# shayneobrien/generative-models

Hardware: AMD Instinct MI355X
Metric: images/sec (28x28 MNIST) per D+G step, NSGAN bs=256 (higher is better)
Workload: dtype f32; 1 GPU; NSGAN MNIST bs=256 fp32 per GPU (BASELINE.json configs[1]); 784-400-20 MLPs, N=50000 synthetic Bernoulli images, parity-mode RNG protocol, Adam 2e-4, D_steps=1; global_batch=256, parallelism=dp1, ranks_seen=1, gradient_exchange=none (1 rank), timing=one 2064-step timed region, cold_start_inclusive=False

## Files before the change

generative_models_amd/_lib.py:

```python
import ctypes
import os
from ctypes import POINTER, c_char_p, c_float, c_int, c_int32, c_int64, c_void_p

HERE = os.path.dirname(os.path.abspath(__file__))
LIB_PATH = os.environ.get("GM_LIB_PATH") or os.path.join(HERE, "libgm_hip.so")

GM_EINVAL = -10001
ACT_ID, ACT_RELU, ACT_SIGMOID = 0, 1, 2
ACT = {"id": ACT_ID, None: ACT_ID, "relu": ACT_RELU, "sigmoid": ACT_SIGMOID}
LOSS = {"ns": 0, "mm": 1, "w": 2, "ls": 3, "ra": 4, "fisher": 5, "f_total_variation": 6,
        "f_forward_kl": 7, "f_reverse_kl": 8, "f_pearson": 9, "f_hellinger": 10,
        "f_jensen_shannon": 11}


class Slot(ctypes.Structure):
    _fields_ = [("ctr", c_void_p), ("mul", c_int32), ("add", c_int32), ("ring", c_int32),
                ("stride", c_int64)]


def slot(ctr=0, mul=0, add=0, ring=0, stride=0):
    return Slot(ctr or None, mul, add, ring, stride)


NO_SLOT = Slot(None, 0, 0, 0, 0)
# ... 74 lines not shown


DRAW_SAMPLER, DRAW_NORMAL, DRAW_UNIFORM, DRAW_INFO = 0, 1, 2, 3
GM_EUNSUPPORTED = -10002

_P = c_void_p

_SIGNATURES = {
    "gm_version": (c_int, []),
    "gm_arch": (c_char_p, []),
    "gm_last_error": (c_char_p, []),
    "gm_tick": (c_int, [_P, _P, c_int64]),
    "gm_copy_slot_f32": (c_int, [_P, _P, Slot, _P, Slot, c_int64]),
    "gm_gather_rows": (c_int, [_P, _P, c_int64, _P, Slot, _P, c_int64, c_int, c_int]),
    "gm_linear_fwd": (c_int, [_P, _P, c_int64, Slot, _P, _P, _P, c_int64, c_int, c_int, c_int,
                              c_int]),
    "gm_linear_bwd_dx": (c_int, [_P, _P, c_int64, _P, _P, c_int64, _P, c_int64, c_int, c_int,
                                 c_int, c_int]),
    "gm_linear_bwd_dw": (c_int, [_P, _P, c_int64, _P, c_int64, Slot, _P, _P, c_int, c_int, c_int,
                                 c_int]),
    "gm_gan_loss": (c_int, [_P, c_int, c_int, _P, _P, c_int, c_int, POINTER(c_float), c_int,
                            c_float, _P, Slot, _P, _P, _P, _P]),
    "gm_gan_loss_phase": (c_int, [_P, c_int, c_int, _P, _P, c_int, c_int, POINTER(c_float), c_int,
                                  c_float, _P, Slot, _P, _P, _P, _P, c_int, _P, c_float]),
    "gm_l1_rows_dp": (c_int, [_P, _P, c_int64, _P, c_int64, c_int, c_int, c_int, c_int, _P, _P, c_int64, _P]),
    "gm_began_dloss_dp": (c_int, [_P, _P, c_int, c_int, _P, _P, Slot]),
    "gm_std_sums": (c_int, [_P, _P, c_int64, c_int, c_int, _P, _P]),
    "gm_std_from_sums": (c_int, [_P, _P, c_int64, _P]),
    "gm_adam": (c_int, [_P, _P, _P, _P, _P, c_int64, _P, Slot, ctypes.c_double, ctypes.c_double,
                        ctypes.c_double, ctypes.c_double, c_float]),
    "gm_interp": (c_int, [_P, _P, Slot, _P, c_int64, _P, c_int64, _P, c_int64, c_int, c_int]),
    "gm_gp_u": (c_int, [_P, _P, _P, c_int64, _P, _P, c_int64, c_int, c_int]),
    "gm_gp_norm": (c_int, [_P, _P, c_int64, _P, c_int64, _P, c_float, c_float, c_float, c_int,
                           c_int]),
    "gm_gp_dw2": (c_int, [_P, _P, _P, c_int64, _P, c_int64, _P, c_int, c_int]),
    "gm_bir_reparam": (c_int, [_P, _P, c_int64, _P, Slot, _P, c_int64, c_int, c_int]),
    "gm_bir_mmd": (c_int, [_P, _P, c_int64, _P, Slot, _P, _P, c_int64, c_int, c_int, c_float]),
    "gm_vae_reparam": (c_int, [_P, _P, c_int64, _P, Slot, _P, c_int64, _P, Slot, c_int, c_int]),
    "gm_vae_reparam_bwd": (c_int, [_P, _P, c_int64, _P, Slot, _P, c_int64, _P, c_int64, c_int,
                                   c_int]),
    "gm_sqerr_sigmoid_bwd": (c_int, [_P, _P, c_int64, _P, c_int64, _P, c_int64, _P, c_int, c_int]),
    "gm_sum_finalize": (c_int, [_P, _P, c_int, c_float, _P, Slot]),
    "gm_sum_finalize_tick": (c_int, [_P, _P, c_int, c_float, _P, Slot, _P]),
    "gm_sum_finalize2_tick": (c_int, [_P, _P, c_int, c_float, _P, Slot, _P, c_int, c_float, _P, Slot, _P]),
    "gm_vae_reparam_wide": (c_int, [_P, _P, c_int64, _P, Slot, _P, c_int64, _P, c_int, c_int, c_int]),
    "gm_vae_bwd_mid": (c_int, [_P, _P, c_int64, _P, _P, c_int64, _P, Slot, _P, c_int64, _P, _P, c_int64, _P, c_int64,
                               c_int, c_int, c_int]),
    "gm_vae_reparam_fwd": (c_int, [_P, _P, c_int64, _P, Slot, _P, c_int64, _P, c_int, c_int, c_int, _P, _P, _P,
                                   c_int64, c_int, c_int]),
    "gm_linear_bwd_dw_adam": (c_int, [_P, _P, c_int64, _P, c_int64, Slot, _P, _P, c_int, c_int, c_int,
                                      _P, _P, _P, _P, _P, _P, _P, Slot, ctypes.c_double,
                                      ctypes.c_double, ctypes.c_double, ctypes.c_double, c_float]),
    "gm_linear_fwd_interp": (c_int, [_P, _P, c_int64, Slot, _P, _P, _P, c_int64, c_int, c_int, c_int, c_int,
                                     _P, Slot, _P, c_int64, _P, c_int64, c_int]),
    "gm_linear_fwd_gather": (c_int, [_P, _P, c_int64, Slot, _P, _P, _P, c_int64, c_int, c_int, c_int,
                                     c_int, _P, c_int64, _P, Slot, _P, c_int64, c_int, c_int]),
    "gm_linear_fwd_gather_bits": (c_int, [_P, _P, c_int64, Slot, _P, _P, _P, c_int64, c_int, c_int, c_int,
                                          c_int, _P, c_int, c_int64, _P, Slot, _P, c_int64, c_int, c_int]),
    "gm_gather_rows_bits": (c_int, [_P, _P, c_int, c_int64, _P, Slot, _P, c_int64, c_int, c_int]),
    "gm_linear_bwd_dx_head": (c_int, [_P, _P, c_int64, _P, _P, c_int64, _P, c_int64, c_int, c_int,
                                      c_int, c_int, POINTER(HeadBwdArgs)]),
    "gm_linear_bwd_dx_head_fold": (c_int, [_P, _P, c_int64, _P, _P, c_int64, _P, c_int64, c_int, c_int,
                                           c_int, c_int, POINTER(HeadBwdArgs), POINTER(HeadFoldArgs)]),
    "gm_linear_fwd_sqerr": (c_int, [_P, _P, c_int64, _P, _P, _P, c_int64, c_int, c_int, c_int, _P, c_int64,
                                    _P, c_int64, _P, c_int64]),
    "gm_linear_bwd_dx_reparam": (c_int, [_P, _P, c_int64, _P, _P, c_int64, c_int, c_int, c_int, _P, c_int64,
                                         _P, Slot, _P, c_int64]),
    "gm_linear_fwd_headpart": (c_int, [_P, _P, c_int64, Slot, _P, _P, _P, c_int64, c_int, c_int, c_int, c_int,
                                       _P, _P, _P, c_int64, _P]),
    "gm_linear_bwd_dw_adam_head_fold": (c_int, [_P, _P, c_int64, _P, c_int64, Slot, _P, _P, c_int, c_int,
                                                c_int, _P, _P, _P, _P, _P, _P, _P, Slot, ctypes.c_double,
                                                ctypes.c_double, ctypes.c_double, ctypes.c_double, c_float,
                                                POINTER(HeadBwdArgs), POINTER(HeadFoldArgs)]),
    "gm_gather_rows_bits_packed": (c_int, [_P, _P, c_int, c_int64, _P, Slot, _P, c_int]),
    "gm_linear_fwd_gather_bits_packed": (c_int, [_P, _P, c_int64, Slot, _P, _P, _P, c_int64, c_int, c_int, c_int,
                                                 c_int, _P, c_int, c_int64, _P, Slot, _P, c_int]),
    "gm_linear_fwd_headpart_bits": (c_int, [_P, _P, c_int64, Slot, _P, _P, _P, c_int64, c_int, c_int, c_int, c_int,
                                            _P, _P, _P, c_int64, _P, _P, c_int, c_int]),
    "gm_linear_bwd_dw_adam_head_fold_bits": (c_int, [_P, _P, c_int64, _P, c_int64, Slot, _P, _P, c_int, c_int,
                                                     c_int, _P, _P, _P, _P, _P, _P, _P, Slot, ctypes.c_double,
                                                     ctypes.c_double, ctypes.c_double, ctypes.c_double, c_float,
                                                     POINTER(HeadBwdArgs), POINTER(HeadFoldArgs), _P, c_int, c_int]),
    "gm_linear_bwd_dw_adam_pair": (c_int, [_P, POINTER(DwAdamArgs), POINTER(DwAdamArgs)]),
    "gm_linear_bwd_dw_adam_pair_finalize": (c_int, [_P, POINTER(DwAdamArgs), POINTER(DwAdamArgs),
                                                    POINTER(Finalize2Args)]),
    "gm_linear_bwd_dw_adam_head": (c_int, [_P, _P, c_int64, _P, c_int64, Slot, _P, _P, c_int, c_int,
                                           c_int, _P, _P, _P, _P, _P, _P, _P, Slot, ctypes.c_double,
                                           ctypes.c_double, ctypes.c_double, ctypes.c_double, c_float,
                                           POINTER(HeadBwdArgs)]),
    "gm_linear_bwd_dw_adam_head_ex": (c_int, [_P, _P, c_int64, _P, c_int64, Slot, _P, _P, c_int, c_int,
                                              c_int, _P, _P, _P, _P, _P, _P, _P, Slot, ctypes.c_double,
                                              ctypes.c_double, ctypes.c_double, ctypes.c_double, c_float,
                                              POINTER(HeadBwdArgs), c_int]),
    "gm_gp_dw2_store": (c_int, [_P, _P, _P, c_int64, _P, c_int64, _P, c_int, c_int]),
    "gm_head_gp": (c_int, [_P, _P, c_int64, _P, _P, _P, _P, c_int64, c_int, c_int]),
    "gm_head_bwd_fused": (c_int, [_P, _P, c_int64, _P, _P, _P, _P, _P, c_int64, _P, _P, _P, Slot,
                                  c_float, c_int, c_int, c_int, c_int, _P, _P, _P, _P, _P, Slot,
                                  ctypes.c_double, ctypes.c_double, ctypes.c_double,
                                  ctypes.c_double, c_float, _P]),
    "gm_head_fwd_loss": (c_int, [_P, c_int, c_int, _P, c_int64, _P, _P, c_int, c_int, c_int,
                                 POINTER(c_float), c_int, c_float, _P, _P, _P, _P, _P, c_int64]),
    "gm_head_fwd_loss_final": (c_int, [_P, c_int, c_int, _P, c_int64, _P, _P, c_int, c_int, c_int,
                                       POINTER(c_float), c_int, c_float, _P, _P, _P, _P, _P, c_int64,
                                       _P, Slot, _P, _P]),
    "gm_head_bwd": (c_int, [_P, _P, c_int64, _P, _P, _P, _P, c_int64, _P, _P, _P, Slot, c_float,
                            c_int, c_int, c_int]),
    "gm_clock_probe": (c_int, [_P, c_int, _P, _P]),
    "gm_stream_create": (c_int, [POINTER(c_void_p)]),
    "gm_stream_destroy": (c_int, [_P]),
    "gm_stream_wait_event": (c_int, [_P, _P]),
    "gm_l1_rows": (c_int, [_P, _P, c_int64, _P, c_int64, c_int, c_int, c_int, _P, _P, c_int64, _P]),
    "gm_began_dloss": (c_int, [_P, _P, c_int, _P, _P, Slot]),
    "gm_began_update": (c_int, [_P, _P, _P, _P, c_float, c_float, c_int64, _P]),
    "gm_adam_scaled": (c_int, [_P, _P, _P, _P, _P, c_int64, _P, Slot, ctypes.c_double, ctypes.c_double,
                               ctypes.c_double, ctypes.c_double, c_float, _P]),
    "gm_linear_bwd_dx_add": (c_int, [_P, _P, c_int64, _P, _P, c_int64, _P, c_int64, c_int, c_int,
                                     c_int, c_int, _P, c_int64, c_float]),
    "gm_std_all": (c_int, [_P, _P, c_int64, c_int, c_int, _P, _P]),
    "gm_dragan_xhat": (c_int, [_P, _P, c_int64, _P, Slot, _P, Slot, _P, c_float, _P, c_int64, c_int,
                               c_int]),
    "gm_dragan_rows": (c_int, [_P, _P, _P, c_int64, _P, c_int64, _P, _P, c_float, c_float, c_float,
                               c_int, c_int]),
    "gm_dragan_head_bwd": (c_int, [_P, _P, c_int64, _P, c_int64, _P, _P, _P, _P, _P, c_int64, c_int,
                                   c_int]),
    "gm_fisher_commit": (c_int, [_P, _P]),
    "gm_dragan_head_bwd_store": (c_int, [_P, _P, c_int64, _P, c_int64, _P, _P, _P, _P, _P, c_int64, c_int,
                                   c_int]),
    "gm_info_q_loss": (c_int, [_P, _P, c_int64, _P, Slot, c_int64, c_int, c_int, c_int, c_int, c_float,
                               _P, c_int64, _P, Slot]),
    "gm_info_q_loss_dp": (c_int, [_P, _P, c_int64, _P, Slot, c_int64, c_int, c_int, c_int, c_int, c_int, c_float,
                                  _P, c_int64, _P, Slot]),
    "gm_act_bwd": (c_int, [_P, _P, _P, _P, c_int64, c_int]),
    "gm_randperm_prefix": (c_int, [ctypes.c_uint64, c_int64, c_int, _P]),
    "gm_mt19937_skip": (c_int, [_P, c_int64, ctypes.c_uint64]),
    "gm_comm_create": (c_int, [c_int, c_int, c_int64, POINTER(c_void_p), _P]),
    "gm_comm_connect": (c_int, [_P, _P]),
    "gm_comm_destroy": (c_int, [_P]),
    "gm_comm_error": (c_int, [_P, POINTER(c_int)]),
    "gm_comm_info": (c_int, [_P, POINTER(c_int)]),
    "gm_rccl_available": (c_int, []),
    "gm_rccl_unique_id": (c_int, [_P]),
    "gm_rccl_comm_create": (c_int, [c_int, c_int, _P, POINTER(c_void_p)]),
    "gm_rccl_allreduce_f32": (c_int, [_P, _P, _P, c_int64]),
    "gm_rccl_comm_destroy": (c_int, [_P]),
    "gm_comm_set_exchange": (c_int, [_P, c_int]),
    "gm_comm_set_max_blocks": (c_int, [_P, c_int]),
    "gm_comm_set_wait_seconds": (c_int, [_P, ctypes.c_double]),
    "gm_comm_buffer": (c_int, [_P, POINTER(c_void_p), POINTER(c_int64)]),
    "gm_allreduce_f32": (c_int, [_P, _P, _P, c_int64]),
    "gm_allreduce_adam_f32": (c_int, [_P, _P, _P, c_int64, _P, _P, _P, _P, Slot, ctypes.c_double,
                                      ctypes.c_double, ctypes.c_double, ctypes.c_double, c_float, _P]),
    "gm_allreduce_scalars": (c_int, [_P, _P, _P, c_int]),
    "gm_stage_in": (c_int, [_P, POINTER(StageSeg), c_int, Slot, c_int]),
    "gm_stage_in_gated": (c_int, [_P, POINTER(StageSeg), c_int, Slot, c_int, _P, Slot, ctypes.c_double, _P,
                                  c_int]),
    "gm_host_device_ptr": (c_int, [_P, POINTER(c_void_p)]),
    "gm_host_replay": (c_int, [_P, c_int64, POINTER(DrawOp), c_int, c_int]),
    "gm_host_replay_threads": (c_int, [c_int]),
    "gm_numpy_legacy_normal_f32": (c_int, [_P, _P, _P, _P, ctypes.c_double, ctypes.c_double, c_int64, _P, c_int]),
    "gm_fill_submit": (c_int64, [_P, c_int64, POINTER(DrawOp), c_int, c_int, _P, c_int64]),
    "gm_fill_wait": (c_int, [c_int64]),
    "gm_fill_completed": (c_int64, []),
    "gm_fill_reset": (c_int, []),
    "gm_host_replay_flavour": (c_int, [c_int]),
    "gm_graph_begin": (c_int, [_P]),
    "gm_graph_end": (c_int, [_P, POINTER(c_void_p)]),
# ... 61 lines not shown
```

generative_models_amd/csrc/gm_gemm.hip:

```cpp
#include "gm_common.h"
#include "gm_head.h"
#include "gm_gather.h"
#include "gm_ldsdma.h"

#include <cstdlib>
#include <type_traits>

typedef float f32x16 __attribute__((ext_vector_type(16)));

#ifdef GM_STAMPS
namespace gm_stamps {
constexpr int WAVES = 16, IDS = 40, HDR = 8, MAXB = 512, SLOT_WORDS = HDR + 2 * MAXB + WAVES * IDS * 2, SLOTS = 64;
static unsigned long long* host_buf = nullptr;
static int host_tile = 0, host_next = 0;
struct Ctx { unsigned long long* slot; int tile; };
__device__ __forceinline__ void rec(const Ctx& c, int tile, int id) {
    if (!c.slot || tile != c.tile || (threadIdx.x & 63)) return;
    __builtin_amdgcn_sched_barrier(0);
    unsigned long long* w = c.slot + HDR + 2 * MAXB + ((threadIdx.x >> 6) * IDS + id) * 2;
    w[0] = clock64(); w[1] = wall_clock64();
    __builtin_amdgcn_sched_barrier(0);
}
__device__ __forceinline__ void edge(const Ctx& c, bool exit_, int tile, int M, int N, int K, int mode) {
    if (!c.slot || threadIdx.x) return;
// ... 44 lines not shown
    int epi;
    int accumulate;
    gm_slot a_slot, b_slot;
    int tn;
    int lds_tm, lds_mpx;
    int dma;
    int vec_epi;
    const float* ip_eps; gm_slot ip_slot;
    const float* ip_x; int64_t ip_ldx;
    float* ip_out; int64_t ip_ldo;
    int ip_rows;
    gm_adam_epi adam;
    const float* hd_w2; const float* hd_b2; float* hd_part; int64_t hd_ldp; float* hd_snap;
    const float* sq_x; int64_t sq_ldx; float* sq_dA; int64_t sq_lda; float* sq_part; int64_t sq_ldp;
    const float* rp_ml; int64_t rp_ldml; const float* rp_eps; gm_slot rp_slot; float* rp_dml; int64_t rp_ldd;
    int rp_Z;
    const float* fold_w2;
    const float* add;
    int64_t ldadd;
    float add_scale;
    const uint32_t* pk_bits; int pk_wpr; int pk_rows;
    gm_label_src lb; const float* lb_E; int lb_C;
#ifdef GM_STAMPS
    gm_stamps::Ctx stamp;
#endif
};

template <bool SL>
__device__ __forceinline__ const float* slot_base(const float* P, const gm_slot& s) {
    if constexpr (SL) return P + gm_slot_offset(s);
    return P;
}
inline bool has_slot(const gm_slot& s) { return s.ctr != nullptr || s.add != 0; }

__device__ __forceinline__ float4 pk_expand(uint32_t word, int e) {
    const uint32_t v = word >> (e & 31);
    return make_float4((float)(v & 1u), (float)((v >> 1) & 1u), (float)((v >> 2) & 1u), (float)((v >> 3) & 1u));
}



template <bool VEC>
__device__ __forceinline__ float4 raw_kc(const float* __restrict__ P, int64_t ld, int x, int X,
                                         int kb, int K) {
    const float* row = P + (int64_t)min(x, X - 1) * ld;
    if (VEC)
        return *reinterpret_cast<const float4*>(row + min(kb, K - 4));
    return make_float4(row[min(kb + 0, K - 1)], row[min(kb + 1, K - 1)], row[min(kb + 2, K - 1)],
                       row[min(kb + 3, K - 1)]);
}
__device__ __forceinline__ float4 fix_kc(float4 v, int x, int X, int kb, int K) {
    const bool okx = x < X;
    v.x = (okx && kb + 0 < K) ? v.x : 0.f;
    v.y = (okx && kb + 1 < K) ? v.y : 0.f;
    v.z = (okx && kb + 2 < K) ? v.z : 0.f;
    v.w = (okx && kb + 3 < K) ? v.w : 0.f;
    return v;
}

__device__ __forceinline__ float4 raw_xc(const float* __restrict__ P, int64_t ld, int x, int X,
                                         int kb, int K) {
    const float* col = P + min(x, X - 1);
    return make_float4(col[(int64_t)min(kb + 0, K - 1) * ld], col[(int64_t)min(kb + 1, K - 1) * ld],
                       col[(int64_t)min(kb + 2, K - 1) * ld], col[(int64_t)min(kb + 3, K - 1) * ld]);
}
__device__ __forceinline__ float4 fix_xc(float4 v, int x, int X, int kb, int K, int ones_col,
                                         int ones_from = 0) {
    const bool okx = x < X, oc = (x == ones_col);
    v.x = (kb + 0 < K) ? (okx ? v.x : ((oc && kb + 0 >= ones_from) ? 1.f : 0.f)) : 0.f;
    v.y = (kb + 1 < K) ? (okx ? v.y : ((oc && kb + 1 >= ones_from) ? 1.f : 0.f)) : 0.f;
    v.z = (kb + 2 < K) ? (okx ? v.z : ((oc && kb + 2 >= ones_from) ? 1.f : 0.f)) : 0.f;
    v.w = (kb + 3 < K) ? (okx ? v.w : ((oc && kb + 3 >= ones_from) ? 1.f : 0.f)) : 0.f;
    return v;
}

__device__ __forceinline__ float fwd_value(const GemmP& p, float v, int n) {
    if (p.bias) v += p.bias[n];
    if (p.epi == GM_ACT_RELU) v = fmaxf(v, 0.f);
    else if (p.epi == GM_ACT_SIGMOID) v = gm_sigmoid(v);
    return v;
}

template <int MODE, bool LBL = false>
__device__ __forceinline__ void store_element(const GemmP& p, float v, int m, int n) {
    if (MODE == MODE_FWD) {
        if constexpr (LBL) v += p.lb_E[(int64_t)n * p.lb_C + gm_row_label(p.lb, m, p.lb_C)];
        v = fwd_value(p, v, n);
        p.C[(int64_t)m * p.ldc + n] = v;
        if (p.ip_out && m < p.ip_rows) {
            const float ev = (p.ip_eps + gm_slot_offset(p.ip_slot))[m];
            p.ip_out[(int64_t)m * p.ip_ldo + n] = gm_interp_unfused(ev, p.ip_x[(int64_t)m * p.ip_ldx + n], v);
        }
    } else if (MODE == MODE_DX) {
        if (p.add) v += p.add_scale * p.add[(int64_t)m * p.ldadd + n];
        if (p.epi == GM_ACT_RELU) {
            v = (p.aux[(int64_t)m * p.ldaux + n] > 0.f) ? v : 0.f;
        } else if (p.epi == GM_ACT_SIGMOID) {
            const float y = p.aux[(int64_t)m * p.ldaux + n];
            v = v * (y * (1.f - y));
        }
        float* cp = p.C + (int64_t)m * p.ldc + n;
        *cp = p.accumulate ? (*cp + v) : v;
        if (p.rp_dml) {
            const int Z = p.rp_Z;
            const float mu = p.rp_ml[(int64_t)m * p.rp_ldml + n], lv = p.rp_ml[(int64_t)m * p.rp_ldml + Z + n];
            const float e = (p.rp_eps + gm_slot_offset(p.rp_slot))[(int64_t)m * Z + n];
            p.rp_dml[(int64_t)m * p.rp_ldd + n] = v + 0.5f * (2.f * mu);
            p.rp_dml[(int64_t)m * p.rp_ldd + Z + n] = ((v * e) * expf(lv / 2.f)) / 2.f + 0.5f * (expf(lv) - 1.f);
        }
    } else {
        const bool is_b = (n == p.n_real);
        float* cp = is_b ? (p.db + m) : (p.C + (int64_t)m * p.ldc + n);
        if (p.accumulate) v += *cp;
        *cp = v;
        if (p.adam.enabled) {
            const int64_t o = is_b ? (int64_t)m : ((int64_t)m * p.ldc + n);
            float* pp = (is_b ? p.adam.pb : p.adam.pW) + o;
            float* mm = (is_b ? p.adam.mb : p.adam.mW) + o;
            float* vv = (is_b ? p.adam.vb : p.adam.vW) + o;
            const int64_t si = gm_slot_index(p.adam.sched_slot);
            const float step_size = p.adam.sched[2 * si], bc2_sqrt = p.adam.sched[2 * si + 1];
            float P = *pp, M = *mm, V = *vv;
            adam_update(P, v, M, V, step_size, bc2_sqrt, p.adam.omb1, p.adam.b2, p.adam.omb2,
                        p.adam.eps, p.adam.wd, p.adam.clamp);
            *pp = P; *mm = M; *vv = V;
        }
    }
}

__device__ __forceinline__ float4 ld4(const float* q) { return *reinterpret_cast<const float4*>(q); }
__device__ __forceinline__ void st4(float* q, float4 v) { *reinterpret_cast<float4*>(q) = v; }

template <int MODE>
__device__ __forceinline__ void store4(const GemmP& p, float4 v, int m, int n) {
    if (MODE == MODE_FWD) {
        if (p.bias) { const float4 b = ld4(p.bias + n); v.x += b.x; v.y += b.y; v.z += b.z; v.w += b.w; }
        if (p.epi == GM_ACT_RELU) { v.x = fmaxf(v.x, 0.f); v.y = fmaxf(v.y, 0.f); v.z = fmaxf(v.z, 0.f); v.w = fmaxf(v.w, 0.f); }
        else if (p.epi == GM_ACT_SIGMOID) { v.x = gm_sigmoid(v.x); v.y = gm_sigmoid(v.y); v.z = gm_sigmoid(v.z); v.w = gm_sigmoid(v.w); }
        st4(p.C + (int64_t)m * p.ldc + n, v);
        if (p.ip_out && m < p.ip_rows) {
            const float ev = (p.ip_eps + gm_slot_offset(p.ip_slot))[m];
            const float4 x = ld4(p.ip_x + (int64_t)m * p.ip_ldx + n);
            st4(p.ip_out + (int64_t)m * p.ip_ldo + n,
                make_float4(gm_interp_unfused(ev, x.x, v.x), gm_interp_unfused(ev, x.y, v.y),
                            gm_interp_unfused(ev, x.z, v.z), gm_interp_unfused(ev, x.w, v.w)));
        }
    } else if (MODE == MODE_DX) {
        if (p.add) {
            const float4 a = ld4(p.add + (int64_t)m * p.ldadd + n);
            v.x += p.add_scale * a.x; v.y += p.add_scale * a.y; v.z += p.add_scale * a.z; v.w += p.add_scale * a.w;
        }
        if (p.epi == GM_ACT_RELU) {
            const float4 y = ld4(p.aux + (int64_t)m * p.ldaux + n);
            v.x = (y.x > 0.f) ? v.x : 0.f; v.y = (y.y > 0.f) ? v.y : 0.f; v.z = (y.z > 0.f) ? v.z : 0.f; v.w = (y.w > 0.f) ? v.w : 0.f;
        } else if (p.epi == GM_ACT_SIGMOID) {
            const float4 y = ld4(p.aux + (int64_t)m * p.ldaux + n);
            v.x = v.x * (y.x * (1.f - y.x)); v.y = v.y * (y.y * (1.f - y.y));
            v.z = v.z * (y.z * (1.f - y.z)); v.w = v.w * (y.w * (1.f - y.w));
        }
        float* cp = p.C + (int64_t)m * p.ldc + n;
        if (p.accumulate) { const float4 c = ld4(cp); v.x = c.x + v.x; v.y = c.y + v.y; v.z = c.z + v.z; v.w = c.w + v.w; }
        st4(cp, v);
    } else {
        const int64_t o = (int64_t)m * p.ldc + n;
        if (p.accumulate) { const float4 c = ld4(p.C + o); v.x += c.x; v.y += c.y; v.z += c.z; v.w += c.w; }
        st4(p.C + o, v);
        if (p.adam.enabled) {
            const int64_t si = gm_slot_index(p.adam.sched_slot);
            const float step_size = p.adam.sched[2 * si], bc2_sqrt = p.adam.sched[2 * si + 1];
            float4 P = ld4(p.adam.pW + o), M = ld4(p.adam.mW + o), V = ld4(p.adam.vW + o);
            adam_update(P.x, v.x, M.x, V.x, step_size, bc2_sqrt, p.adam.omb1, p.adam.b2, p.adam.omb2, p.adam.eps, p.adam.wd, p.adam.clamp);
            adam_update(P.y, v.y, M.y, V.y, step_size, bc2_sqrt, p.adam.omb1, p.adam.b2, p.adam.omb2, p.adam.eps, p.adam.wd, p.adam.clamp);
            adam_update(P.z, v.z, M.z, V.z, step_size, bc2_sqrt, p.adam.omb1, p.adam.b2, p.adam.omb2, p.adam.eps, p.adam.wd, p.adam.clamp);
            adam_update(P.w, v.w, M.w, V.w, step_size, bc2_sqrt, p.adam.omb1, p.adam.b2, p.adam.omb2, p.adam.eps, p.adam.wd, p.adam.clamp);
            st4(p.adam.pW + o, P); st4(p.adam.mW + o, M); st4(p.adam.vW + o, V);
        }
    }
}

template <int MODE>
__device__ __forceinline__ void store_group(const GemmP& p, float4 v, int m, int n, int ncap) {
    const int nreal = (MODE == MODE_DW) ? p.n_real : p.N;
    if (n + 3 < nreal && n + 3 < ncap) { store4<MODE>(p, v, m, n); return; }
    if (n < p.N && n < ncap) store_element<MODE>(p, v.x, m, n);
    if (n + 1 < p.N && n + 1 < ncap) store_element<MODE>(p, v.y, m, n + 1);
    if (n + 2 < p.N && n + 2 < ncap) store_element<MODE>(p, v.z, m, n + 2);
    if (n + 3 < p.N && n + 3 < ncap) store_element<MODE>(p, v.w, m, n + 3);
}

__device__ __forceinline__ int red_idx(int w, int row, int col) {
    return (w * 32 + row) * 32 + (col ^ ((((row >> 2) ^ row) & 1) << 4));
}

template <int MODE, int WAVES, int ROWS = 32, bool LBL = false>
__device__ __forceinline__ void reduce_and_store(const GemmP& p, const float* red, int t, int m0,
                                                 int n0, int ncap = 0x7fffffff, int rcap = 32) {
    if (MODE == MODE_FWD && p.hd_part) {
#pragma unroll
        for (int e = 0; e < 1024 / (WAVES * 64); ++e) {
            const int row = (t >> 5) + e * (WAVES * 2), col = t & 31;
            const bool live = !(ROWS < 32 && row >= ROWS) && row < rcap;
            float v = 0.f;
            if (live) {
#pragma unroll
                for (int ww = 0; ww < WAVES; ++ww) v += red[red_idx(ww, row, col)];
            }
            const int m = m0 + row, n = n0 + col;
            const bool ok = live && m < p.M && n < p.N && n < ncap;
            float pv = 0.f;
            if (ok) {
                const float w = p.hd_w2[n];
                const float y = fwd_value(p, v, n);
                p.C[(int64_t)m * p.ldc + n] = y;
                pv = y * w;
                if (m == 0 && p.hd_snap) {
                    p.hd_snap[n] = w;
                    if (n == 0) p.hd_snap[p.N] = p.hd_b2[0];
                }
            }
#pragma unroll
            for (int o = 16; o > 0; o >>= 1) pv += __shfl_xor(pv, o, 64);
            if (col == 0 && live && m < p.M) p.hd_part[(int64_t)m * p.hd_ldp + (n0 >> 5)] = pv;
        }
        return;
    }
    if (MODE == MODE_FWD && p.sq_part) {
#pragma unroll
        for (int e = 0; e < 1024 / (WAVES * 64); ++e) {
            const int row = (t >> 5) + e * (WAVES * 2), col = t & 31;
            const bool live = !(ROWS < 32 && row >= ROWS) && row < rcap;
            float v = 0.f;
            if (live) {
#pragma unroll
                for (int ww = 0; ww < WAVES; ++ww) v += red[red_idx(ww, row, col)];
            }
            const int m = m0 + row, n = n0 + col;
            const bool ok = live && m < p.M && n < p.N && n < ncap;
            float pv = 0.f;
            if (ok) {
                const float r = fwd_value(p, v, n);
                p.C[(int64_t)m * p.ldc + n] = r;
                const float d = p.sq_x[(int64_t)m * p.sq_ldx + n] - r;
                pv = d * d;
                const float go = -(2.f * d);
                p.sq_dA[(int64_t)m * p.sq_lda + n] = (go * (1.f - r)) * r;
            }
#pragma unroll
            for (int o = 16; o > 0; o >>= 1) pv += __shfl_xor(pv, o, 64);
            if (col == 0 && live && m < p.M) p.sq_part[(int64_t)m * p.sq_ldp + (n0 >> 5)] = pv;
        }
        return;
    }
#pragma unroll
    for (int e = 0; e < 1024 / (WAVES * 64); ++e) {
        const int row = (t >> 5) + e * (WAVES * 2), col = t & 31;
        if ((ROWS < 32 && row >= ROWS) || row >= rcap) continue;
        float v = 0.f;
#pragma unroll
        for (int ww = 0; ww < WAVES; ++ww) v += red[red_idx(ww, row, col)];
        const int m = m0 + row, n = n0 + col;
        if (m >= p.M || n >= p.N || n >= ncap) continue;
        store_element<MODE, LBL>(p, v, m, n);
    }
}

__device__ __forceinline__ float4 keep4(bool ok, float4 v) {
    return make_float4(ok ? v.x : 0.f, ok ? v.y : 0.f, ok ? v.z : 0.f, ok ? v.w : 0.f);
}

template <int NMFMA, int NDSR, int NVMEM, int NDSW>
__device__ __forceinline__ void lds_stage_schedule() {
    constexpr int NMEM = NDSR + NVMEM + NDSW;
    int done = 0;
#pragma unroll
    for (int q = 0; q < NMFMA; ++q) {
        __builtin_amdgcn_sched_group_barrier(0x008, 1, 0);
        const int upto = (NMEM * (q + 1) + NMFMA - 1) / NMFMA;
#pragma unroll
        for (int i = 0; i < 8; ++i) {
            if (done < upto) {
                if (done < NDSR) __builtin_amdgcn_sched_group_barrier(0x100, 1, 0);
                else if (done < NDSR + NVMEM) __builtin_amdgcn_sched_group_barrier(0x020, 1, 0);
                else __builtin_amdgcn_sched_group_barrier(0x200, 1, 0);
                ++done;
            }
        }
    }
}

template <int MODE, int BM, int BN, int WTM, int WTN, int WK, int KU>
struct LdsCfg {
    static constexpr int WM = BM / WTM, WN = BN / WTN, NW = WM * WN * WK, NT = 64 * NW, BK = 8 * WK * KU;
    static constexpr int TI = WTM / 32, TJ = WTN / 32;
    static constexpr bool B_KC = (MODE == MODE_FWD);
    static constexpr int LDK = BK + 4, LDXB = BN + 4;
    static constexpr int A_SZ = BM * LDK;
    static constexpr int B_SZ = B_KC ? BN * LDK : BK * LDXB;
    static constexpr int STAGE = A_SZ + B_SZ;
    static constexpr int NBUF = 3;
    static constexpr int RED = WK * BM * BN;
    static constexpr int FLOATS = (NBUF * STAGE > RED) ? NBUF * STAGE : RED;
};

template <int MODE, int BM, int BN, int WTM, int WTN, int WK, int KU, int PD, int NS>
__global__ __launch_bounds__(64 * (BM / WTM) * (BN / WTN) * WK) void gemm_lds_kernel(GemmP p) {
    using C = LdsCfg<MODE, BM, BN, WTM, WTN, WK, KU>;
    constexpr int NT = C::NT, BK = C::BK, LDK = C::LDK, LDXB = C::LDXB, TI = C::TI, TJ = C::TJ;
    static_assert(MODE != MODE_DW, "forward (A, B k-contiguous) and input gradient (B = W[k][n]) only");
    static_assert(PD >= 2, "two stages are stored before the first barrier");
    __shared__ __attribute__((aligned(16))) float lds[C::FLOATS];

    const int t = threadIdx.x, lane = t & 63, w = t >> 6;
    const int r = lane & 31, h = lane >> 5;
    const int wk = w / (C::WM * C::WN), wmn = w % (C::WM * C::WN), wm = wmn / C::WN, wn = wmn % C::WN;
    const int b = blockIdx.x, xcd = b & 7, l = b >> 3;
    const int tile_m = xcd * p.lds_mpx + l / p.tn, tile_n = l % p.tn;
    if (tile_m >= p.lds_tm) return;
    const int m0 = tile_m * BM, n0 = tile_n * BN;
    const float* A = p.A;
    const float* B = p.B;
#ifdef GM_STAMPS
    const gm_stamps::Ctx st_slot = p.stamp; const int st_tile = (int)blockIdx.x;
#endif
    GM_STAMP_EDGE(p, false, st_tile, MODE + 10);
    GM_STAMP(st_slot, st_tile, 0);

    constexpr int KQ = BK / 4;
    constexpr int XQ = BN / 4;
    constexpr int UA = BM * KQ, CA = (UA + NT - 1) / NT;
    constexpr int UB = C::B_KC ? BN * KQ : BK * XQ, CB = (UB + NT - 1) / NT;
    const float* baseA[CA];
    const float* baseB[CB];
#pragma unroll
    for (int i = 0; i < CA; ++i) {
        const int u = min(t + i * NT, UA - 1);
        baseA[i] = A + (int64_t)min(m0 + u / KQ, p.M - 1) * p.lda + 4 * (u % KQ);
    }
#pragma unroll
    for (int i = 0; i < CB; ++i) {
        const int u = min(t + i * NT, UB - 1);
        if (C::B_KC) baseB[i] = B + (int64_t)min(n0 + u / KQ, p.N - 1) * p.ldb + 4 * (u % KQ);
        else baseB[i] = B + min(n0 + 4 * (u % XQ), p.N - 4);
    }
    auto load_a = [&](const float* base, int i, int q, bool inside) -> float4 {
        if (inside) return *reinterpret_cast<const float4*>(base + q * BK);
// ... 368 lines not shown
        }
    };

    float fw[FOLD == 1 ? MI : 1];
    if constexpr (FOLD == 1) {
#pragma unroll
        for (int e = 0; e < MI; ++e) fw[e] = (am + e < p.M) ? p.fold_w2[min(am + e, p.M - 1)] : 0.f;
    }
    f32x4 acc[MI][NI];
#pragma unroll
    for (int e = 0; e < MI; ++e)
#pragma unroll
        for (int f = 0; f < NI; ++f) acc[e][f] = f32x4{0.f, 0.f, 0.f, 0.f};

    const int nq = (nchunks - w + WAVES - 1) / WAVES;
    const bool special = (ones_col >= n0 && ones_col < n0 + 16 * NI) || (p.K & 15) || OF;
    auto run = [&](auto special_tag) {
        constexpr bool SPECIAL = decltype(special_tag)::value;
        if (nq > 0) issue(w);
        GM_STAMP(st_slot, st_tile, 17);
        if constexpr (FOLD == 1) fold_fill_lds(*fold, sds, fold->R);
        for (int q = 0; q < nq; ++q) {
            const int c = w + q * WAVES;
            slab::wait_vm<0>();
            if (q < 8) GM_STAMP(st_slot, st_tile, 20 + 2 * q);
            ILV<MI> ra[4]; ILV<NI> rb[4];
#pragma unroll
            for (int s = 0; s < 4; ++s) {
                const int row = 4 * s + g4;
                ra[s] = *reinterpret_cast<const ILV<MI>*>(buf + row * (16 * MI) + MI * i16);
                rb[s] = *reinterpret_cast<const ILV<NI>*>(buf + 256 * MI + row * (16 * NI) + NI * i16);
            }
            slab::wait_lgkm0();
            if (q + 1 < nq) issue(c + WAVES);
#pragma unroll
            for (int s = 0; s < 4; ++s) {
                const int k = 16 * c + 4 * s + g4;
                float fa[MI], fb[NI];
#pragma unroll
                for (int e = 0; e < MI; ++e) {
                    float v = ra[s].v[e];
                    if constexpr (FOLD == 1) v = (v > 0.f) ? sds[min(k, p.K - 1)] * fw[e] : 0.f;
                    if constexpr (SPECIAL) v = (k < p.K) ? v : 0.f;
                    fa[e] = v;
                }
#pragma unroll
                for (int f = 0; f < NI; ++f) {
                    float v = rb[s].v[f];
                    if constexpr (SPECIAL) {
                        float one = 1.f;
                        if constexpr (OF) one = (k >= p.ones_from) ? 1.f : 0.f;
                        v = (bn + f == ones_col) ? one : v;
                    }
                    fb[f] = v;
                }
#pragma unroll
                for (int e = 0; e < MI; ++e)
#pragma unroll
                    for (int f = 0; f < NI; ++f)
                        acc[e][f] = __builtin_amdgcn_mfma_f32_16x16x4f32(fa[e], fb[f], acc[e][f], 0, 0, 0);
            }
            GM_STAMP_AFTER(acc[MI - 1][NI - 1][0]);
            if (q < 8) GM_STAMP(st_slot, st_tile, 21 + 2 * q);
        }
    };
    if (special) run(std::true_type{}); else run(std::false_type{});
    GM_STAMP(st_slot, st_tile, 9);
    dw_il_reduce<MI, NI>(p, red, acc, m0, n0, true);
    GM_STAMP(st_slot, st_tile, 12);
    GM_STAMP_EDGE(p, true, st_tile, MODE_DW + 20);
}

template <int MODE, bool DMA, int MI, int NI> struct RedSize {
    static constexpr int base = 16 * 32 * 32;
    static constexpr int onepass = (MODE == MODE_DW && MI * NI > 4) ? 16 * 256 * MI * NI : 0;
    static constexpr int dma = (MODE == MODE_DW && DMA) ? 16 * (MI + NI) * 256 : 0;
    static constexpr int m1 = base > onepass ? base : onepass;
    static constexpr int value = m1 > dma ? m1 : dma;
};

template <int MODE, bool VEC, int WAVES, int G, bool XV, int MI, int NI, bool OF = false, int FOLD = 0, bool DMA = false,
          bool TP = false, bool PK = false, bool SL = true, bool LBL = false>
__device__ __forceinline__ void gemm16_body(const GemmP& p, float* red, int bx, int by,
                                            float* sds = nullptr, const FoldP* fold = nullptr, int gx = 0) {
    static_assert(!TP || (FOLD == 1 && !DMA), "two-phase losses: folded weight gradient, operands through registers");
    static_assert(FOLD == 0 || (FOLD == 1 && MODE == MODE_DW && XV) || (FOLD == 2 && MODE == MODE_DX && VEC),
                  "folded head: 16-byte operand paths only");
    static_assert(G == 1, "per-chunk schedule (G stays in the kernel names so that they keep their shape across rounds)");
    static_assert(!PK || (WAVES == 16 && !DMA && ((MODE == MODE_FWD && VEC) || (MODE == MODE_DW && XV))),
                  "bit-packed operand rows: 16-byte operand paths through registers only");
    if constexpr (DMA && MODE == MODE_DW && XV && WAVES == 16 && FOLD != 2) {
        gemm16_dw_dma<MI, NI, OF, FOLD, SL>(p, red, bx, by, sds, fold, gx);
        return;
    }
    const int t = threadIdx.x;
    const int lane = t & 63, w = t >> 6;
    const int i16 = lane & 15, g4 = lane >> 4;
    const int m0 = by * (16 * MI), n0 = bx * (16 * NI);
#ifdef GM_STAMPS
    const gm_stamps::Ctx st_slot = p.stamp; const int st_tile = by * (int)gridDim.x + bx;
#endif
    GM_STAMP_EDGE(p, false, st_tile, MODE);
    GM_STAMP(st_slot, st_tile, 0);

    const float* A = slot_base<SL>(p.A, p.a_slot);
    const float* B = slot_base<SL>(p.B, p.b_slot);
    const int b_cols = (MODE == MODE_DW) ? p.n_real : p.N;
    const int ones_col = (MODE == MODE_DW && p.db) ? p.n_real : -1;
    const int nchunks = (p.K + 15) >> 4;
    GM_STAMP_AFTER(A); GM_STAMP_AFTER(B); GM_STAMP_AFTER(nchunks);
    GM_STAMP(st_slot, st_tile, 16);

    float4 fw[FOLD == 1 ? MI : 1];
    float fds[FOLD == 2 ? MI : 1];
    const int xq_ld = lane & 3, xe_ld = (lane >> 2) & 3;
    constexpr bool XMAP_A = MODE == MODE_DW && XV, XMAP_B = MODE != MODE_FWD && XV;
    const int ia = XMAP_A ? sigma16(i16) : i16, ib = XMAP_B ? sigma16(i16) : i16;
    if constexpr (FOLD == 1) {
#pragma unroll
        for (int mi = 0; mi < MI; ++mi)
            fw[mi] = *reinterpret_cast<const float4*>(
                p.fold_w2 + min(m0 + 16 * mi + 4 * xq_ld, p.M - 4));
    }
    auto load_a = [&](int c, int mi) -> float4 {
        const int kb = 16 * c + 4 * g4, x0 = m0 + 16 * mi;
        if (MODE == MODE_DW) {
            if (XV) return raw_xc4_16(A, p.lda, x0, p.M, c, p.K, lane);
            return raw_xc(A, p.lda, x0 + i16, p.M, kb, p.K);
        }
        return raw_kc<VEC>(A, p.lda, x0 + i16, p.M, kb, p.K);
    };
    auto load_b = [&](int c, int ni) -> float4 {
        const int kb = 16 * c + 4 * g4, x0 = n0 + 16 * ni;
        if (MODE == MODE_FWD) return raw_kc<VEC>(B, p.ldb, x0 + i16, p.N, kb, p.K);
        if (XV) return raw_xc4_16(B, p.ldb, x0, b_cols, c, p.K, lane);
        return raw_xc(B, p.ldb, x0 + i16, b_cols, kb, p.K);
    };
    auto fix_a = [&](float4 v, int c, int mi, float4 wk) -> float4 {
        const int kb = 16 * c + 4 * g4, x = m0 + 16 * mi + ia;
        if constexpr (FOLD == 1)
            v = fold_dh4(v, sds[min(16 * c + 4 * g4 + xe_ld, p.K - 1)], fw[mi]);
        if constexpr (FOLD == 2) v = fold_dh4(v, fds[mi], wk);
        if (MODE == MODE_DW)
            return fix_xc(XV ? lane48_transpose(v, lane) : v, x, p.M, kb, p.K, -1);
        return fix_kc(v, x, p.M, kb, p.K);
    };
    auto fix_b = [&](float4 v, int c, int ni) -> float4 {
        const int kb = 16 * c + 4 * g4, x = n0 + 16 * ni + ib;
        if (MODE == MODE_FWD) return fix_kc(v, x, p.N, kb, p.K);
        return fix_xc(XV ? lane48_transpose(v, lane) : v, x, b_cols, kb, p.K, ones_col, OF ? p.ones_from : 0);
    };

    f32x4 acc[MI][NI];
#pragma unroll
    for (int mi = 0; mi < MI; ++mi)
#pragma unroll
        for (int ni = 0; ni < NI; ++ni) acc[mi][ni] = f32x4{0.f, 0.f, 0.f, 0.f};

    const int nq = (nchunks - w + WAVES - 1) / WAVES;
    auto consume = [&](const float4 (&ra)[MI], const float4 (&rb)[NI], float4 wk, int q) {
        const int cq = w + q * WAVES;
        float4 fa[MI], fb[NI];
#pragma unroll
        for (int mi = 0; mi < MI; ++mi) fa[mi] = fix_a(ra[mi], cq, mi, wk);
#pragma unroll
        for (int ni = 0; ni < NI; ++ni) fb[ni] = fix_b(rb[ni], cq, ni);
        GM_STAMP_AFTER(fa[MI - 1].x); GM_STAMP_AFTER(fb[NI - 1].x);
// ... 100 lines not shown
        }
        for (int q = q0; q < q_pk; ++q) do_chunk(yes, no, q);
        for (int q = max(q0, q_pk); q < nq_s; ++q) do_chunk(no, no, q);
    } else {
    int q_first = 0;
    if constexpr (FOLD != 0) {
        float4 ra[MI], rb[NI];
        float4 wk = make_float4(0.f, 0.f, 0.f, 0.f);
        const bool have = nq > 0;
        float4 pv[4];
        if constexpr (FOLD == 1 && !TP) {
            if (t < fold->R) fold_part_load(*fold, t, pv);
        }
        if constexpr (FOLD == 2) {
            if (t < 16 * MI) fold_part_load(*fold, min(m0 + t, fold->R - 1), pv);
        }
        if (have) {
#pragma unroll
            for (int mi = 0; mi < MI; ++mi) ra[mi] = load_a(w, mi);
#pragma unroll
            for (int ni = 0; ni < NI; ++ni) rb[ni] = load_b(w, ni);
            wk = load_wk(w);
        }
        GM_STAMP(st_slot, st_tile, 17);
        if constexpr (FOLD == 1 && !TP) fold_fill_lds_pre(*fold, sds, fold->R, pv);
        else if constexpr (FOLD == 2) {
            if (t < 16 * MI) {
                float s_, ds_, l_;
                fold_row_of(*fold, min(m0 + t, fold->R - 1), fold_score_of(*fold, pv), s_, ds_, l_);
                sds[t] = ds_;
            }
            GM_STAMP(st_slot, st_tile, 15);
            __syncthreads();
#pragma unroll
            for (int mi = 0; mi < MI; ++mi) fds[mi] = sds[16 * mi + i16];
        }
        else fold_prologue();
        GM_STAMP(st_slot, st_tile, 13);
        if (have) consume(ra, rb, wk, 0);
        q_first = 1;
    }
    for (int q = q_first; q < nq; ++q) {
        float4 ra[MI], rb[NI];
        const int cc = w + q * WAVES;
#pragma unroll
        for (int mi = 0; mi < MI; ++mi) ra[mi] = load_a(cc, mi);
#pragma unroll
        for (int ni = 0; ni < NI; ++ni) rb[ni] = load_b(cc, ni);
        const float4 wk = load_wk(cc);
        consume(ra, rb, wk, q);
    }
    }
    GM_STAMP(st_slot, st_tile, 9);
    if constexpr (MODE == MODE_DW && WAVES == 16 && MI * NI > 4) {
        if (p.vec_epi) {
            dw_reduce_onepass<MI, NI, false, XMAP_A>(p, red, acc, m0, n0, false);
            GM_STAMP(st_slot, st_tile, 12);
            GM_STAMP_EDGE(p, true, st_tile, MODE);
            return;
        }
    }
#pragma unroll
    for (int bm = 0; bm < (MI + 1) / 2; ++bm)
#pragma unroll
        for (int bn = 0; bn < (NI + 1) / 2; ++bn) {
            if (bm + bn > 0) __syncthreads();
#pragma unroll
            for (int rgi = 0; rgi < 4; ++rgi) {
                const int row = XMAP_A ? sigma16(g4 * 4 + rgi) : g4 * 4 + rgi;
                red[red_idx(w, row, ib)] = acc[2 * bm][2 * bn][rgi];
                if (2 * bn + 1 < NI) red[red_idx(w, row, 16 + ib)] = acc[2 * bm][(2 * bn + 1 < NI) ? 2 * bn + 1 : 0][rgi];
                if (2 * bm + 1 < MI) {
                    constexpr int MIX = MI > 1 ? MI - 1 : 0;
                    const int mu = (2 * bm + 1 < MI) ? 2 * bm + 1 : MIX;
                    red[red_idx(w, 16 + row, ib)] = acc[mu][2 * bn][rgi];
                    if (2 * bn + 1 < NI)
                        red[red_idx(w, 16 + row, 16 + ib)] = acc[mu][(2 * bn + 1 < NI) ? 2 * bn + 1 : 0][rgi];
                }
            }
            __syncthreads();
            if (bm + bn == 0) GM_STAMP(st_slot, st_tile, 10);
            reduce_and_store<MODE, WAVES, (MI > 1 ? 32 : 16), LBL>(p, red, t, m0 + 32 * bm, n0 + 32 * bn,
                                                              (2 * bn + 1 < NI) ? 0x7fffffff : n0 + 32 * bn + 16,
                                                              (2 * bm + 1 < MI) ? 32 : 16);
        }
    GM_STAMP(st_slot, st_tile, 12);
    GM_STAMP_EDGE(p, true, st_tile, MODE);
}

template <int MODE, bool VEC, int WAVES, int G, bool XV, int MI, int NI, bool DMA = false, bool SL = false>
__global__ __launch_bounds__(WAVES * 64) void gemm16_kernel(GemmP p) {
    __shared__ __attribute__((aligned(16))) float red[(WAVES == 16) ? RedSize<MODE, DMA, MI, NI>::value : WAVES * 32 * 32];
    gemm16_body<MODE, VEC, WAVES, G, XV, MI, NI, false, 0, DMA, false, false, SL>(p, red, blockIdx.x, blockIdx.y, nullptr, nullptr,
                                                                                  (int)gridDim.x);
}

template <bool VEC, int MI, int NI>
__global__ __launch_bounds__(1024) void gemm16_fwd_label_kernel(GemmP p) {
    __shared__ __attribute__((aligned(16))) float red[RedSize<MODE_FWD, false, MI, NI>::value];
    gemm16_body<MODE_FWD, VEC, 16, 1, false, MI, NI, false, 0, false, false, false, false, true>(p, red, blockIdx.x, blockIdx.y,
                                                                                                nullptr, nullptr, (int)gridDim.x);
}

template <int MODE, bool VEC, int G, bool XV, int MI, int NI, bool OF = false, bool FOLDED = false, bool DMA = false,
          bool TP = false, bool PK = false>
__device__ __forceinline__ void gemm16_with_head(const GemmP& p, const HeadBwdP& hp, int hrows,
                                                 int hblocks) {
    __shared__ __attribute__((aligned(16))) float red[RedSize<MODE, DMA, MI, NI>::value];
    __shared__ float sds[FOLDED ? FOLD_MAX_ROWS : 1];
    constexpr int FOLD = FOLDED ? (MODE == MODE_DW ? 1 : 2) : 0;
    if ((int)blockIdx.y < hrows) {
        const int bid = blockIdx.y * gridDim.x + blockIdx.x;
        if (bid < hblocks) head_bwd_body<TP>(hp, bid, sds);
        return;
    }
    gemm16_body<MODE, VEC, 16, G, XV, MI, NI, OF, FOLD, DMA, TP, PK, false>(p, red, blockIdx.x, blockIdx.y - hrows, sds, &hp.fold,
                                                                            (int)gridDim.x);
}

template <bool VEC, int G, bool XV, int MI, int NI, bool OF = false, bool FOLDED = false, bool DMA = false>
__global__ __launch_bounds__(1024) void gemm16_dw_head_kernel(GemmP p, HeadBwdP hp, int hrows,
                                                              int hblocks) {
    gemm16_with_head<MODE_DW, VEC, G, XV, MI, NI, OF, FOLDED, DMA>(p, hp, hrows, hblocks);
}

__global__ __launch_bounds__(1024) void gemm16_fwd_bits_kernel(GemmP p) {
    __shared__ __attribute__((aligned(16))) float red[RedSize<MODE_FWD, false, 2, 2>::value];
    gemm16_body<MODE_FWD, true, 16, 1, false, 2, 2, false, 0, false, false, true, false>(p, red, blockIdx.x, blockIdx.y);
}
__global__ __launch_bounds__(1024) void gemm16_dw_head_bits_kernel(GemmP p, HeadBwdP hp, int hrows, int hblocks) {
    gemm16_with_head<MODE_DW, false, 1, true, 2, 3, false, true, false, false, true>(p, hp, hrows, hblocks);
}

template <int MI, int NI>
__global__ __launch_bounds__(1024) void gemm16_dw_head_tp_kernel(GemmP p, HeadBwdP hp, int hrows, int hblocks) {
    gemm16_with_head<MODE_DW, false, 1, true, MI, NI, false, true, false, true>(p, hp, hrows, hblocks);
}

template <int G, int MI, int NI, bool FOLDED = false>
__global__ __launch_bounds__(1024) void gemm16_dx_head_kernel(GemmP p, HeadBwdP hp, int hrows,
                                                              int hblocks) {
    gemm16_with_head<MODE_DX, true, G, true, MI, NI, false, FOLDED>(p, hp, hrows, hblocks);
}

inline bool aligned16(const void* p) { return (reinterpret_cast<uintptr_t>(p) & 15) == 0; }

template <bool VEC, int G, int MI, int NI>
__global__ __launch_bounds__(1024) void gemm16_fwd_gather_kernel(GemmP p, GatherP gp, int grows,
                                                                 int gblocks) {
    __shared__ __attribute__((aligned(16))) float red[16 * 32 * 32];
    if ((int)blockIdx.y < grows) {
        const int bid = blockIdx.y * gridDim.x + blockIdx.x;
        if (bid < gblocks) gather_body(gp, bid);
        return;
    }
    gemm16_body<MODE_FWD, VEC, 16, G, false, MI, NI>(p, red, blockIdx.x, blockIdx.y - grows);
}

template <bool SL, bool GATHER>
__global__ __launch_bounds__(256) void gemm16_k32_fwd_kernel(GemmP p, GatherP gp, int grows, int gblocks) {
    if constexpr (GATHER) {
        if ((int)blockIdx.y < grows) {
            const int bid = blockIdx.y * gridDim.x + blockIdx.x;
            if (bid < gblocks) gather_body(gp, bid);
            return;
        }
    }
    const int by = (int)blockIdx.y - (GATHER ? grows : 0), bx = blockIdx.x;
    const int t = threadIdx.x, lane = t & 63, w = __builtin_amdgcn_readfirstlane(t >> 6);
    const int i16 = lane & 15, g4 = lane >> 4;
    const int m0 = 32 * by + 16 * (w >> 1), n0 = 64 * bx + 32 * (w & 1);
#ifdef GM_STAMPS
    const gm_stamps::Ctx st_slot = p.stamp; const int st_tile = by * (int)gridDim.x + bx;
#endif
    GM_STAMP_EDGE(p, false, st_tile, MODE_FWD);
    GM_STAMP(st_slot, st_tile, 0);
    if (m0 >= p.M || n0 >= p.N) { GM_STAMP_EDGE(p, true, st_tile, MODE_FWD); return; }
    const float* A = slot_base<SL>(p.A, p.a_slot);
    const float* B = slot_base<SL>(p.B, p.b_slot);
    float4 ra[2], rb[2][2];
#pragma unroll
    for (int c = 0; c < 2; ++c) {
        const int kb = 16 * c + 4 * g4;
        ra[c] = raw_kc<true>(A, p.lda, m0 + i16, p.M, kb, p.K);
#pragma unroll
        for (int ni = 0; ni < 2; ++ni) rb[c][ni] = raw_kc<true>(B, p.ldb, n0 + 16 * ni + i16, p.N, kb, p.K);
    }
    f32x4 part[2][2];
#pragma unroll
    for (int c = 0; c < 2; ++c) {
        const int kb = 16 * c + 4 * g4;
        const float4 fa = fix_kc(ra[c], m0 + i16, p.M, kb, p.K);
#pragma unroll
        for (int ni = 0; ni < 2; ++ni) {
            const float4 fb = fix_kc(rb[c][ni], n0 + 16 * ni + i16, p.N, kb, p.K);
            f32x4 c4 = f32x4{0.f, 0.f, 0.f, 0.f};
            c4 = __builtin_amdgcn_mfma_f32_16x16x4f32(fa.x, fb.x, c4, 0, 0, 0);
            c4 = __builtin_amdgcn_mfma_f32_16x16x4f32(fa.y, fb.y, c4, 0, 0, 0);
            c4 = __builtin_amdgcn_mfma_f32_16x16x4f32(fa.z, fb.z, c4, 0, 0, 0);
            c4 = __builtin_amdgcn_mfma_f32_16x16x4f32(fa.w, fb.w, c4, 0, 0, 0);
            part[c][ni] = c4;
            if (c == 0 && ni == 0) { GM_STAMP_AFTER(fa.x); GM_STAMP_AFTER(fb.x); GM_STAMP(st_slot, st_tile, 1); }
        }
    }
    GM_STAMP_AFTER(part[1][1][0]);
    GM_STAMP(st_slot, st_tile, 2);
    float v[2][4];
#pragma unroll
    for (int ni = 0; ni < 2; ++ni) {
        const int n = min(n0 + 16 * ni + i16, p.N - 1);
        const float bv = p.bias ? p.bias[n] : 0.f;
#pragma unroll
        for (int r = 0; r < 4; ++r) {
            float x = 0.f;
            x += part[0][ni][r];
            x += part[1][ni][r];
            if (p.bias) x += bv;
            v[ni][r] = x;
        }
    }
    if (p.epi == GM_ACT_RELU) {
#pragma unroll
        for (int ni = 0; ni < 2; ++ni)
#pragma unroll
            for (int r = 0; r < 4; ++r) v[ni][r] = fmaxf(v[ni][r], 0.f);
    } else if (p.epi == GM_ACT_SIGMOID) {
#pragma unroll
        for (int ni = 0; ni < 2; ++ni)
#pragma unroll
            for (int r = 0; r < 4; ++r) v[ni][r] = gm_sigmoid(v[ni][r]);
    }
#pragma unroll
    for (int ni = 0; ni < 2; ++ni) {
        const int n = n0 + 16 * ni + i16;
#pragma unroll
        for (int r = 0; r < 4; ++r) {
            const int m = m0 + 4 * g4 + r;
            if (m < p.M && n < p.N) p.C[(int64_t)m * p.ldc + n] = v[ni][r];
        }
    }
    if (p.ip_out) {
#pragma unroll
        for (int ni = 0; ni < 2; ++ni) {
            const int n = n0 + 16 * ni + i16;
#pragma unroll
            for (int r = 0; r < 4; ++r) {
                const int m = m0 + 4 * g4 + r;
                if (m < p.M && n < p.N && m < p.ip_rows) {
                    const float ev = (p.ip_eps + gm_slot_offset(p.ip_slot))[m];
                    p.ip_out[(int64_t)m * p.ip_ldo + n] = gm_interp_unfused(ev, p.ip_x[(int64_t)m * p.ip_ldx + n], v[ni][r]);
                }
            }
        }
    }
    GM_STAMP(st_slot, st_tile, 12);
    GM_STAMP_EDGE(p, true, st_tile, MODE_FWD);
}

template <int G, bool XV, int MI, int NI, bool DMA = false, bool SLA = true, bool SLB = true>
__global__ __launch_bounds__(1024) void gemm16_dw_pair_kernel(GemmP pa, GemmP pb, int na, int tna,
                                                              int tnb) {
    __shared__ __attribute__((aligned(16))) float red[RedSize<MODE_DW, DMA, MI, NI>::value];
    const int id = blockIdx.x;
    if (id < na) gemm16_body<MODE_DW, false, 16, G, XV, MI, NI, false, 0, DMA, false, false, SLA>(pa, red, id % tna, id / tna);
    else gemm16_body<MODE_DW, false, 16, G, XV, MI, NI, false, 0, DMA, false, false, SLB>(pb, red, (id - na) % tnb, (id - na) / tnb);
}

template <int G, bool XV, int MI, int NI, bool DMA = false, bool SLA = true, bool SLB = true>
__global__ __launch_bounds__(1024) void gemm16_dw_pair_fin_kernel(GemmP pa, GemmP pb, int na, int tna, int tnb,
                                                                  gm_fin2 f) {
    __shared__ __attribute__((aligned(16))) float red[RedSize<MODE_DW, DMA, MI, NI>::value];
    const int id = (int)blockIdx.x - 1;
    if (id < 0) gm_fin2_sums(f, reinterpret_cast<double*>(red));
    else if (id < na) gemm16_body<MODE_DW, false, 16, G, XV, MI, NI, false, 0, DMA, false, false, SLA>(pa, red, id % tna, id / tna);
    else gemm16_body<MODE_DW, false, 16, G, XV, MI, NI, false, 0, DMA, false, false, SLB>(pb, red, (id - na) % tnb, (id - na) / tnb);
    __syncthreads();
    if (threadIdx.x == 0) {
        const unsigned int arrived = __hip_atomic_fetch_add(f.done, 1u, __ATOMIC_RELAXED, __HIP_MEMORY_SCOPE_AGENT);
        if (arrived == gridDim.x - 1) {
            __hip_atomic_store(f.done, 0u, __ATOMIC_RELAXED, __HIP_MEMORY_SCOPE_AGENT);
            if (f.tick) *f.tick += 1;
        }
    }
}

template <int MODE>
int vec_epi_ok(const GemmP& p) {
    if (!aligned16(p.C) || p.ldc % 4 != 0) return 0;
    if (MODE == MODE_FWD) {
        if (p.bias && !aligned16(p.bias)) return 0;
        if (p.ip_out && !(aligned16(p.ip_out) && aligned16(p.ip_x) && p.ip_ldo % 4 == 0 && p.ip_ldx % 4 == 0)) return 0;
    } else if (MODE == MODE_DX) {
        if (p.epi != GM_ACT_ID && !(aligned16(p.aux) && p.ldaux % 4 == 0)) return 0;
        if (p.add && !(aligned16(p.add) && p.ldadd % 4 == 0)) return 0;
    } else {
        if (p.adam.enabled && !(aligned16(p.adam.pW) && aligned16(p.adam.mW) && aligned16(p.adam.vW))) return 0;
    }
    return 1;
}

struct Rider {
    const HeadBwdP* head = nullptr;
    const GatherP* gather = nullptr;
    const GemmP* pair = nullptr;
    bool pair_xvec = false;
    const gm_fin2* fin = nullptr;
};

enum { T22 = 0, T24, T42, T12, T23, T32 };
inline int tile_mi(int t) { return t == T42 ? 4 : t == T32 ? 3 : t == T12 ? 1 : 2; }
inline int tile_ni(int t) { return t == T24 ? 4 : t == T23 ? 3 : 2; }

template <int MODE>
int pick_tile(const GemmP& p) {
    const int tm = (p.M + TM - 1) / TM, tn = (p.N + TN - 1) / TN;
    int t = T22;
    if (tm * tn > 256 && (p.K + 15) / 16 >= 32) t = (tn >= tm) ? T24 : T42;
    else if (tm * tn <= 128 && p.M > 16) t = T12;
    if (MODE == MODE_DW) {
        if (t == T24 && tm * ((p.N + 47) / 48) <= 256) t = T23;
        else if (t == T42 && tn * ((p.M + 47) / 48) <= 256) t = T32;
        else if (t == T22 && tm * tn > 256) {
            if (tn >= tm && tm * ((p.N + 47) / 48) <= 256) t = T23;
            else if (tn < tm && tn * ((p.M + 47) / 48) <= 256) t = T32;
        }
    }
    if (MODE == MODE_FWD && t == T42 && !p.hd_part && !p.sq_part && tn * ((p.M + 47) / 48) <= 256) t = T32;
    return t;
}

#define GM_TILE_SWITCH(tile, dma, LAUNCH)                                           \
    do {                                                                            \
        switch (tile) {                                                             \
        case T24: LAUNCH(2, 4, false); break;                                       \
        case T42: LAUNCH(4, 2, false); break;                                       \
        case T12: LAUNCH(1, 2, false); break;                                       \
        case T23: if (dma) LAUNCH(2, 3, true); else LAUNCH(2, 3, false); break;     \
        case T32: if (dma) LAUNCH(3, 2, true); else LAUNCH(3, 2, false); break;     \
        default: LAUNCH(2, 2, false); break;                                        \
        }                                                                           \
    } while (0)

template <int MODE>
int launch(hipStream_t s, const GemmP& p_in, bool vec, bool xvec = false, const Rider& rider = Rider()) {
    const HeadBwdP* head = rider.head;
    const bool folded = head && head->fold.enabled;
    GemmP p = p_in;
    p.vec_epi = vec_epi_ok<MODE>(p);
#ifdef GM_STAMPS
    p.stamp.slot = gm_stamps::host_buf ? gm_stamps::host_buf + (size_t)(gm_stamps::host_next++ % gm_stamps::SLOTS) * gm_stamps::SLOT_WORDS
                                       : nullptr;
    p.stamp.tile = gm_stamps::host_tile;
#endif
    const bool xv = xvec && MODE != MODE_FWD;
    const bool slots = has_slot(p.a_slot) || has_slot(p.b_slot);
    if (slots && (folded || p.pk_bits)) {
        gm_set_error("ring slots on the operands of a folded-head / bit-packed launch are not supported");
        return GM_EINVAL;
    }
    const bool ride_head = head && !slots;
    auto dma_ok = [&](const GemmP& q, bool qxv) {
        constexpr int dma_min_k = 768;
        return MODE == MODE_DW && qxv && q.K >= dma_min_k && q.M >= 4 && q.n_real >= 4 &&
               ((int64_t)q.K + 64) * (q.lda > q.ldb ? q.lda : q.ldb) < (1ll << 31);
    };
    p.dma = dma_ok(p, xv);
    if (p.pk_bits) {
        if constexpr (MODE == MODE_FWD) {
            if (!vec || !p.hd_part || rider.gather || p.ip_out) {
                gm_set_error("bit-packed rows: the forward needs 16-byte aligned operands and the folded head's partial dots");
                return GM_EINVAL;
            }
            const dim3 bgrid((p.N + 31) / 32, (p.M + 31) / 32);
            hipLaunchKernelGGL(gemm16_fwd_bits_kernel, bgrid, dim3(1024), 0, s, p);
            GM_LAUNCH_RET();
        } else if constexpr (MODE == MODE_DW) {
            if (!head || !folded || head->fold.enabled != 1 || !xv || p.ones_from > 0 || rider.pair) {
                gm_set_error("bit-packed rows: the weight gradient needs the folded head of a separable loss and "
                             "16-byte aligned operands");
                return GM_EINVAL;
            }
            p.dma = false;
            const dim3 bgrid((p.N + 47) / 48, (p.M + 31) / 32);
            const int hblocks = gm_head_bwd_blocks(*head);
            const int hrows = (hblocks + (int)bgrid.x - 1) / (int)bgrid.x;
            hipLaunchKernelGGL(gemm16_dw_head_bits_kernel, dim3(bgrid.x, bgrid.y + hrows), dim3(1024), 0, s, p, *head,
                               hrows, hblocks);
            GM_LAUNCH_RET();
        } else {
// ... 8 lines not shown
                if (head) hipLaunchKernelGGL(head_bwd_kernel, dim3(gm_head_bwd_blocks(*head)), dim3(1024), 0, s, *head);
                if (rider.gather)
                    hipLaunchKernelGGL(gather_rows_kernel, dim3(gm_gather_blocks(*rider.gather, 4)), dim3(256), 0, s, *rider.gather);
                return launch_lds<MODE>(s, p, cfg);
            }
        }
    }
    if constexpr (MODE == MODE_FWD) {
        if (vec && p.K <= 32 && !head && !p.hd_part && !p.sq_part) {
            const dim3 kgrid((p.N + 63) / 64, (p.M + 31) / 32);
            if (rider.gather) {
                const GatherP& gp = *rider.gather;
                const int gblocks = gm_gather_blocks(gp, 4);
                const int grows = (gblocks + (int)kgrid.x - 1) / (int)kgrid.x;
                const dim3 ggrid(kgrid.x, kgrid.y + grows);
                if (slots) hipLaunchKernelGGL((gemm16_k32_fwd_kernel<true, true>), ggrid, dim3(256), 0, s, p, gp, grows, gblocks);
                else hipLaunchKernelGGL((gemm16_k32_fwd_kernel<false, true>), ggrid, dim3(256), 0, s, p, gp, grows, gblocks);
            } else {
                if (slots) hipLaunchKernelGGL((gemm16_k32_fwd_kernel<true, false>), kgrid, dim3(256), 0, s, p, GatherP{}, 0, 0);
                else hipLaunchKernelGGL((gemm16_k32_fwd_kernel<false, false>), kgrid, dim3(256), 0, s, p, GatherP{}, 0, 0);
            }
            GM_LAUNCH_RET();
        }
    }
    const int tile = pick_tile<MODE>(p);
    const int mi = tile_mi(tile), ni = tile_ni(tile);
    const dim3 grid((p.N + 16 * ni - 1) / (16 * ni), (p.M + 16 * mi - 1) / (16 * mi));
    if constexpr (MODE == MODE_DW) {
        if (ride_head) {
            const int hblocks = gm_head_bwd_blocks(*head);
            const int hrows = (hblocks + (int)grid.x - 1) / (int)grid.x;
            const dim3 hgrid(grid.x, grid.y + hrows);
            if (folded && (!xv || p.ones_from > 0)) {
                gm_set_error("folded head: the weight gradient needs 16-byte aligned operands and no stacked rows");
                return GM_EINVAL;
            }
#define GM_LH(X, OFV, FD) GM_TILE_SWITCH(tile, p.dma && (X), GM_LH1_##X##_##OFV##_##FD)
#define GM_LHK(X, OFV, FD, MI_, NI_, D_) hipLaunchKernelGGL((gemm16_dw_head_kernel<false, 1, X, MI_, NI_, OFV, FD, ((X) && (D_))>), hgrid, dim3(1024), 0, s, p, *head, hrows, hblocks)
#define GM_LH1_true_false_true(MI_, NI_, D_) GM_LHK(true, false, true, MI_, NI_, D_)
#define GM_LH1_true_true_false(MI_, NI_, D_) GM_LHK(true, true, false, MI_, NI_, D_)
#define GM_LH1_true_false_false(MI_, NI_, D_) GM_LHK(true, false, false, MI_, NI_, D_)
#define GM_LH1_false_true_false(MI_, NI_, D_) GM_LHK(false, true, false, MI_, NI_, D_)
#define GM_LH1_false_false_false(MI_, NI_, D_) GM_LHK(false, false, false, MI_, NI_, D_)
            if (folded && head->fold.enabled == 2) {
                p.dma = false;
#define GM_LHTP(MI_, NI_, D_) hipLaunchKernelGGL((gemm16_dw_head_tp_kernel<MI_, NI_>), hgrid, dim3(1024), 0, s, p, *head, hrows, hblocks)
                GM_TILE_SWITCH(tile, false, GM_LHTP);
#undef GM_LHTP
            } else if (folded) GM_LH(true, false, true);
            else if (xv) { if (p.ones_from > 0) GM_LH(true, true, false); else GM_LH(true, false, false); }
            else { if (p.ones_from > 0) GM_LH(false, true, false); else GM_LH(false, false, false); }
#undef GM_LH1_false_false_false
#undef GM_LH1_false_true_false
#undef GM_LH1_true_false_false
#undef GM_LH1_true_true_false
#undef GM_LH1_true_false_true
#undef GM_LHK
#undef GM_LH
            GM_LAUNCH_RET();
        }
    }
    if constexpr (MODE == MODE_DX) {
        if (ride_head && vec && xv && (tile == T22 || tile == T12)) {
            const int hblocks = gm_head_bwd_blocks(*head);
            const int hrows = (hblocks + (int)grid.x - 1) / (int)grid.x;
            const dim3 hgrid(grid.x, grid.y + hrows);
            if (tile == T12) {
                if (folded) hipLaunchKernelGGL((gemm16_dx_head_kernel<1, 1, 2, true>), hgrid, dim3(1024), 0, s, p, *head, hrows, hblocks);
                else hipLaunchKernelGGL((gemm16_dx_head_kernel<1, 1, 2, false>), hgrid, dim3(1024), 0, s, p, *head, hrows, hblocks);
            } else {
                if (folded) hipLaunchKernelGGL((gemm16_dx_head_kernel<1, 2, 2, true>), hgrid, dim3(1024), 0, s, p, *head, hrows, hblocks);
                else hipLaunchKernelGGL((gemm16_dx_head_kernel<1, 2, 2, false>), hgrid, dim3(1024), 0, s, p, *head, hrows, hblocks);
            }
            GM_LAUNCH_RET();
        }
    }
    if (folded) {
        gm_set_error("folded head: this launch configuration cannot carry it (needs the riding kernels: 16-byte "
                     "aligned operands)");
        return GM_EINVAL;
    }
    if (head)
        hipLaunchKernelGGL(head_bwd_kernel, dim3(gm_head_bwd_blocks(*head)), dim3(1024), 0, s, *head);
    if constexpr (MODE == MODE_FWD) {
        if (rider.gather) {
            const GatherP& gp = *rider.gather;
            if (vec && (tile == T22 || tile == T12)) {
                const int gblocks = gm_gather_blocks(gp, 16);
                const int grows = (gblocks + (int)grid.x - 1) / (int)grid.x;
                const dim3 ggrid(grid.x, grid.y + grows);
                if (tile == T12) hipLaunchKernelGGL((gemm16_fwd_gather_kernel<true, 1, 1, 2>), ggrid, dim3(1024), 0, s, p, gp, grows, gblocks);
                else hipLaunchKernelGGL((gemm16_fwd_gather_kernel<true, 1, 2, 2>), ggrid, dim3(1024), 0, s, p, gp, grows, gblocks);
                GM_LAUNCH_RET();
            }
            hipLaunchKernelGGL(gather_rows_kernel, dim3(gm_gather_blocks(gp, 4)), dim3(256), 0, s, gp);
        }
    }
    if constexpr (MODE == MODE_DW) {
        if (rider.pair) {
            GemmP pb = *rider.pair;
            pb.vec_epi = vec_epi_ok<MODE_DW>(pb);
            if (xv && rider.pair_xvec && tile != T12 && pb.K == p.K) {
                const bool dma = p.dma && dma_ok(pb, true);
                p.dma = pb.dma = dma;
                const int tna = (int)grid.x, na = (int)(grid.x * grid.y);
                const int tnb = (pb.N + 16 * ni - 1) / (16 * ni), tmb = (pb.M + 16 * mi - 1) / (16 * mi);
                const dim3 pgrid(na + tnb * tmb);
                const bool sl_b = has_slot(pb.a_slot) || has_slot(pb.b_slot);
#define GM_LP2(K_, GRID_, MI_, NI_, D_, ...)                                                                              \
    do {                                                                                                                  \
        if (slots) hipLaunchKernelGGL((K_<1, true, MI_, NI_, D_, true, true>), GRID_, dim3(1024), 0, s, __VA_ARGS__);     \
        else if (sl_b) hipLaunchKernelGGL((K_<1, true, MI_, NI_, D_, false, true>), GRID_, dim3(1024), 0, s, __VA_ARGS__); \
        else hipLaunchKernelGGL((K_<1, true, MI_, NI_, D_, false, false>), GRID_, dim3(1024), 0, s, __VA_ARGS__);         \
    } while (0)
#define GM_LP(MI_, NI_, D_) GM_LP2(gemm16_dw_pair_kernel, pgrid, MI_, NI_, D_, p, pb, na, tna, tnb)
#define GM_LPF(MI_, NI_, D_) GM_LP2(gemm16_dw_pair_fin_kernel, dim3(pgrid.x + 1), MI_, NI_, D_, p, pb, na, tna, tnb, *rider.fin)
                if (rider.fin) GM_TILE_SWITCH(tile, dma, GM_LPF);
                else GM_TILE_SWITCH(tile, dma, GM_LP);
#undef GM_LP2
#undef GM_LPF
#undef GM_LP
                GM_LAUNCH_RET();
            }
            Rider none;
            int rc = launch<MODE_DW>(s, p_in, vec, xvec, none);
            if (rc) return rc;
            rc = launch<MODE_DW>(s, pb, false, rider.pair_xvec, none);
            if (rc || !rider.fin) return rc;
            const gm_fin2& f = *rider.fin;
            return gm_sum_finalize2_tick(s, f.pa, f.na, f.sa, f.oa, f.slot_a, f.pb, f.nb, f.sb, f.ob, f.slot_b, f.tick);
        }
    }
    if (MODE == MODE_DX && slots) { gm_set_error("ring slots: forward and weight-gradient operands only"); return GM_EINVAL; }
#define GM_L16K(V, X, MI_, NI_, D_)                                                                                          \
    do {                                                                                                                     \
        if (MODE != MODE_DX && slots)                                                                                        \
            hipLaunchKernelGGL((gemm16_kernel<MODE, V, 16, 1, X, MI_, NI_, (MODE == MODE_DW && (X) && (D_)), MODE != MODE_DX>), grid, dim3(1024), 0, s, p); \
        else                                                                                                                 \
            hipLaunchKernelGGL((gemm16_kernel<MODE, V, 16, 1, X, MI_, NI_, (MODE == MODE_DW && (X) && (D_)), false>), grid, dim3(1024), 0, s, p); \
    } while (0)
#define GM_L16_tt(MI_, NI_, D_) GM_L16K(true, true, MI_, NI_, D_)
#define GM_L16_tf(MI_, NI_, D_) GM_L16K(true, false, MI_, NI_, D_)
#define GM_L16_ft(MI_, NI_, D_) GM_L16K(false, true, MI_, NI_, D_)
#define GM_L16_ff(MI_, NI_, D_) GM_L16K(false, false, MI_, NI_, D_)
    if (xv) { if (vec) GM_TILE_SWITCH(tile, p.dma, GM_L16_tt); else GM_TILE_SWITCH(tile, p.dma, GM_L16_ft); }
    else    { if (vec) GM_TILE_SWITCH(tile, false, GM_L16_tf); else GM_TILE_SWITCH(tile, false, GM_L16_ff); }
#undef GM_L16_ff
#undef GM_L16_ft
#undef GM_L16_tf
#undef GM_L16_tt
#undef GM_L16K
    GM_LAUNCH_RET();
}

inline gm_slot no_slot() { gm_slot z; z.ctr = nullptr; z.mul = 0; z.add = 0; z.ring = 0; z.stride = 0; return z; }

}

extern "C" int gm_linear_fwd(void* stream, const float* X, int64_t ldx, gm_slot x_slot,
                             const float* W, const float* bias, float* Y, int64_t ldy, int M,
                             int K, int N, int act) {
    GM_CHECK_ARG(X && W && Y && M > 0 && K > 0 && N > 0 && ldx >= K && ldy >= N);
    GM_CHECK_ARG(act >= GM_ACT_ID && act <= GM_ACT_SIGMOID);
    GemmP p{};
    p.A = X; p.B = W; p.C = Y; p.M = M; p.N = N; p.K = K;
    p.lda = ldx; p.ldb = K; p.ldc = ldy; p.bias = bias; p.epi = act;
    p.a_slot = x_slot; p.b_slot = no_slot();
    const bool vec = aligned16(X) && aligned16(W) && (ldx % 4 == 0) && (K % 4 == 0) &&
                     (x_slot.stride % 4 == 0);
    return launch<MODE_FWD>((hipStream_t)stream, p, vec);
}

extern "C" int gm_linear_fwd_label(void* stream, const float* X, int64_t ldx, const float* W, const float* bias,
                                   const float* E, int C, gm_label_src lab, float* Y, int64_t ldy, int M, int K, int N,
                                   int act) {
    GM_CHECK_ARG(X && W && E && lab.labels && Y && M > 0 && K > 0 && N > 0 && C > 0 && C <= 32 && ldx >= K && ldy >= N);
    GM_CHECK_ARG(act >= GM_ACT_ID && act <= GM_ACT_SIGMOID);
    GemmP p{};
    p.A = X; p.B = W; p.C = Y; p.M = M; p.N = N; p.K = K;
    p.lda = ldx; p.ldb = K; p.ldc = ldy; p.bias = bias; p.epi = act;
    p.a_slot = no_slot(); p.b_slot = no_slot();
    p.lb = lab; p.lb_E = E; p.lb_C = C;
    const bool vec = aligned16(X) && aligned16(W) && (ldx % 4 == 0) && (K % 4 == 0);
    const int tile = pick_tile<MODE_FWD>(p);
    const dim3 grid((N + 16 * tile_ni(tile) - 1) / (16 * tile_ni(tile)), (M + 16 * tile_mi(tile) - 1) / (16 * tile_mi(tile)));
    hipStream_t s = (hipStream_t)stream;
#define GM_LBL(MI_, NI_, D_)                                                                                \
    do {                                                                                                    \
// ... 58 lines not shown
    p.lda = ldx; p.ldb = K; p.ldc = ldy; p.bias = bias; p.epi = act;
    p.a_slot = x_slot; p.b_slot = no_slot();
    p.hd_w2 = w2; p.hd_b2 = b2; p.hd_part = part; p.hd_ldp = ldp; p.hd_snap = snap;
    p.pk_bits = xbits; p.pk_wpr = words_per_row; p.pk_rows = rows;
    const bool vec = aligned16(X) && aligned16(W) && (ldx % 4 == 0) && (K % 4 == 0) &&
                     (x_slot.stride % 4 == 0);
    return launch<MODE_FWD>((hipStream_t)stream, p, vec);
}

extern "C" int gm_linear_fwd_sqerr(void* stream, const float* X, int64_t ldx, const float* W,
                                  const float* bias, float* Y, int64_t ldy, int M, int K, int N,
                                  const float* target, int64_t ld_target, float* dA, int64_t lda,
                                  float* part, int64_t ldp) {
    GM_CHECK_ARG(X && W && Y && M > 0 && K > 0 && N > 0 && ldx >= K && ldy >= N);
    GM_CHECK_ARG(target && dA && part && ld_target >= N && lda >= N && ldp >= (N + 31) / 32);
    GM_CHECK_ARG(dA != Y && part != Y && part != dA && (const float*)dA != X && (const float*)part != X &&
                 (const float*)Y != target && (const float*)dA != target);
    GemmP p{};
    p.A = X; p.B = W; p.C = Y; p.M = M; p.N = N; p.K = K;
    p.lda = ldx; p.ldb = K; p.ldc = ldy; p.bias = bias; p.epi = GM_ACT_SIGMOID;
    p.a_slot = no_slot(); p.b_slot = no_slot();
    p.sq_x = target; p.sq_ldx = ld_target; p.sq_dA = dA; p.sq_lda = lda; p.sq_part = part; p.sq_ldp = ldp;
    const bool vec = aligned16(X) && aligned16(W) && (ldx % 4 == 0) && (K % 4 == 0);
    return launch<MODE_FWD>((hipStream_t)stream, p, vec);
}

static int fwd_gather_impl(void* stream, const float* X, int64_t ldx, gm_slot x_slot,
                           const float* W, const float* bias, float* Y, int64_t ldy, int M,
                           int K, int N, int act, const GatherP& g, float* out);

extern "C" int gm_linear_fwd_gather(void* stream, const float* X, int64_t ldx, gm_slot x_slot,
                                    const float* W, const float* bias, float* Y, int64_t ldy, int M,
                                    int K, int N, int act, const float* data, int64_t n_rows,
                                    const int64_t* idx, gm_slot idx_slot, float* out,
                                    int64_t ld_out, int B, int row_elems) {
    GatherP g{};
    const int rc = gm_gather_fill(data, n_rows, idx, idx_slot, out, ld_out, B, row_elems, &g);
    if (rc) return rc;
    return fwd_gather_impl(stream, X, ldx, x_slot, W, bias, Y, ldy, M, K, N, act, g, out);
}

extern "C" int gm_linear_fwd_gather_bits(void* stream, const float* X, int64_t ldx, gm_slot x_slot,
                                         const float* W, const float* bias, float* Y, int64_t ldy, int M,
                                         int K, int N, int act, const uint32_t* bits, int words_per_row,
                                         int64_t n_rows, const int64_t* idx, gm_slot idx_slot, float* out,
                                         int64_t ld_out, int B, int row_elems) {
    GatherP g{};
    const int rc = gm_gather_fill_bits(bits, words_per_row, n_rows, idx, idx_slot, out, ld_out, B, row_elems, &g);
    if (rc) return rc;
    return fwd_gather_impl(stream, X, ldx, x_slot, W, bias, Y, ldy, M, K, N, act, g, out);
}

extern "C" int gm_linear_fwd_gather_bits_packed(void* stream, const float* X, int64_t ldx, gm_slot x_slot,
                                                const float* W, const float* bias, float* Y, int64_t ldy, int M,
                                                int K, int N, int act, const uint32_t* bits, int words_per_row,
                                                int64_t n_rows, const int64_t* idx, gm_slot idx_slot,
                                                uint32_t* out_bits, int B) {
    GatherP g{};
    const int rc = gm_gather_fill_bits_packed(bits, words_per_row, n_rows, idx, idx_slot, out_bits, B, &g);
    if (rc) return rc;
    return fwd_gather_impl(stream, X, ldx, x_slot, W, bias, Y, ldy, M, K, N, act, g, reinterpret_cast<float*>(out_bits));
}

static int fwd_gather_impl(void* stream, const float* X, int64_t ldx, gm_slot x_slot,
                           const float* W, const float* bias, float* Y, int64_t ldy, int M,
                           int K, int N, int act, const GatherP& g, float* out) {
    GM_CHECK_ARG(X && W && Y && M > 0 && K > 0 && N > 0 && ldx >= K && ldy >= N);
    GM_CHECK_ARG(act >= GM_ACT_ID && act <= GM_ACT_SIGMOID);
    GM_CHECK_ARG(out != Y && out != X);
    GemmP p{};
    p.A = X; p.B = W; p.C = Y; p.M = M; p.N = N; p.K = K;
    p.lda = ldx; p.ldb = K; p.ldc = ldy; p.bias = bias; p.epi = act;
    p.a_slot = x_slot; p.b_slot = no_slot();
    const bool vec = aligned16(X) && aligned16(W) && (ldx % 4 == 0) && (K % 4 == 0) &&
                     (x_slot.stride % 4 == 0);
    Rider r;
    r.gather = &g;
    return launch<MODE_FWD>((hipStream_t)stream, p, vec, false, r);
}

static int dx_impl(void* stream, const float* dA, int64_t lda, const float* W, float* dX, int64_t ldx,
                   const float* below, int64_t ld_below, int M, int K, int N, int epi,
                   const float* add, int64_t ldadd, float add_scale, const HeadBwdP* head = nullptr,
                   const float* fold_w2 = nullptr);

extern "C" int gm_linear_bwd_dx_head(void* stream, const float* dA, int64_t lda, const float* W,
                                     float* dX, int64_t ldx, const float* below, int64_t ld_below,
                                     int M, int K, int N, int epi, const gm_head_bwd_args* head) {
    GM_CHECK_ARG(head);
    GM_CHECK_ARG((const float*)dX != head->H && (const float*)dX != head->dS &&
                 (const float*)dX != head->rowloss && dX != head->dH);
    HeadBwdP hp{};
    const int rc = gm_head_from_args(*head, &hp);
    if (rc) return rc;
    return dx_impl(stream, dA, lda, W, dX, ldx, below, ld_below, M, K, N, epi, nullptr, 0, 0.f, &hp);
}

extern "C" int gm_linear_bwd_dx_reparam(void* stream, const float* dA, int64_t lda, const float* W,
                                        float* dZ, int64_t ldz, int M, int Z, int N, const float* ml,
                                        int64_t ldml, const float* eps, gm_slot eps_slot, float* dml,
                                        int64_t ldd) {
    GM_CHECK_ARG(dA && W && dZ && M > 0 && Z > 0 && N > 0 && lda >= N && ldz >= Z);
    GM_CHECK_ARG(ml && eps && dml && ldml >= 2 * Z && ldd >= 2 * Z && dml != dZ && (const float*)dml != ml &&
                 (const float*)dml != dA);
    GemmP p{};
    p.A = dA; p.B = W; p.C = dZ; p.M = M; p.N = Z; p.K = N;
    p.lda = lda; p.ldb = Z; p.ldc = ldz; p.epi = GM_ACT_ID;
    p.a_slot = no_slot(); p.b_slot = no_slot();
    p.rp_ml = ml; p.rp_ldml = ldml; p.rp_eps = eps; p.rp_slot = eps_slot; p.rp_dml = dml; p.rp_ldd = ldd;
    p.rp_Z = Z;
    const bool vec = aligned16(dA) && (lda % 4 == 0) && (N % 4 == 0);
    const bool xvec = aligned16(W) && (Z % 4 == 0);
    return launch<MODE_DX>((hipStream_t)stream, p, vec, xvec);
}

extern "C" int gm_linear_bwd_dx_head_fold(void* stream, const float* H, int64_t ldh, const float* W,
                                          float* dX, int64_t ldx, const float* below, int64_t ld_below,
                                          int M, int K, int N, int epi, const gm_head_bwd_args* head,
                                          const gm_head_fold_args* fold) {
    GM_CHECK_ARG(head && fold && head->gen_mode && head->H == H && head->B == M && head->Hd == N);
    GM_CHECK_ARG((const float*)dX != H && dX != fold->S && dX != fold->dS && dX != fold->rowloss);
    HeadBwdP hp{};
    const int rc = gm_head_from_args(*head, &hp, fold);
    if (rc) return rc;
    return dx_impl(stream, H, ldh, W, dX, ldx, below, ld_below, M, K, N, epi, nullptr, 0, 0.f, &hp, fold->snap);
}

extern "C" int gm_linear_bwd_dx(void* stream, const float* dA, int64_t lda, const float* W,
                                float* dX, int64_t ldx, const float* below, int64_t ld_below,
                                int M, int K, int N, int epi) {
    return dx_impl(stream, dA, lda, W, dX, ldx, below, ld_below, M, K, N, epi, nullptr, 0, 0.f);
}

extern "C" int gm_linear_bwd_dx_add(void* stream, const float* dA, int64_t lda, const float* W,
                                    float* dX, int64_t ldx, const float* below, int64_t ld_below,
                                    int M, int K, int N, int epi, const float* add, int64_t ldadd,
                                    float add_scale) {
    GM_CHECK_ARG(add && ldadd >= K);
    return dx_impl(stream, dA, lda, W, dX, ldx, below, ld_below, M, K, N, epi, add, ldadd, add_scale);
}

static int dx_impl(void* stream, const float* dA, int64_t lda, const float* W, float* dX, int64_t ldx,
                   const float* below, int64_t ld_below, int M, int K, int N, int epi,
                   const float* add, int64_t ldadd, float add_scale, const HeadBwdP* head,
                   const float* fold_w2) {
    GM_CHECK_ARG(dA && W && dX && M > 0 && K > 0 && N > 0 && lda >= N && ldx >= K);
    GM_CHECK_ARG(epi == GM_ACT_ID || (below && ld_below >= K));
    GemmP p{};
    p.A = dA; p.B = W; p.C = dX; p.M = M; p.N = K; p.K = N;
    p.lda = lda; p.ldb = K; p.ldc = ldx; p.aux = below; p.ldaux = ld_below; p.epi = epi;
    p.add = add; p.ldadd = ldadd; p.add_scale = add_scale;
    p.fold_w2 = fold_w2;
    p.a_slot = no_slot(); p.b_slot = no_slot();
    const bool vec = aligned16(dA) && (lda % 4 == 0) && (N % 4 == 0) && (!fold_w2 || aligned16(fold_w2));
    const bool xvec = aligned16(W) && (K % 4 == 0);
    Rider r;
    r.head = head;
    return launch<MODE_DX>((hipStream_t)stream, p, vec, xvec, r);
}

static int dw_impl(void* stream, const float* dA, int64_t lda, const float* X, int64_t ldx,
                   gm_slot x_slot, float* dW, float* db, int M, int K, int N, int accumulate,
                   const gm_adam_epi* adam, const HeadBwdP* head = nullptr, int ones_from = 0,
                   const float* fold_w2 = nullptr);
static int dw_fill(const float* dA, int64_t lda, const float* X, int64_t ldx, gm_slot x_slot,
                   float* dW, float* db, int M, int K, int N, int accumulate,
                   const gm_adam_epi* adam, GemmP* out, bool* xvec);

extern "C" int gm_linear_bwd_dw(void* stream, const float* dA, int64_t lda, const float* X,
                                int64_t ldx, gm_slot x_slot, float* dW, float* db, int M, int K,
                                int N, int accumulate) {
    return dw_impl(stream, dA, lda, X, ldx, x_slot, dW, db, M, K, N, accumulate, nullptr);
}

extern "C" int gm_linear_bwd_dw_adam(void* stream, const float* dA, int64_t lda, const float* X,
                                     int64_t ldx, gm_slot x_slot, float* dW, float* db, int M,
                                     int K, int N, float* pW, float* mW, float* vW, float* pb,
                                     float* mb, float* vb, const float* sched, gm_slot sched_slot,
                                     double beta1, double beta2, double eps, double weight_decay,
                                     float clamp) {
    GM_CHECK_ARG(db && pW && mW && vW && pb && mb && vb && sched);
    gm_adam_epi a{};
    a.pW = pW; a.mW = mW; a.vW = vW; a.pb = pb; a.mb = mb; a.vb = vb; a.sched = sched;
    a.sched_slot = sched_slot; a.omb1 = (float)(1.0 - beta1); a.b2 = (float)beta2;
    a.omb2 = (float)(1.0 - beta2); a.eps = (float)eps; a.wd = (float)weight_decay; a.clamp = clamp;
    a.enabled = 1;
    return dw_impl(stream, dA, lda, X, ldx, x_slot, dW, db, M, K, N, 0, &a);
}

extern "C" int gm_linear_bwd_dw_adam_head(void* stream, const float* dA, int64_t lda,
                                          const float* X, int64_t ldx, gm_slot x_slot, float* dW,
                                          float* db, int M, int K, int N, float* pW, float* mW,
                                          float* vW, float* pb, float* mb, float* vb,
                                          const float* sched, gm_slot sched_slot, double beta1,
                                          double beta2, double eps, double weight_decay, float clamp,
                                          const gm_head_bwd_args* head) {
    return gm_linear_bwd_dw_adam_head_ex(stream, dA, lda, X, ldx, x_slot, dW, db, M, K, N, pW, mW, vW, pb, mb,
                                         vb, sched, sched_slot, beta1, beta2, eps, weight_decay, clamp, head, 0);
}

extern "C" int gm_linear_bwd_dw_adam_head_ex(void* stream, const float* dA, int64_t lda,
                                             const float* X, int64_t ldx, gm_slot x_slot, float* dW,
                                             float* db, int M, int K, int N, float* pW, float* mW,
                                             float* vW, float* pb, float* mb, float* vb,
                                             const float* sched, gm_slot sched_slot, double beta1,
                                             double beta2, double eps, double weight_decay, float clamp,
                                             const gm_head_bwd_args* head, int ones_from) {
    GM_CHECK_ARG(head);
    GM_CHECK_ARG(!sched || (db && pW && mW && vW && pb && mb && vb));
    GM_CHECK_ARG((const float*)head->w2 != pW || !pW);
    GM_CHECK_ARG(head->gw2 != dW);
    HeadBwdP hp{};
    const int rc = gm_head_from_args(*head, &hp);
    if (rc) return rc;
    gm_adam_epi a{};
    if (sched) {
        a.pW = pW; a.mW = mW; a.vW = vW; a.pb = pb; a.mb = mb; a.vb = vb; a.sched = sched;
        a.sched_slot = sched_slot; a.omb1 = (float)(1.0 - beta1); a.b2 = (float)beta2;
        a.omb2 = (float)(1.0 - beta2); a.eps = (float)eps; a.wd = (float)weight_decay; a.clamp = clamp;
        a.enabled = 1;
    }
    return dw_impl(stream, dA, lda, X, ldx, x_slot, dW, db, M, K, N, 0, sched ? &a : nullptr, &hp, ones_from);
}

extern "C" int gm_linear_bwd_dw_adam_head_fold(void* stream, const float* H, int64_t ldh,
                                               const float* X, int64_t ldx, gm_slot x_slot, float* dW,
                                               float* db, int M, int K, int N, float* pW, float* mW,
                                               float* vW, float* pb, float* mb, float* vb,
                                               const float* sched, gm_slot sched_slot, double beta1,
                                               double beta2, double eps, double weight_decay, float clamp,
                                               const gm_head_bwd_args* head, const gm_head_fold_args* fold) {
    GM_CHECK_ARG(head && fold && !head->gen_mode && head->H == H && 2 * head->B == M && head->Hd == N);
    GM_CHECK_ARG(!sched || (db && pW && mW && vW && pb && mb && vb));
    GM_CHECK_ARG((const float*)head->w2 != pW || !pW);
    GM_CHECK_ARG(head->gw2 != dW && (const float*)dW != H);
    GM_CHECK_ARG(fold->snap != (const float*)head->w2 && fold->snap != (const float*)head->b2);
    HeadBwdP hp{};
    const int rc = gm_head_from_args(*head, &hp, fold);
    if (rc) return rc;
    gm_adam_epi a{};
    if (sched) {
        a.pW = pW; a.mW = mW; a.vW = vW; a.pb = pb; a.mb = mb; a.vb = vb; a.sched = sched;
        a.sched_slot = sched_slot; a.omb1 = (float)(1.0 - beta1); a.b2 = (float)beta2;
        a.omb2 = (float)(1.0 - beta2); a.eps = (float)eps; a.wd = (float)weight_decay; a.clamp = clamp;
        a.enabled = 1;
    }
    return dw_impl(stream, H, ldh, X, ldx, x_slot, dW, db, M, K, N, 0, sched ? &a : nullptr, &hp, 0, fold->snap);
}

extern "C" int gm_linear_bwd_dw_adam_head_fold_bits(void* stream, const float* H, int64_t ldh,
                                                    const float* X, int64_t ldx, gm_slot x_slot, float* dW,
                                                    float* db, int M, int K, int N, float* pW, float* mW,
                                                    float* vW, float* pb, float* mb, float* vb,
                                                    const float* sched, gm_slot sched_slot, double beta1,
                                                    double beta2, double eps, double weight_decay, float clamp,
                                                    const gm_head_bwd_args* head, const gm_head_fold_args* fold,
                                                    const uint32_t* xbits, int words_per_row, int rows) {
    GM_CHECK_ARG(head && fold && !head->gen_mode && head->H == H && 2 * head->B == M && head->Hd == N);
    GM_CHECK_ARG(!sched || (db && pW && mW && vW && pb && mb && vb));
    GM_CHECK_ARG((const float*)head->w2 != pW || !pW);
    GM_CHECK_ARG(head->gw2 != dW && (const float*)dW != H);
    GM_CHECK_ARG(fold->snap != (const float*)head->w2 && fold->snap != (const float*)head->b2);
    GM_CHECK_ARG(xbits && rows > 0 && rows <= M && rows % 32 == 0 && words_per_row * 32 >= K && K % 4 == 0);
    GM_CHECK_ARG((const void*)xbits != (const void*)dW && (const void*)xbits != (const void*)pW);
    HeadBwdP hp{};
    const int rc = gm_head_from_args(*head, &hp, fold);
    if (rc) return rc;
    gm_adam_epi a{};
    if (sched) {
        a.pW = pW; a.mW = mW; a.vW = vW; a.pb = pb; a.mb = mb; a.vb = vb; a.sched = sched;
        a.sched_slot = sched_slot; a.omb1 = (float)(1.0 - beta1); a.b2 = (float)beta2;
        a.omb2 = (float)(1.0 - beta2); a.eps = (float)eps; a.wd = (float)weight_decay; a.clamp = clamp;
        a.enabled = 1;
    }
    GemmP p{};
    bool xvec = false;
    const int rf = dw_fill(H, ldh, X, ldx, x_slot, dW, db, M, K, N, 0, sched ? &a : nullptr, &p, &xvec);
    if (rf) return rf;
    p.fold_w2 = fold->snap;
    if (!aligned16(fold->snap)) xvec = false;
    p.pk_bits = xbits; p.pk_wpr = words_per_row; p.pk_rows = rows;
    Rider r;
    r.head = &hp;
    return launch<MODE_DW>((hipStream_t)stream, p, false, xvec, r);
}

static int dw_adam_fill(const gm_dw_adam_args& a, GemmP* p, bool* xvec) {
    if (!a.sched)
        return dw_fill(a.dA, a.lda, a.X, a.ldx, a.x_slot, a.dW, a.db, a.M, a.K, a.N, 0, nullptr, p, xvec);
    GM_CHECK_ARG(a.db && a.pW && a.mW && a.vW && a.pb && a.mb && a.vb);
    gm_adam_epi e{};
    e.pW = a.pW; e.mW = a.mW; e.vW = a.vW; e.pb = a.pb; e.mb = a.mb; e.vb = a.vb; e.sched = a.sched;
    e.sched_slot = a.sched_slot; e.omb1 = (float)(1.0 - a.beta1); e.b2 = (float)a.beta2;
    e.omb2 = (float)(1.0 - a.beta2); e.eps = (float)a.eps; e.wd = (float)a.weight_decay;
    e.clamp = a.clamp; e.enabled = 1;
    return dw_fill(a.dA, a.lda, a.X, a.ldx, a.x_slot, a.dW, a.db, a.M, a.K, a.N, 0, &e, p, xvec);
}

extern "C" int gm_linear_bwd_dw_adam_pair(void* stream, const gm_dw_adam_args* first,
                                          const gm_dw_adam_args* second) {
    GM_CHECK_ARG(first && second);
    GM_CHECK_ARG(first->dW != second->dW && (first->pW != second->pW || !first->pW));
    GM_CHECK_ARG(!first->pW || ((const float*)first->pW != second->dA && (const float*)first->pW != second->X));
    GM_CHECK_ARG(!second->pW || ((const float*)second->pW != first->dA && (const float*)second->pW != first->X));
    GM_CHECK_ARG(first->dW != second->dA && first->dW != second->X && second->dW != first->dA && second->dW != first->X);
    GemmP pa{}, pb{};
    bool xa = false, xb = false;
    int rc = dw_adam_fill(*first, &pa, &xa);
    if (rc) return rc;
    rc = dw_adam_fill(*second, &pb, &xb);
    if (rc) return rc;
    Rider r;
    r.pair = &pb;
    r.pair_xvec = xb;
    return launch<MODE_DW>((hipStream_t)stream, pa, false, xa, r);
}

extern "C" int gm_linear_bwd_dw_adam_pair_finalize(void* stream, const gm_dw_adam_args* first,
                                                   const gm_dw_adam_args* second, const gm_finalize2_args* fin) {
    GM_CHECK_ARG(first && second && fin);
    GM_CHECK_ARG(fin->pa && fin->pb && fin->out_a && fin->out_b && fin->na > 0 && fin->nb > 0 && fin->done);
    GM_CHECK_ARG(first->dW != second->dW && (first->pW != second->pW || !first->pW));
    GM_CHECK_ARG(!first->pW || ((const float*)first->pW != second->dA && (const float*)first->pW != second->X));
    GM_CHECK_ARG(!second->pW || ((const float*)second->pW != first->dA && (const float*)second->pW != first->X));
    GM_CHECK_ARG(first->dW != second->dA && first->dW != second->X && second->dW != first->dA && second->dW != first->X);
    GemmP pa{}, pb{};
    bool xa = false, xb = false;
    int rc = dw_adam_fill(*first, &pa, &xa);
    if (rc) return rc;
    rc = dw_adam_fill(*second, &pb, &xb);
    if (rc) return rc;
    const gm_fin2 f{fin->pa, fin->na, fin->scale_a, fin->out_a, fin->slot_a, fin->pb, fin->nb, fin->scale_b,
                    fin->out_b, fin->slot_b, fin->tick, fin->done};
    Rider r;
    r.pair = &pb;
    r.pair_xvec = xb;
    r.fin = &f;
    return launch<MODE_DW>((hipStream_t)stream, pa, false, xa, r);
}

static int dw_impl(void* stream, const float* dA, int64_t lda, const float* X, int64_t ldx,
                   gm_slot x_slot, float* dW, float* db, int M, int K, int N, int accumulate,
                   const gm_adam_epi* adam, const HeadBwdP* head, int ones_from, const float* fold_w2) {
    GemmP p{};
    bool xvec = false;
    const int rc = dw_fill(dA, lda, X, ldx, x_slot, dW, db, M, K, N, accumulate, adam, &p, &xvec);
    if (rc) return rc;
    GM_CHECK_ARG(ones_from >= 0 && ones_from <= M && (ones_from == 0 || head));
    p.ones_from = ones_from;
    p.fold_w2 = fold_w2;
    if (fold_w2 && !aligned16(fold_w2)) xvec = false;
    Rider r;
    r.head = head;
    return launch<MODE_DW>((hipStream_t)stream, p, false, xvec, r);
}

static int dw_fill(const float* dA, int64_t lda, const float* X, int64_t ldx, gm_slot x_slot,
                   float* dW, float* db, int M, int K, int N, int accumulate,
                   const gm_adam_epi* adam, GemmP* out, bool* xvec_out) {
    GM_CHECK_ARG(dA && X && dW && M > 0 && K > 0 && N > 0 && lda >= N && ldx >= K);
    GemmP p{};
    if (adam) p.adam = *adam;
    p.A = dA; p.B = X; p.C = dW; p.M = N; p.N = K + (db ? 1 : 0); p.K = M;
    p.lda = lda; p.ldb = ldx; p.ldc = K; p.db = db; p.n_real = K; p.accumulate = accumulate;
    p.a_slot = no_slot(); p.b_slot = x_slot;
    const bool xvec = aligned16(dA) && aligned16(X) && (lda % 4 == 0) && (ldx % 4 == 0) &&
                      (N % 4 == 0) && (K % 4 == 0) && (x_slot.stride % 4 == 0) && N >= 4 && K >= 4;
    *out = p;
    *xvec_out = xvec;
    return 0;
}
```

generative_models_amd/engine.py:

```python
import numpy as np
import torch

from . import ops
from ._lib import GMError
from .gan_steps import CriticStep, GeneratorStep, InfoQStep, PenaltySteps

CHUNK = 64
GAN_RING = 128


def _align4(n):
    return (n + 3) // 4 * 4


class FlatParams:

    def __init__(self, params, device, grad_alloc=None):
        self.params, offs, n = [], [], 0
        for item in params:
            group = item if isinstance(item, (tuple, list)) else (item,)
            for p in group:
                self.params.append(p)
                offs.append(n)
                n += p.numel()
# ... 250 lines not shown
                    run += 1
            cls._call(state, 0.0, scale, (run * B * Z) if b == B else b * Z, dst.data_ptr() + k * stride, thr)
            k += run
        np.random.set_state(("MT19937", state[0], state[1], state[2], state[3]))
        return True

    @classmethod
    def _selfcheck(cls):
        try:
            rs = np.random.RandomState(0x5EED)
            rs.normal(size=5)
            rs.random_sample(301)
            state = cls._unpack(rs.get_state(legacy=True))
            if state is None:
                return False
            ok = True
            for n, thr in ((1, 1), (10240 * 3, 2), (7, 1), (4097, 3)):
                ref = torch.from_numpy(rs.normal(0.0, 0.37, n)).float()
                got = torch.empty(n)
                cls._call(state, 0.0, 0.37, n, got.data_ptr(), thr)
                ok = ok and torch.equal(ref.view(torch.int32), got.view(torch.int32))
            end = rs.get_state(legacy=True)
            return bool(ok and np.array_equal(end[1], state[0]) and (int(end[2]), int(end[3]), float(end[4])) ==
                        (state[1], state[2], state[3]))
        except Exception:
            return False


class GANEngine(CriticStep, InfoQStep, GeneratorStep, PenaltySteps):

    SUPPORTED = ("ns", "mm", "w", "ls", "ra", "f", "fisher", "wgp", "info", "be", "dra")

    def __init__(self, variant, model, data, B, device, method=None, use_graph=True,
                 world_size=1, rank=0, process_group=None, force_dp=False):
        assert variant in self.SUPPORTED, variant
        from . import _respect_cpu_quota
        _respect_cpu_quota(force=False)
        self.variant, self.model, self.device = variant, model, device
        self.method = method
        self.loss_key = ("f_" + method) if variant == "f" else \
            {"wgp": "w", "info": "ns", "dra": "ns"}.get(variant, variant)
        self.out_act = "relu" if variant == "wgp" else "sigmoid"
        self.B = B
        self.world, self.rank, self.pg = world_size, rank, process_group
        assert B % world_size == 0, "global batch must divide across ranks"
        self.Bl = B // world_size
        import os as _os
        if not isinstance(data, ops.PackedData) and _os.environ.get("GM_PACKED", "1") != "0" \
                and ops.PackedData.is_binary(data):
            data = ops.PackedData(data)
        self.data = data
        self.N, self.I = data.shape
        G, D = model.G, model.D
        import os
        self.comm_mode = os.environ.get("GM_DP_COMM", "peer")
        self.force_segments = bool(force_dp)
        self._comms = None
        self.comm_memory, self.comm_fallback = "none", None
        if (world_size > 1 or force_dp) and self.comm_mode == "peer":
            sizes = {"D": sum(_align4(p.numel()) for p in D.parameters()),
                     "G": sum(_align4(p.numel()) for p in G.parameters())}
            if variant == "info":
                sizes["Q"] = sum(_align4(p.numel()) for p in model.Q.parameters())
            self._setup_peer_comm(sizes)
        self._rccl = None
        if (world_size > 1 or force_dp) and self.comm_mode == "rccl" and use_graph and \
                os.environ.get("GM_RCCL_IN_GRAPH", "1") != "0":
            self._setup_rccl_graph_comm()
        alloc = (lambda net: (lambda n: self._comms[net].grad_buffer()[:n])) if self._comms else \
            (lambda net: None)
        self.fG = FlatParams(G.parameters(), device, grad_alloc=alloc("G"))
        self.fD = FlatParams(D.parameters(), device, grad_alloc=alloc("D"))
        g1, g2 = list(G.children())[:2]
        d1, d2 = list(D.children())[:2]
        self.G1, self.G2 = _Linear(self.fG, g1), _Linear(self.fG, g2)
        self.D1, self.D2 = _Linear(self.fD, d1), _Linear(self.fD, d2)
        self.Z = self.G1.W.shape[1]
        self.H = self.G1.W.shape[0]
        self.Hd_dim = self.D1.W.shape[0]
        assert self.D2.W.shape[0] == 1 or variant == "be", "score-based critics (BEGAN: autoencoder)"
        self.use_graph = use_graph
        self.fuse_head = self.fuse_adam = self.fold_tick = self.ride_head_dx = True
        self.group_head = self.ride_gather = self.pair_dw = self.batch_gen_env = True
        self.fold_env = os.environ.get("GM_FOLD_HEAD", "1")
        self.graph_iters = max(1, int(os.environ.get("GM_GRAPH_ITERS", "32")))
        self.gated = True
        self._early_submit = True
        self._gate = None
        self._standalone_G = False
        Bl, I, H, Hd = self.Bl, self.I, self.H, self.Hd_dim
        dev = device
        z = lambda *s: torch.zeros(*s, device=dev)
        self.XX4 = z(4 * Bl, I)
        self.XX = self.XX4[Bl:]
        self.X2, self.Xg2 = self.XX[:2 * Bl], self.XX[2 * Bl:]
        self.HG = z(2 * Bl, H)
        self.Hg, self.Hg2 = self.HG[:Bl], self.HG[Bl:]
        self.Hd = z(2 * Bl, Hd)
        self.S2 = z(2 * Bl)
        self.dS = z(2 * Bl)
        self.DU = z(3 * Bl, Hd)
        self.dHd = self.DU[Bl:]
        self.dXg = z(Bl, I)
        self.dHg = z(Bl, H)
        self.rowloss = z(2 * Bl)
        self.fold = ops.HeadFold(2 * Bl, Hd, dev) if (self.D2.W.shape[0] == 1 and Hd <= 512) else None
        self.aux = z(8)
        self.pre = z(16)
        if variant in ("wgp", "dra"):
            self.Xh, self.Hh, self.Sh = z(Bl, I), z(Bl, Hd), z(Bl)
            self.merge_fwd3 = True
            if self.merge_fwd3:
                self.HH3 = z(3 * Bl, Hd)
                self.Hh, self.Hd = self.HH3[:Bl], self.HH3[Bl:]
                self.Xh = self.XX4[:Bl]
            self.Gr, self.T = z(Bl, I), z(Bl, Hd)
            if variant == "wgp":
                self.U, self.Gam = self.DU[:Bl], self.XX4[:Bl]
                self.gw2_pen = z(Hd)
                self.pen_in_head = os.environ.get("GM_WGP_PEN_IN_HEAD", "1") != "0"
            else:
                self.U, self.Gam = z(Bl, Hd), z(Bl, I)
            self.pen = z(Bl)
        if variant == "dra":
            self.da2, self.dA1, self.stdv = z(Bl), z(Bl, Hd), z(1)
            self.dra_stack = self.merge_fwd3 and os.environ.get("GM_DRA_STACK", "1") != "0"
            if self.dra_stack:
                self.XX5 = z(5 * Bl, I)
                self.Gam, self.Xh = self.XX5[:Bl], self.XX5[Bl:2 * Bl]
                self.XX = self.XX5[2 * Bl:]
                self.XX4 = self.XX5[Bl:]
                self.X2, self.Xg2 = self.XX[:2 * Bl], self.XX[2 * Bl:]
                self.DU4 = z(4 * Bl, Hd)
                self.U, self.dA1, self.dHd = self.DU4[:Bl], self.DU4[Bl:2 * Bl], self.DU4[2 * Bl:]
                self.gw2_pen, self.gb2_pen = z(Hd), z(1)
            from . import ops_fused as _of
            self.std_ws = _of.std_workspace(dev)
        if variant == "info":
            Q = model.Q
            self.fQ = FlatParams(Q.parameters(), device, grad_alloc=alloc("Q"))
            q1, q2 = list(Q.children())[:2]
            self.Q1, self.Q2 = _Linear(self.fQ, q1), _Linear(self.fQ, q2)
            self.mi_m, self.mi_v = torch.zeros_like(self.fG.m), torch.zeros_like(self.fG.v)
            self.G1mi = _Linear(self.fG, g1, m=self.mi_m, v=self.mi_v)
            self.G2mi = _Linear(self.fG, g2, m=self.mi_m, v=self.mi_v)
            self.zd, self.nd, self.nc = model.z_dim, model.disc_dim, model.cont_dim
            nq = self.Q2.W.shape[0]
            self.Hq, self.Qo, self.dQo, self.dHq = z(Bl, self.Q1.W.shape[0]), z(Bl, nq), z(Bl, nq), \
                z(Bl, self.Q1.W.shape[0])
        self.ctr = torch.zeros(1, dtype=torch.int64, device=dev)
        self.graph = None
        self._graph_key = None

    def _single(self):
        return self.world == 1 and not self.force_segments

    def _peer(self):
        return not self._single() and self.comm_mode == "peer"

    def _rccl_in_graph(self):
        return not self._single() and self.comm_mode == "rccl" and self._rccl is not None

    def _one_graph(self):
        return self._single() or self._peer() or self._rccl_in_graph()

    def _tick_in_head(self):
        return self.use_graph and self.fold_tick and self.fuse_head

    def _adam_in_epilogue(self, net):
        if not (self.fuse_adam and self._single()):
            return False
        if net == "D":
            if self.variant == "dra":
                return self._dra_stacked()
            if self.variant in ("ra", "fisher"):
                return self._fold_head()
            return self.fuse_head and (self.variant != "wgp" or self._wgp_stacked())
        return True

    def _fold_ok(self, rows):
        if self.fold_env == "0" or self.fold is None or self.variant == "be":
            return False
        if not (self.fuse_head and self.group_head and self.ride_head_dx):
            return False
        if self.Hd_dim % 4 or self.I % 4 or rows > 2048 or self.Hd_dim > 512:
            return False
        return self.fold_env == "2" or rows < ops.lds_min_m()

    def _fold_head(self):
        import os
        if self.variant in ("ra", "fisher"):
            return self._single() and not self.force_segments and self._fold_ok(2 * self.Bl) and \
                os.environ.get("GM_FOLD_HEAD_TP", "1") != "0"
        return self.variant in ("ns", "mm", "w", "ls", "f", "info") and self._fold_ok(2 * self.Bl)

    def _fold_head_G(self):
        import os
        return self._fold_ok(self.Bl)

    def _wgp_stacked(self):
        import os
        return self.variant == "wgp" and self.fuse_head and self.group_head and \
            os.environ.get("GM_WGP_STACK", "1") != "0"

    def _dra_stacked(self):
        return self.variant == "dra" and getattr(self, "dra_stack", False) and self.fuse_head and \
            self.group_head

    def _slot(self, it, mul, add, ring, stride, post=False):
        if self.use_graph:
            if post and self._tick_in_head():
                add -= mul
            return ops.slot(self.ctr.data_ptr(), mul, add, ring, stride)
        i = it * mul + add
        if ring > 0:
            i %= ring
        return ops.slot(0, 0, i, 0, stride)

    def _segments(self):
        d = self.D_steps
        segs = []
        def seg(parts, ar):
            def run(st, it, parts=parts):
                for f in parts:
                    f(st, it)
            segs.append((run, ar))
        pending = []
        for j in range(d):
            pending.append(lambda st, it, j=j: self._issue_D_pre(st, it, j))
            seg(pending, ("D", j))
            pending = [lambda st, it, j=j: self._issue_D_post(st, it, j)]
        pending.append(lambda st, it: self._issue_G_pre(st, it))
        seg(pending, ("G", 0))
        tail = [lambda st, it: self._issue_G_post(st, it)]
        if self.variant == "info":
            tail.append(lambda st, it: self._issue_Q(st, it))
        if self.variant == "be":
            tail.append(lambda st, it: self._issue_end(st, it))
        elif self.use_graph and not self._tick_in_head():
            tail.append(lambda st, it: ops.tick(self.ctr, 1, stream=st))
        seg(tail, None)
        return segs

    def _issue_iteration(self, st, it):
        for run, ar in self._segments():
            run(st, it)
            if ar is not None:
                self._allreduce(ar, st, it)

    def _allreduce(self, ar, st=None, it=0):
        if self._single():
            return
        net, j = ar
        fp = self.fD if net == "D" else self.fG
        if self._peer():
            if net == "D":
                slot, clamp = self._slot(it, self.D_steps, j, 0, 1), self.clip
                sched, scale = self.schedD, self._lr_scale("D")
            else:
                slot, clamp = self._G_sched_slot(it), 0.0
                sched, scale = self.schedG, self._lr_scale("G")
            self._comms[net].allreduce_adam(fp.grad, fp.flat, fp.m, fp.v, sched, slot, clamp=clamp,
                                            lr_scale=scale, stream=st)
            return
        if self._rccl_in_graph():
            self._rccl.allreduce(fp.grad, stream=st)
            return
        from . import dp
        dp.allreduce_sum_(fp.grad, self.pg)

    def _lr_scale(self, net):
        return None

    def _dp(self):
        return not self._single()

    def _exchange_scalars(self, st, vals, k):
        self._comms["D"].allreduce_scalars(vals, k, stream=st)

    def _issue_D(self, st, it, j):
        self._issue_D_pre(st, it, j)
        self._allreduce(("D", j), st, it)
        self._issue_D_post(st, it, j)

    def _issue_G(self, st, it):
        self._issue_G_pre(st, it)
        self._allreduce(("G", 0), st, it)
        self._issue_G_post(st, it)

    AHEAD = 3
    RAMP = (1, 1, 2, 4, 8, 16)
    FIRST_PIECE = 2
    GATE_TIMEOUT_S = 20.0

    def _ring_and_graph_size(self, D_steps):
        import os
        B, Z, d = self.B, self.Z, D_steps
        per_it = d * B * (8 + 4 * Z) + B * 4 * Z
        if self.variant == "wgp":
            per_it += d * B * 4
        if self.variant == "info":
            per_it += B * 4 * Z
        if self.variant == "dra":
            per_it += d * B * 4 * (1 + self.I)
        env_ring, env_gi = os.environ.get("GM_RING"), os.environ.get("GM_GRAPH_ITERS")
        if env_ring:
            ring = int(env_ring)
        else:
            ring = 512 if per_it <= (64 << 10) else 256 if per_it <= (128 << 10) else GAN_RING
        R = max(1, min(ring, 64) if self.variant == "dra" else ring)
        gi = max(1, int(env_gi)) if env_gi else max(32, min(128, R // 4))
        return R, gi

    def _alloc_rings(self, R):
        d, B, Z, dev = self.D_steps, self.B, self.Z, self.device
        self.R = R
        self.SUB = max(1, min(32, self.graph_iters, R))
        self.z_joint = self._batch_gen()
        layout = {"idx": ((R * d,), d, (), torch.int64)}
        if self.z_joint:
            layout["z"] = ((R, 2), 2, (Z,), torch.float32)
        else:
            layout["zD"] = ((R * d,), d, (Z,), torch.float32)
            layout["zG"] = ((R,), 1, (Z,), torch.float32)
        if self.variant == "wgp":
            layout["eps"] = ((R * d,), d, (), torch.float32)
        if self.variant == "info":
            layout["zQ"] = ((R,), 1, (Z,), torch.float32)
        if self.variant == "dra":
            layout["delta"] = ((R * d,), d, (), torch.float32)
            layout["U"] = ((R * d,), d, (self.I,), torch.float32)
# ... 279 lines not shown
                                       wait_bound_s=max(c.selfcheck_bound_s for c in comms.values()),
                                       passed={k: bool(v) for k, v in zip(comms, checks)})
            if not ok:
                why = "self-check failed for %s" % [k for k, c in zip(comms, checks) if not c]
        except Exception as e:
            ok, why = False, "%s: %s" % (type(e).__name__, e)
        if self.world > 1:
            import torch.distributed as dist
            flag = torch.tensor([1 if ok else 0], dtype=torch.int32)
            if dist.get_backend(self.pg) == "nccl":
                flag = flag.to(self.device)
            dist.all_reduce(flag, op=dist.ReduceOp.MIN, group=self.pg)
            if ok and not bool(flag.item()):
                why = "another rank could not use the peer exchange"
            ok = bool(flag.item())
        self.comm_memory = "fine-grained" if comms and all(c.fine_grained for c in comms.values()) else \
            ("coarse-grained (one shared device)" if comms else "none")
        if ok:
            self._comms = comms
        else:
            import warnings
            for c in comms.values():
                try:
                    c.close()
                except Exception:
                    pass
            self.comm_mode = "rccl"
            self.comm_fallback = why or "unknown"
            warnings.warn("generative_models_amd: in-graph peer gradient exchange unavailable (%s); "
                          "falling back to host-launched RCCL all-reduces" % self.comm_fallback)

    def _setup_rccl_graph_comm(self):
        from . import dp
        ok, why = True, None
        try:
            self._rccl = dp.RcclGraphComm(self.world, self.rank, self.pg)
        except Exception as e:
            ok, why, self._rccl = False, "%s: %s" % (type(e).__name__, e), None
        if self.world > 1:
            import torch.distributed as dist
            flag = torch.tensor([1 if ok else 0], dtype=torch.int32)
            if dist.get_backend(self.pg) == "nccl":
                flag = flag.to(self.device)
            dist.all_reduce(flag, op=dist.ReduceOp.MIN, group=self.pg)
            if not bool(flag.item()) and self._rccl is not None:
                self._rccl.close()
                self._rccl = None
        if self._rccl is None and why:
            import warnings
            warnings.warn("generative_models_amd: RCCL all-reduce inside the graph unavailable (%s); host-launched "
                          "collectives between segment graphs" % why)

    def exchange_form(self):
        if not self._dp():
            return "none"
        if not self._peer():
            return "rccl_in_graph" if self._rccl_in_graph() else "rccl"
        comms = getattr(self, "_comms", None) or {}
        if any(c.two_kernels for c in comms.values()):
            return "two_kernels"
        return "one_kernel_push" if any(getattr(c, "push", False) for c in comms.values()) else "one_kernel"

    def optim_state(self):
        torch.cuda.synchronize()
        cpu = lambda t: t.detach().cpu().clone()
        st = {net: {"m": cpu(fp.m), "v": cpu(fp.v), "step": self.step0[net] + self.steps_planned[net]}
              for net, fp in (("G", self.fG), ("D", self.fD))}
        st["config"] = dict(self.run_config)
        if self.variant == "info":
            st["MI"] = {"m_G": cpu(self.mi_m), "v_G": cpu(self.mi_v), "m_Q": cpu(self.fQ.m),
                        "v_Q": cpu(self.fQ.v), "step": self.step0["MI"] + self.n_planned}
        if self.variant == "fisher":
            st["fisher_aux"] = cpu(self.aux)
        return st

    def _ensure_graph(self):
        if not self.use_graph or self._graph_key == self._key:
            return
        torch.cuda.synchronize()
        if self._one_graph():
            def body(k):
                def fn(st):
                    self._issue_stage_in(st, 0, k)
                    for _ in range(k):
                        self._issue_iteration(st, 0)
                return fn
            self.graph = ops.Graph().capture(body(1))
            self.graphs_by_size = [(1, self.graph)]
            k = 2
            while k <= self._graph_max:
                self.graphs_by_size.insert(0, (k, ops.Graph().capture(body(k))))
                k *= 2
            if self.graphs_by_size[0][0] != self._graph_max and self._graph_max > 1:
                self.graphs_by_size.insert(0, (self._graph_max, ops.Graph().capture(body(self._graph_max))))
            self.seg_graphs = None
        else:
            segs = self._segments()
            first = segs[0][0]
            segs[0] = (lambda st, it: (self._issue_stage_in(st, it, 1), first(st, it)), segs[0][1])
            self.seg_graphs = [(ops.Graph().capture(lambda st, run=run: run(st, 0)), ar)
                               for run, ar in segs]
        self._graph_key = self._key

    def _drain(self):
        pend = getattr(self, "_fills", None)
        failed = False
        while pend:
            _, _, fut = pend.popleft()
            try:
                fut.result()
            except Exception:
                failed = True
        if getattr(self, "_rng_owned", False):
            self._release_rng()
        if failed and getattr(self, "_native_fill", False):
            from . import _lib
            _lib.load().gm_fill_reset()

    def _pump(self, limit, upto=None):
        unfinished = sum(n for _, n, f in self._fills if not f.done())
        while self._cursor < limit and (upto is None or self._cursor < upto):
            if unfinished >= self.AHEAD * self.SUB:
                break
            it = self._cursor
            want = self._ramp[0] if self._ramp else self.SUB
            n = min(want, self.SUB, self.R - it % self.R, limit - it)
            if not self._slots_free_now(it, n, wait=upto is not None):
                break
            if self._native_fill:
                fut = self._submit_native(it, n)
            else:
                fut = _prefetch_pool().submit(self._fill, it, n)
            if self._ramp:
                self._ramp.pop(0)
            self._fills.append((it, n, fut))
            self._cursor += n
            unfinished += n

    def _slots_free_now(self, c0, n, wait):
        need = c0 + n - self.R
        if need <= 0:
            return True
        for it_end, e in self._launched:
            if it_end >= need:
                if not e.query():
                    if not wait:
                        return False
                    e.synchronize()
                while self._launched and self._launched[0][0] < need:
                    self._event_pool.append(self._launched.popleft()[1])
                return True
        if wait:
            raise GMError("host ring: iteration %d was never launched" % (need - 1))
        return False

    def _submit_native(self, c0, n):
        from . import _lib
        if not self._rng_owned:
            self._rng_state = torch.get_rng_state()
            self._rng_owned = True
        prog = self._host_views(c0 % self.R)["program"]
        job = _lib.load().gm_fill_submit(self._rng_state.data_ptr(), self._rng_state.numel(), prog, len(prog),
                                         n, self._gate.data_ptr(), c0 + n)
        if job <= 0:
            _lib.check(int(job), "gm_fill_submit")
        return _FillJob(job)

    def _release_rng(self):
        if self._rng_owned and not self._fills:
            torch.set_rng_state(self._rng_state)
            self._rng_owned = False

    def _reap(self, block=False, upto=None):
        fl = self._fills
        while fl and (block or fl[0][2].done() or (upto is not None and fl[0][0] < upto)):
            fl.popleft()[2].result()
            block = False

    def _plan(self, it, n, cold):
        cap = 1
        while cap * 2 <= min(self.graph_iters, self.R):
            cap *= 2
        out, done = [], 0
        while n > 0:
            seg = min(n, self.R - it % self.R)
            q, r = divmod(seg, cap)
            pieces = [1 << i for i in range(cap.bit_length()) if (r >> i) & 1] + [cap] * q
            if cold:
                fixed = []
                for s_ in pieces:
                    stack = [s_]
                    while stack:
                        x = stack.pop()
                        bound = self.FIRST_PIECE if done == 0 else 4 * done
                        if x > bound and x > 1:
                            stack += [x // 2, x // 2]
                        else:
                            fixed.append(x)
                            done += x
                pieces = fixed
            out += pieces
            it += seg
            n -= seg
        return out

    def _copy_U(self, upto):
        if self._u_stream is None:
            self._u_stream = torch.cuda.Stream(device=self.device)
        d, R = self.D_steps, self.R
        with torch.cuda.stream(self._u_stream):
            while self._u_copied < upto:
                r = self._u_copied % R
                m = min(upto - self._u_copied, R - r)
                self.dring["U"][r * d:(r + m) * d].copy_(self.hring["U"][r * d:(r + m) * d], non_blocking=True)
                self._u_copied += m
        ev = torch.cuda.Event()
        ev.record(self._u_stream)
        torch.cuda.current_stream(self.device).wait_event(ev)

    def _check_gate(self):
        if self._gate is not None and self._gate_np[1] != 0:
            raise GMError("a stage-in kernel gave up waiting for the host draws of its iterations "
                          "(%g s): results of this run are invalid" % self.GATE_TIMEOUT_S)

    def _launch(self, it, k):
        if self.use_graph and self._one_graph():
            for size, g in self.graphs_by_size:
                while k >= size:
                    g.launch()
                    k -= size
        elif self.use_graph:
            for _ in range(k):
                for g, ar in self.seg_graphs:
                    g.launch()
                    if ar is not None:
                        self._allreduce(ar)
        else:
            st = ops.stream_ptr()
            self._issue_stage_in(st, it, k)
            for i in range(k):
                self._issue_iteration(st, it + i)

    def run(self, n_iters, it_start=0, horizon=None):
        if self._dp() and self.variant in ("ra", "fisher", "dra", "be", "info") and not self._peer():
            raise GMError("%s needs exchanges inside the step (scalar pre-reductions over the global "
                          "batch / a third gradient bucket, SURVEY.md 8e); they run on the in-graph peer "
                          "communicator (GM_DP_COMM=peer), which is not active here" % self.variant)
        if it_start != self._next_it:
            raise GMError("run(): iterations are consumed in order (next is %d, got %d)"
                          % (self._next_it, it_start))
        self._ensure_graph()
        end = it_start + n_iters
        if end > self.n_planned:
            raise GMError("run(): configure() planned %d iterations" % self.n_planned)
        limit = min(self.n_planned, max(end, horizon or 0))
        it = it_start
        cold = not self._fills and self._cursor == it_start
        gated = self.gated
        self._check_gate()
        trace = self._trace
        try:
            if cold:
                self._ramp = list(self.RAMP)
                if gated and self._native_fill and self._early_submit:
                    self._pump(limit, upto=it_start + min(self.FIRST_PIECE, n_iters))
        except BaseException:
            self._drain()
            raise
        if trace is not None:
            import time
            trace.append(("run", it_start, time.perf_counter()))
            tev = [torch.cuda.Event(enable_timing=True)]
            tev[0].record()
        try:
            plan = self._plan(it_start, n_iters, cold)
            if trace is not None:
                trace.append(("plan", len(plan), time.perf_counter()))
            for k in plan:
                self._reap()
                if trace is not None:
                    trace.append(("reaped", it, time.perf_counter()))
                self._pump(limit, upto=it + k)
                if trace is not None:
                    trace.append(("pumped", it, time.perf_counter()))
                while self._cursor < it + k:
                    self._reap(block=True)
                    self._pump(limit, upto=it + k)
                if not gated:
                    self._reap(upto=it + k)
                    self._pump(limit)
                if self._u_copy:
                    self._reap(upto=it + k)
                    self._copy_U(it + k)
                if trace is not None:
                    trace.append(("got", it, time.perf_counter()))
                self._launch(it, k)
                if trace is not None:
                    trace.append(("graph", it, time.perf_counter()))
                ev = self._event_pool.pop() if self._event_pool else torch.cuda.Event()
                ev.record()
                self._launched.append((it + k, ev))
                if gated:
                    self._pump(limit)
                if trace is not None:
                    trace.append(("pump2", it, time.perf_counter()))
                if trace is not None:
                    tev.append(torch.cuda.Event(enable_timing=True))
                    tev[-1].record()
                while len(self._launched) > 4 * self.R:
                    self._event_pool.append(self._launched.popleft()[1])
                if trace is not None:
                    trace.append(("launched", it + k, time.perf_counter()))
                it += k
            self._reap(upto=end)
            self._pump(limit)
            self._reap()
            self._release_rng()
            if trace is not None:
                import os
                if os.environ.get("GM_TRACE_NOSYNC") == "1":
                    trace.append(("gpu_piece_events", tev, time.perf_counter()))
                else:
                    tev[-1].synchronize()
                    trace.append(("gpu_piece_ends_us", [round(tev[0].elapsed_time(e) * 1e3, 1) for e in tev[1:]],
# ... 93 lines not shown
```

generative_models_amd/gan_steps.py:

```python
import torch

from . import ops


class CriticStep:
    def _gather_rides(self):
        return self.ride_gather

    def _packed_operand(self):
        import os
        if os.environ.get("GM_PACKED_OPERAND", "0") != "1":
            return False
        return isinstance(self.data, ops.PackedData) and self._fold_head() and \
            self.variant not in ("ra", "fisher") and self.Bl % 32 == 0 and self.I % 4 == 0

    def _xbits(self):
        if not self._packed_operand():
            return None
        if getattr(self, "Xbits", None) is None:
            self.Xbits = torch.zeros(self.Bl, self.data.wpr, dtype=torch.int32, device=self.device)
        return (self.Xbits, self.data.wpr, self.Bl)

    def _gather_args(self, it, j):
        Bl, d, R = self.Bl, self.D_steps, self.R
        r0 = self.ring_r0
        xb = self._xbits()
        return dict(data=self.data, idx=self.idx_ring.view(-1)[r0:], out=self.X2 if xb is None else xb[0], B=Bl,
                    idx_slot=self._slot(it, d, j, R * d, self.ring_B))

    def _D_gather(self, st, it, j):
        if self._gather_rides():
            return
        ops.gather_rows(stream=st, **self._gather_args(it, j))

    def _batch_gen(self):
        return self.batch_gen_env and self.D_steps == 1 and \
            (self.world == 1 or self._local_rings())

    def _local_rings(self):
        import os
        return self.world > 1 and self.variant != "dra"

    def _D_gen(self, st, it, j):
        Bl, d, R = self.Bl, self.D_steps, self.R
        G1, G2 = self.G1, self.G2
        zD_slot = self._slot(it, d, j, R * d, self.zD_stride)
        zbase = self.zD_base[self.ring_r0 * self.Z:].view(-1, self.Z)
        rows = 2 * Bl if (self._batch_gen() and not self._standalone_G) else Bl
        if self._gather_rides():
            ops.linear_fwd_gather(zbase, G1.W, G1.b, self.HG, "relu", M=rows, x_slot=zD_slot,
                                  stream=st, **self._gather_args(it, j))
        else:
            ops.linear_fwd(zbase, G1.W, G1.b, self.HG, "relu", M=rows, x_slot=zD_slot, stream=st)
        if self._interp_in_gen():
            r0 = self.ring_r0
            ops.linear_fwd_interp(self.HG, G2.W, G2.b, self.XX[Bl:], "sigmoid", self.eps_ring.view(-1)[r0:],
                                  self._slot(it, d, j, R * d, self.ring_B), self.XX[:Bl], self.Xh, Bl, M=rows,
                                  stream=st)
        else:
            ops.linear_fwd(self.HG, G2.W, G2.b, self.XX[Bl:], "sigmoid", M=rows, stream=st)

    def _interp_in_gen(self):
        import os
        return self.variant == "wgp"

    def _D_rest(self, st, it, j):
        if self._fold_head():
            return self._critic_folded(st, it, j)
        if self.fuse_head and self.variant not in ("ra", "fisher"):
            return self._critic_fused_head(st, it, j)
        return self._critic_unfused(st, it, j)

    def _critic_folded(self, st, it, j):
        Bl, d = self.Bl, self.D_steps
        D1, D2 = self.D1, self.D2
        X2, Hd, S2, dS = self.X2, self.Hd, self.S2, self.dS
        loss_slot = self._slot(it, d, j, 0, 1)
        xb = self._xbits()
        ops.linear_fwd_headpart(X2, D1.W, D1.b, Hd, "relu", D2, self.fold, M=2 * Bl, stream=st, xbits=xb)
        adam = self._adam_args("D", self._slot(it, d, j, 0, 1)) if self._adam_in_epilogue("D") else None
        fa = self.fold.args(self.loss_key, self.out_act, self.hyper, S=S2, dS=dS, rowloss=self.rowloss,
                            pen=self.aux if self.variant == "fisher" else None)
        head = dict(H=Hd, lin=D2, loss_out=self.lossD, loss_slot=loss_slot, inv_b=self.inv_b, B=Bl,
                    adam=adam)
        ops.linear_bwd_dw_adam_head_fold(Hd, X2, D1, adam, head, fa, M=2 * Bl, stream=st, xbits=xb)
        if self.variant == "fisher":
            from . import ops_fused as of
            of.fisher_commit(self.aux, stream=st)

    def _critic_forward(self, st, it, j):
        Bl = self.Bl
        D1 = self.D1
        merged = self.variant in ("wgp", "dra") and self.merge_fwd3
        if merged:
            if self.variant == "wgp":
                self._gp_prepare(st, it, j)
            else:
                self._dra_prepare(st, it, j)
            ops.linear_fwd(self.XX4[:3 * Bl], D1.W, D1.b, self.HH3, "relu", M=3 * Bl, stream=st)
        else:
            ops.linear_fwd(self.X2, D1.W, D1.b, self.Hd, "relu", M=2 * Bl, stream=st)
        aux, hyper = (self.aux if self.variant == "fisher" else None), self.hyper
        if self.variant == "wgp":
            self._issue_gp_forward(st, it, j, fwd_done=merged)
            aux, hyper = self.pen, (0.0,) * 7 + (self.gp_lambda,)
        if self.variant == "dra":
            self._issue_dra_forward(st, it, j, fwd_done=merged)
            aux, hyper = self.pen, tuple(self.hyper) + (0.0,) * (7 - len(self.hyper)) + (self.gp_lambda,)
        return aux, hyper

    def _critic_dw1(self, st, it, j):
        Bl, d = self.Bl, self.D_steps
        if self._adam_in_epilogue("D"):
            ops.linear_bwd_dw_adam(self.dHd, self.X2, self.D1, self._adam_args("D", self._slot(it, d, j, 0, 1)),
                                   M=2 * Bl, stream=st)
        else:
            ops.linear_bwd_dw(self.dHd, self.X2, self.D1.gW, self.D1.gb, M=2 * Bl, stream=st)

    def _critic_penalty_backward(self, st):
        if self.variant == "wgp" and not self._wgp_stacked():
            self._issue_gp_backward(st)
        if self.variant == "dra" and not self._dra_stacked():
            self._issue_dra_backward(st)

    def _critic_fused_head(self, st, it, j):
        from . import ops_fused as of
        Bl, d = self.Bl, self.D_steps
        D1, D2 = self.D1, self.D2
        X2, Hd, S2, dS, dHd = self.X2, self.Hd, self.S2, self.dS, self.dHd
        loss_slot = self._slot(it, d, j, 0, 1)
        aux, hyper = self._critic_forward(st, it, j)
        of.head_fwd_loss(self.loss_key, False, Hd, D2.W, D2.b, self.out_act, Bl, hyper,
# ... 86 lines not shown
        fused = self.fuse_adam and self._single()
        if fused:
            adam = self._adam_args("MI", s_slot)
            dw = lambda dA, X, lin, **kw: ops.linear_bwd_dw_adam(dA, X, lin, adam, M=Bl, stream=st, **kw)
            g1, g2 = self.G1mi, self.G2mi
        else:
            dw = lambda dA, X, lin, **kw: ops.linear_bwd_dw(dA, X, lin.gW, lin.gb, M=Bl, stream=st, **kw)
            g1, g2 = G1, G2
        ops.linear_bwd_dx(self.dQo, Q2.W, self.dHq, below=self.Hq, epi="relu", M=Bl, stream=st)
        ops.linear_bwd_dx(self.dHq, Q1.W, self.dXg, below=Xg, epi="sigmoid", M=Bl, stream=st)
        ops.linear_bwd_dx(self.dXg, G2.W, self.dHg, below=Hg, epi="relu", M=Bl, stream=st)
        if self.pair_dw and fused:
            ops.linear_bwd_dw_adam_pair(dict(dA=self.dHq, X=Xg, lin=Q1, adam=adam, M=Bl),
                                        dict(dA=self.dQo, X=self.Hq, lin=Q2, adam=adam, M=Bl), stream=st)
            ops.linear_bwd_dw_adam_pair(dict(dA=self.dXg, X=Hg, lin=g2, adam=adam, M=Bl),
                                        dict(dA=self.dHg, X=zbase, lin=g1, adam=adam, M=Bl, x_slot=z_slot), stream=st)
        else:
            dw(self.dQo, self.Hq, Q2)
            dw(self.dHq, Xg, Q1)
            dw(self.dXg, Hg, g2)
            dw(self.dHg, zbase, g1, x_slot=z_slot)
        if self._peer():
            self._comms["G"].allreduce_adam(self.fG.grad, self.fG.flat, self.mi_m, self.mi_v, self.schedMI,
                                            s_slot, stream=st)
            self._comms["Q"].allreduce_adam(self.fQ.grad, self.fQ.flat, self.fQ.m, self.fQ.v, self.schedMI,
                                            s_slot, stream=st)
        elif not fused:
            ops.adam(self.fG.flat, self.fG.grad, self.mi_m, self.mi_v, self.schedMI, s_slot, stream=st)
            ops.adam(self.fQ.flat, self.fQ.grad, self.fQ.m, self.fQ.v, self.schedMI, s_slot, stream=st)


class GeneratorStep:
    def _G_zslot(self, it):
        zbase = self.zG_base[self.ring_r0 * self.Z:].view(-1, self.Z)
        return zbase, self._slot(it, 1, 0, self.R, self.zG_stride)

    def _G_gen(self, st, it):
        if self._batch_gen() and not self._standalone_G:
            return
        G1, G2 = self.G1, self.G2
        zbase, zG_slot = self._G_zslot(it)
        ops.linear_fwd(zbase, G1.W, G1.b, self.Hg2, "relu", M=self.Bl, x_slot=zG_slot, stream=st)
        ops.linear_fwd(self.Hg2, G2.W, G2.b, self.Xg2, "sigmoid", M=self.Bl, stream=st)

    def _G_critic(self, st, it):
        Bl = self.Bl
        D1, D2 = self.D1, self.D2
        Hd, S2, dS, dHd, Xg = self.Hd, self.S2, self.dS, self.dHd, self.Xg2
        loss_slot = self._slot(it, 1, self.g_off, 0, 1)
        if self._fold_head_G():
            tick = self.ctr if self._tick_in_head() else None
            ops.linear_fwd_headpart(Xg, D1.W, D1.b, Hd, "relu", D2, self.fold, M=Bl, stream=st)
            fa = self.fold.args(self.loss_key, self.out_act, self.hyper, S=S2, dS=dS, rowloss=self.rowloss)
            ops.linear_bwd_dx_head_fold(
                Hd, D1.W, self.dXg, dict(H=Hd, lin=D2, loss_out=self.lossG, loss_slot=loss_slot,
                                         inv_b=self.inv_b, B=Bl, gen_mode=True, tick=tick),
                fa, below=Xg, epi="sigmoid", M=Bl, stream=st)
            return
        ops.linear_fwd(Xg, D1.W, D1.b, Hd, "relu", M=Bl, stream=st)
        if self.fuse_head:
            from . import ops_fused as of
            tick = self.ctr if self._tick_in_head() else None
            of.head_fwd_loss(self.loss_key, True, Hd, D2.W, D2.b, self.out_act, Bl, self.hyper,
                             self.inv_b, None, S2, dS, self.rowloss, dH=dHd, stream=st)
            if self.ride_head_dx:
                ops.linear_bwd_dx_head(
                    dHd, D1.W, self.dXg,
                    dict(H=Hd, dS=dS, lin=D2, rowloss=self.rowloss, loss_out=self.lossG,
                         loss_slot=loss_slot, inv_b=self.inv_b, B=Bl, gen_mode=True, tick=tick),
                    below=Xg, epi="sigmoid", M=Bl, stream=st)
                return
            of.head_bwd(Hd, dS, D2.W, self.rowloss, None, None, None, self.lossG, loss_slot,
                        self.inv_b, True, Bl, tick=tick, stream=st)
        else:
            ops.linear_fwd(Hd, D2.W, D2.b, S2.view(-1, 1), self.out_act, M=Bl, stream=st)
            ops.gan_loss(self.loss_key, True, None, S2, Bl, self.out_act, self.lossG, None, dS,
                         hyper=self.hyper, inv_b=self.inv_b, loss_slot=loss_slot, stream=st)
            ops.linear_bwd_dx(dS.view(-1, 1), D2.W, dHd, below=Hd, epi="relu", M=Bl, stream=st)
        ops.linear_bwd_dx(dHd, D1.W, self.dXg, below=Xg, epi="sigmoid", M=Bl, stream=st)

    def _G_sched_slot(self, it):
        return self._slot(it, 1, self.g_off, 0, 1, post=True)

    def _G_dh(self, st, it):
        ops.linear_bwd_dx(self.dXg, self.G2.W, self.dHg, below=self.Hg2, epi="relu", M=self.Bl,
                          stream=st)

    def _G_dw2(self, st, it):
        if self._adam_in_epilogue("G"):
            ops.linear_bwd_dw_adam(self.dXg, self.Hg2, self.G2,
                                   self._adam_args("G", self._G_sched_slot(it)), M=self.Bl, stream=st)
        else:
            ops.linear_bwd_dw(self.dXg, self.Hg2, self.G2.gW, self.G2.gb, M=self.Bl, stream=st)

    def _G_dw1(self, st, it):
        zbase = self.zG_base[self.ring_r0 * self.Z:].view(-1, self.Z)
        zG_slot = self._slot(it, 1, 0, self.R, self.zG_stride, post=True)
        if self._adam_in_epilogue("G"):
            ops.linear_bwd_dw_adam(self.dHg, zbase, self.G1,
                                   self._adam_args("G", self._G_sched_slot(it)), M=self.Bl,
                                   x_slot=zG_slot, stream=st)
        else:
            ops.linear_bwd_dw(self.dHg, zbase, self.G1.gW, self.G1.gb, M=self.Bl, x_slot=zG_slot,
                              stream=st)

    def _G_dh_dw1(self, st, it):
        self._G_dh(st, it)
        self._G_dw1(st, it)

    def _issue_G_pre(self, st, it):
        self._G_gen(st, it)
        self._G_critic(st, it)
        self._G_dh(st, it)
        if self.pair_dw:
            adam = self._adam_args("G", self._G_sched_slot(it)) if self._adam_in_epilogue("G") else None
            zbase = self.zG_base[self.ring_r0 * self.Z:].view(-1, self.Z)
            zG_slot = self._slot(it, 1, 0, self.R, self.zG_stride, post=True)
            ops.linear_bwd_dw_adam_pair(
                dict(dA=self.dXg, X=self.Hg2, lin=self.G2, adam=adam, M=self.Bl),
                dict(dA=self.dHg, X=zbase, lin=self.G1, adam=adam, M=self.Bl, x_slot=zG_slot),
                stream=st)
            return
        self._G_dw2(st, it)
        self._G_dw1(st, it)

    def _issue_G_post(self, st, it):
        if self._adam_in_epilogue("G") or self._peer():
            return
        ops.adam(self.fG.flat, self.fG.grad, self.fG.m, self.fG.v, self.schedG,
                 self._G_sched_slot(it), stream=st)


class PenaltySteps:
    def _gp_prepare(self, st, it, j):
        from . import ops_fused as ops_gp
        Bl, d, R = self.Bl, self.D_steps, self.R
        if not self._interp_in_gen():
            eps_slot = self._slot(it, d, j, R * d, self.ring_B)
            ops_gp.interp(self.eps_ring.view(-1)[self.ring_r0:], eps_slot, self.X2[:Bl], self.X2[Bl:], self.Xh,
                          stream=st)

    def _issue_gp_forward(self, st, it, j, fwd_done=False):
        from . import ops_fused as ops_gp
        Bl = self.Bl
        D1, D2 = self.D1, self.D2
        if not fwd_done:
            self._gp_prepare(st, it, j)
            ops.linear_fwd(self.Xh, D1.W, D1.b, self.Hh, "relu", M=Bl, stream=st)
        if self._wgp_stacked():
            ops_gp.head_gp(self.Hh, D2.W, D2.b, self.Sh, self.U, stream=st)
        else:
            ops.linear_fwd(self.Hh, D2.W, D2.b, self.Sh.view(-1, 1), "relu", M=Bl, stream=st)
            ops_gp.gp_u(self.Sh, self.Hh, D2.W, self.U, stream=st)
        ops.linear_bwd_dx(self.U, D1.W, self.Gr, M=Bl, stream=st)
        ops_gp.gp_norm(self.Gr, self.Gam, self.pen, self.gp_lambda, self.inv_b, stream=st)
        if self._wgp_stacked():
            ops.linear_fwd(self.Gam, D1.W, None, self.T, "id", M=Bl, stream=st)
            if not self.pen_in_head:
                ops_gp.gp_dw2_store(self.Sh, self.Hh, self.T, self.gw2_pen, stream=st)

    def _dra_prepare(self, st, it, j):
        from . import ops_fused as of
        Bl, d, R = self.Bl, self.D_steps, self.R
        x = self.X2[:Bl]
        if self._dp():
            of.std_sums(x, Bl, self.pre[8:], ws=self.std_ws, stream=st)
            self._exchange_scalars(st, self.pre[8:], 2)
            of.std_from_sums(self.pre[8:], self.B * self.I, self.stdv, stream=st)
        else:
            of.std_all(x, Bl, self.stdv, ws=self.std_ws, stream=st)
        r0 = self.ring_r0
        of.dragan_xhat(x, self.delta_ring.view(-1)[r0:], self._slot(it, d, j, R * d, self.ring_B),
                       self.U_ring.view(-1)[r0 * self.I:], self._slot(it, d, j, R * d, self.ring_B * self.I),
                       self.stdv, self.Xh, Bl, stream=st)

    def _issue_dra_forward(self, st, it, j, fwd_done=False):
        from . import ops_fused as of
        Bl = self.Bl
        D1, D2 = self.D1, self.D2
        if not fwd_done:
            self._dra_prepare(st, it, j)
            ops.linear_fwd(self.Xh, D1.W, D1.b, self.Hh, "relu", M=Bl, stream=st)
        ops.linear_fwd(self.Hh, D2.W, D2.b, self.Sh.view(-1, 1), "sigmoid", M=Bl, stream=st)
        of.gp_u(self.Sh, self.Hh, D2.W, self.U, stream=st)
        ops.linear_bwd_dx(self.U, D1.W, self.Gr, M=Bl, stream=st)
        of.dragan_rows(self.Sh, self.Gr, self.Gam, self.da2, self.pen, self.gp_lambda, self.inv_b,
                       Bl, stream=st)

    def _issue_dra_backward(self, st, stacked=False):
        from . import ops_fused as of
        Bl = self.Bl
        D1, D2 = self.D1, self.D2
        if stacked:
            ops.linear_fwd(self.Gam, D1.W, None, self.T, "id", M=Bl, stream=st)
            of.dragan_head_bwd(self.Hh, self.T, self.da2, D2.W, self.gw2_pen, self.gb2_pen, self.dA1, Bl,
                               store=True, stream=st)
            return
        ops.linear_bwd_dw(self.U, self.Gam, D1.gW, None, M=Bl, accumulate=True, stream=st)
        ops.linear_fwd(self.Gam, D1.W, None, self.T, "id", M=Bl, stream=st)
        of.dragan_head_bwd(self.Hh, self.T, self.da2, D2.W, D2.gW, D2.gb, self.dA1, Bl, stream=st)
        ops.linear_bwd_dw(self.dA1, self.Xh, D1.gW, D1.gb, M=Bl, accumulate=True, stream=st)

    def _issue_gp_backward(self, st):
        from . import ops_fused as ops_gp
# ... 6 lines not shown
```

generative_models_amd/ops.py:

```python
import ctypes

import numpy as np
import torch

from . import _lib
from ._lib import ACT, LOSS, NO_SLOT, Slot, slot


def stream_ptr():
    return torch.cuda.current_stream().cuda_stream


def _chk(t, name):
    if not (t.is_cuda and t.dtype == torch.float32):
        raise _lib.GMError("%s must be a float32 device tensor (got %s on %s)" %
                           (name, t.dtype, t.device))
    return t


def _ld(t):
    if t.dim() == 1:
        return 1
    if t.stride(1) != 1:
        raise _lib.GMError("inner dimension must be contiguous")
# ... 8 lines not shown
              _chk(y, "y").data_ptr(), _ld(y), M, K, N, ACT[act] if not isinstance(act, int) else act)
    return y


def label_src(labels, idx=None, idx_slot=NO_SLOT):
    if not (labels.is_cuda and labels.dtype == torch.int32):
        raise _lib.GMError("labels must be an int32 device tensor (got %s on %s)" % (labels.dtype, labels.device))
    if idx is not None and not (idx.is_cuda and idx.dtype == torch.int64):
        raise _lib.GMError("idx must be an int64 device tensor")
    src = _lib.LabelSrc(labels.data_ptr(), idx.data_ptr() if idx is not None else None, idx_slot)
    src.keep = (labels, idx)
    return src


def _check_labels(lab, M):
    labels, idx = lab.keep
    if idx is None and labels.numel() < M:
        raise _lib.GMError("%d labels for %d rows" % (labels.numel(), M))


def linear_fwd_label(x, W, b, E, lab, y, act, M=None, stream=None):
    N, K = W.shape
    M = x.shape[0] if M is None else M
    if E.dim() != 2 or E.shape[0] != N or not 1 <= E.shape[1] <= 32 or not E.is_contiguous():
        raise _lib.GMError("label weight E must be a contiguous [N=%d, C], 1 <= C <= 32, got %s" % (N, tuple(E.shape)))
    if x.dim() != 2 or x.shape[1] != K or x.shape[0] < M or y.dim() != 2 or y.shape[0] < M or y.shape[1] != N:
        raise _lib.GMError("linear_fwd_label: x %s / y %s do not fit M=%d, K=%d, N=%d"
                           % (tuple(x.shape), tuple(y.shape), M, K, N))
    _check_labels(lab, M)
    _lib.call("gm_linear_fwd_label", stream or stream_ptr(), _chk(x, "x").data_ptr(), _ld(x), _chk(W, "W").data_ptr(),
              b.data_ptr() if b is not None else None, _chk(E, "E").data_ptr(), E.shape[1], lab,
              _chk(y, "y").data_ptr(), _ld(y), M, K, N, ACT[act] if not isinstance(act, int) else act)
    return y


def label_grad_adam(layers, lab, M, C, adam=None, betas=(0.9, 0.999), eps=1e-8, weight_decay=0.0, stream=None):
    arr = (_lib.LabelGradArgs * len(layers))()
    ptr = lambda t: t.data_ptr() if t is not None else None
    _check_labels(lab, M)
    for a, d in zip(arr, layers):
        dp = _chk(d["dPre"], "dPre")
        if dp.dim() != 2 or dp.shape[0] < M:
            raise _lib.GMError("dPre must be [>= M=%d, N], got %s" % (M, tuple(dp.shape)))
        for k in ("gE", "E", "mE", "vE"):
            t = d.get(k)
            if t is not None and (not t.is_cuda or t.dtype != torch.float32 or not t.is_contiguous()
                                  or tuple(t.shape) != (dp.shape[1], C)):
                raise _lib.GMError("%s must be a contiguous float32 device tensor [N=%d, C=%d], got %s"
                                   % (k, dp.shape[1], C, tuple(t.shape)))
        a.dPre, a.ld, a.N = dp.data_ptr(), _ld(dp), dp.shape[1]
        a.gE, a.E, a.mE, a.vE = ptr(d.get("gE")), ptr(d.get("E")), ptr(d.get("mE")), ptr(d.get("vE"))
    _lib.call("gm_label_grad_adam", stream or stream_ptr(), arr, len(layers), lab, M, C,
              adam["sched"].data_ptr() if adam else None, adam["sched_slot"] if adam else NO_SLOT,
              betas[0], betas[1], eps, weight_decay)


def linear_fwd_interp(x, W, b, y, act, eps, eps_slot, x_real, x_hat, rows, M=None, x_slot=NO_SLOT,
                      stream=None):
    N, K = W.shape
    M = x.shape[0] if M is None else M
    _lib.call("gm_linear_fwd_interp", stream or stream_ptr(), _chk(x, "x").data_ptr(), _ld(x), x_slot,
              _chk(W, "W").data_ptr(), b.data_ptr() if b is not None else None,
              _chk(y, "y").data_ptr(), _ld(y), M, K, N, ACT[act] if not isinstance(act, int) else act,
              eps.data_ptr(), eps_slot, _chk(x_real, "x_real").data_ptr(), _ld(x_real),
              _chk(x_hat, "x_hat").data_ptr(), _ld(x_hat), rows)
    return y


def linear_bwd_dx(dA, W, dX, below=None, epi="id", M=None, add=None, add_scale=1.0, stream=None):
    N, K = W.shape
    M = dA.shape[0] if M is None else M
    if add is not None:
        _lib.call("gm_linear_bwd_dx_add", stream or stream_ptr(), _chk(dA, "dA").data_ptr(), _ld(dA),
                  W.data_ptr(), _chk(dX, "dX").data_ptr(), _ld(dX),
                  below.data_ptr() if below is not None else None,
                  _ld(below) if below is not None else 0, M, K, N,
                  ACT[epi] if not isinstance(epi, int) else epi, add.data_ptr(), _ld(add), add_scale)
        return dX
    _lib.call("gm_linear_bwd_dx", stream or stream_ptr(), _chk(dA, "dA").data_ptr(), _ld(dA),
              W.data_ptr(), _chk(dX, "dX").data_ptr(), _ld(dX),
              below.data_ptr() if below is not None else None,
              _ld(below) if below is not None else 0, M, K, N,
              ACT[epi] if not isinstance(epi, int) else epi)
    return dX


def linear_bwd_dw(dA, X, dW, db, M=None, accumulate=False, x_slot=NO_SLOT, stream=None):
    N, K = dW.shape
    M = dA.shape[0] if M is None else M
    _lib.call("gm_linear_bwd_dw", stream or stream_ptr(), _chk(dA, "dA").data_ptr(), _ld(dA),
              _chk(X, "X").data_ptr(), _ld(X), x_slot, dW.data_ptr(),
              db.data_ptr() if db is not None else None, M, K, N, 1 if accumulate else 0)


def linear_bwd_dw_adam(dA, X, lin, adam, M=None, x_slot=NO_SLOT, betas=(0.9, 0.999), eps=1e-8,
                       weight_decay=0.0, stream=None):
    N, K = lin.gW.shape
    M = dA.shape[0] if M is None else M
    _lib.call("gm_linear_bwd_dw_adam", stream or stream_ptr(), _chk(dA, "dA").data_ptr(), _ld(dA),
              _chk(X, "X").data_ptr(), _ld(X), x_slot, lin.gW.data_ptr(), lin.gb.data_ptr(), M, K, N,
              lin.W.data_ptr(), lin.mW.data_ptr(), lin.vW.data_ptr(), lin.b.data_ptr(),
              lin.mb.data_ptr(), lin.vb.data_ptr(), adam["sched"].data_ptr(), adam["sched_slot"],
              betas[0], betas[1], eps, weight_decay, adam.get("clamp", 0.0))


def linear_fwd_gather(x, W, b, y, act, data, idx, out, M=None, B=None, x_slot=NO_SLOT,
                      idx_slot=NO_SLOT, stream=None):
    N, K = W.shape
    M = x.shape[0] if M is None else M
    n_rows, row = data.shape
    B = out.shape[0] if B is None else B
    if isinstance(data, PackedData) and out.dtype == torch.int32:
        assert out.is_contiguous() and out.shape[1] == data.wpr
        _lib.call("gm_linear_fwd_gather_bits_packed", stream or stream_ptr(), _chk(x, "x").data_ptr(), _ld(x),
                  x_slot, _chk(W, "W").data_ptr(), b.data_ptr() if b is not None else None,
                  _chk(y, "y").data_ptr(), _ld(y), M, K, N, ACT[act], data.data_ptr(), data.wpr,
                  n_rows, idx.data_ptr(), idx_slot, out.data_ptr(), B)
        return y
    if isinstance(data, PackedData):
        _lib.call("gm_linear_fwd_gather_bits", stream or stream_ptr(), _chk(x, "x").data_ptr(), _ld(x),
                  x_slot, _chk(W, "W").data_ptr(), b.data_ptr() if b is not None else None,
                  _chk(y, "y").data_ptr(), _ld(y), M, K, N, ACT[act], data.data_ptr(), data.wpr,
                  n_rows, idx.data_ptr(), idx_slot, out.data_ptr(), _ld(out), B, row)
        return y
    _lib.call("gm_linear_fwd_gather", stream or stream_ptr(), _chk(x, "x").data_ptr(), _ld(x),
              x_slot, _chk(W, "W").data_ptr(), b.data_ptr() if b is not None else None,
              _chk(y, "y").data_ptr(), _ld(y), M, K, N, ACT[act], _chk(data, "data").data_ptr(),
              n_rows, idx.data_ptr(), idx_slot, out.data_ptr(), _ld(out), B, row)
    return y


def _dw_adam_args(dA, X, lin, adam, M, x_slot, betas, eps, weight_decay):
    from ._lib import DwAdamArgs
    N, K = lin.gW.shape
    a = DwAdamArgs()
    a.dA, a.lda, a.X, a.ldx, a.x_slot = _chk(dA, "dA").data_ptr(), _ld(dA), _chk(X, "X").data_ptr(), _ld(X), x_slot
    a.dW, a.db, a.M, a.K, a.N = lin.gW.data_ptr(), lin.gb.data_ptr(), (dA.shape[0] if M is None else M), K, N
    if adam is not None:
        a.pW, a.mW, a.vW = lin.W.data_ptr(), lin.mW.data_ptr(), lin.vW.data_ptr()
        a.pb, a.mb, a.vb = lin.b.data_ptr(), lin.mb.data_ptr(), lin.vb.data_ptr()
        a.sched, a.sched_slot = adam["sched"].data_ptr(), adam["sched_slot"]
        a.clamp = adam.get("clamp", 0.0)
    a.beta1, a.beta2, a.eps, a.weight_decay = betas[0], betas[1], eps, weight_decay
    return a


def linear_bwd_dw_adam_pair(first, second, betas=(0.9, 0.999), eps=1e-8, weight_decay=0.0,
                            stream=None):
    import ctypes
    mk = lambda d: _dw_adam_args(d["dA"], d["X"], d["lin"], d.get("adam"), d.get("M"),
                                 d.get("x_slot", NO_SLOT), betas, eps, weight_decay)
    a, b = mk(first), mk(second)
    _lib.call("gm_linear_bwd_dw_adam_pair", stream or stream_ptr(), ctypes.byref(a), ctypes.byref(b))


def linear_bwd_dw_adam_pair_finalize(first, second, fin, betas=(0.9, 0.999), eps=1e-8, weight_decay=0.0,
                                     stream=None):
    import ctypes
    from ._lib import Finalize2Args
    mk = lambda d: _dw_adam_args(d["dA"], d["X"], d["lin"], d.get("adam"), d.get("M"),
                                 d.get("x_slot", NO_SLOT), betas, eps, weight_decay)
    a, b = mk(first), mk(second)
    f = Finalize2Args()
    f.pa, f.na, f.scale_a, f.out_a, f.slot_a = fin["pa"].data_ptr(), fin["na"], fin.get("scale_a", 1.0), \
        fin["out_a"].data_ptr(), fin["slot_a"]
    f.pb, f.nb, f.scale_b, f.out_b, f.slot_b = fin["pb"].data_ptr(), fin["nb"], fin.get("scale_b", 1.0), \
        fin["out_b"].data_ptr(), fin["slot_b"]
    tick = fin.get("tick")
    f.tick = tick.data_ptr() if tick is not None else None
    assert fin["done"].dtype == torch.int32 and fin["done"].numel() >= 1
    f.done = fin["done"].data_ptr()
    _lib.call("gm_linear_bwd_dw_adam_pair_finalize", stream or stream_ptr(), ctypes.byref(a), ctypes.byref(b),
              ctypes.byref(f))


def _head_args(head, betas=(0.9, 0.999), eps=1e-8):
    from ._lib import HeadBwdArgs
    hl, ha, H = head["lin"], head.get("adam"), head["H"]
    gen = bool(head.get("gen_mode", False))
    a = HeadBwdArgs()
    ptr = lambda t: t.data_ptr() if t is not None else None
    a.H, a.ldh, a.dS = H.data_ptr(), _ld(H), ptr(head.get("dS"))
    a.w2, a.b2, a.rowloss = hl.W.data_ptr(), hl.b.data_ptr(), ptr(head.get("rowloss"))
    a.dH, a.lddh = None, 0
    if not gen:
        a.gw2, a.gb2 = hl.gW.data_ptr(), hl.gb.data_ptr()
    a.loss_out, a.loss_slot = head["loss_out"].data_ptr(), head["loss_slot"]
    a.inv_b, a.gen_mode, a.B, a.Hd = head["inv_b"], 1 if gen else 0, head["B"], H.shape[1]
    a.with_adam = 1 if ha is not None else 0
    if ha is not None:
        a.mW, a.vW, a.mb, a.vb = hl.mW.data_ptr(), hl.vW.data_ptr(), hl.mb.data_ptr(), hl.vb.data_ptr()
        a.sched, a.sched_slot = ha["sched"].data_ptr(), ha["sched_slot"]
        a.clamp = ha.get("clamp", 0.0)
    a.beta1, a.beta2, a.eps, a.weight_decay = betas[0], betas[1], eps, 0.0
    tick = head.get("tick")
    a.tick = tick.data_ptr() if tick is not None else None
    add = head.get("gw2_add")
    a.gw2_add = add.data_ptr() if add is not None else None
    addb = head.get("gb2_add")
    a.gb2_add = addb.data_ptr() if addb is not None else None
    pen = head.get("pen")
    if pen is not None:
        a.pen_s, a.pen_h, a.pen_ldh = pen["s"].data_ptr(), pen["h"].data_ptr(), _ld(pen["h"])
        a.pen_t, a.pen_ldt, a.pen_rows = pen["t"].data_ptr(), _ld(pen["t"]), pen["t"].shape[0]
    return a


def linear_fwd_sqerr(x, W, b, y, target, dA, part, M=None, stream=None):
    N, K = W.shape
    M = x.shape[0] if M is None else M
    assert part.dim() == 2 and part.shape[0] >= M and part.shape[1] >= (N + 31) // 32
    _lib.call("gm_linear_fwd_sqerr", stream or stream_ptr(), _chk(x, "x").data_ptr(), _ld(x),
              _chk(W, "W").data_ptr(), b.data_ptr() if b is not None else None, _chk(y, "y").data_ptr(), _ld(y),
              M, K, N, _chk(target, "target").data_ptr(), _ld(target), _chk(dA, "dA").data_ptr(), _ld(dA),
              part.data_ptr(), part.shape[1])
    return y


def linear_bwd_dx_reparam(dA, W, dZ, ml, eps, dml, M=None, eps_slot=NO_SLOT, stream=None):
    N, Z = W.shape
    M = dA.shape[0] if M is None else M
    _lib.call("gm_linear_bwd_dx_reparam", stream or stream_ptr(), _chk(dA, "dA").data_ptr(), _ld(dA),
              _chk(W, "W").data_ptr(), _chk(dZ, "dZ").data_ptr(), _ld(dZ), M, Z, N, ml.data_ptr(), _ld(ml),
              eps.data_ptr(), eps_slot, dml.data_ptr(), _ld(dml))
    return dZ


def lds_min_m():
    import os
    return 1024


class HeadFold:

    def __init__(self, rows, hidden, device):
        self.nparts = (hidden + 31) // 32
# ... 391 lines not shown
```

include/gm_hip.h:

```cpp
#ifndef GM_HIP_H
#define GM_HIP_H

#include <stddef.h>
#include <stdint.h>

#ifdef __cplusplus
extern "C" {
#endif

#define GM_EINVAL (-10001)

enum { GM_ACT_ID = 0, GM_ACT_RELU = 1, GM_ACT_SIGMOID = 2 };

enum {
    GM_LOSS_NS = 0,
    GM_LOSS_MM = 1,
    GM_LOSS_W = 2,
    GM_LOSS_LS = 3,
    GM_LOSS_RA = 4,
    GM_LOSS_FISHER = 5,
    GM_LOSS_F_TV = 6, GM_LOSS_F_FKL = 7, GM_LOSS_F_RKL = 8, GM_LOSS_F_PEARSON = 9,
    GM_LOSS_F_HELLINGER = 10, GM_LOSS_F_JS = 11
};

// ... 137 lines not shown
} gm_head_bwd_args;
int gm_linear_bwd_dw_adam_head(void* stream, const float* dA, int64_t lda, const float* X,
                               int64_t ldx, gm_slot x_slot, float* dW, float* db, int M, int K, int N,
                               float* pW, float* mW, float* vW, float* pb, float* mb, float* vb,
                               const float* sched, gm_slot sched_slot, double beta1, double beta2,
                               double eps, double weight_decay, float clamp,
                               const gm_head_bwd_args* head);
int gm_linear_bwd_dw_adam_head_ex(void* stream, const float* dA, int64_t lda, const float* X,
                                  int64_t ldx, gm_slot x_slot, float* dW, float* db, int M, int K, int N,
                                  float* pW, float* mW, float* vW, float* pb, float* mb, float* vb,
                                  const float* sched, gm_slot sched_slot, double beta1, double beta2,
                                  double eps, double weight_decay, float clamp,
                                  const gm_head_bwd_args* head, int ones_from);
int gm_linear_bwd_dx_head(void* stream, const float* dA, int64_t lda, const float* W, float* dX,
                          int64_t ldx, const float* below, int64_t ld_below, int M, int K, int N,
                          int epi, const gm_head_bwd_args* head);
typedef struct gm_head_fold_args {
    const float* part; int64_t ldp; int nparts;
    const float* snap;
    int variant, out_act;
    float hyper[8]; int n_hyper;
    const float* pen;
    float* S; float* dS; float* rowloss;
} gm_head_fold_args;
int gm_linear_fwd_headpart(void* stream, const float* X, int64_t ldx, gm_slot x_slot, const float* W,
                           const float* bias, float* Y, int64_t ldy, int M, int K, int N, int act,
                           const float* w2, const float* b2, float* part, int64_t ldp, float* snap);
int gm_linear_bwd_dw_adam_head_fold(void* stream, const float* H, int64_t ldh, const float* X,
                                    int64_t ldx, gm_slot x_slot, float* dW, float* db, int M, int K, int N,
                                    float* pW, float* mW, float* vW, float* pb, float* mb, float* vb,
                                    const float* sched, gm_slot sched_slot, double beta1, double beta2,
                                    double eps, double weight_decay, float clamp,
                                    const gm_head_bwd_args* head, const gm_head_fold_args* fold);
int gm_linear_bwd_dx_head_fold(void* stream, const float* H, int64_t ldh, const float* W, float* dX,
                               int64_t ldx, const float* below, int64_t ld_below, int M, int K, int N,
                               int epi, const gm_head_bwd_args* head, const gm_head_fold_args* fold);
int gm_linear_fwd_sqerr(void* stream, const float* X, int64_t ldx, const float* W, const float* bias,
                        float* Y, int64_t ldy, int M, int K, int N, const float* target,
                        int64_t ld_target, float* dA, int64_t lda, float* part, int64_t ldp);
int gm_linear_bwd_dx_reparam(void* stream, const float* dA, int64_t lda, const float* W, float* dZ,
                             int64_t ldz, int M, int Z, int N, const float* ml, int64_t ldml,
                             const float* eps, gm_slot eps_slot, float* dml, int64_t ldd);
int gm_linear_fwd_interp(void* stream, const float* X, int64_t ldx, gm_slot x_slot, const float* W,
                         const float* bias, float* Y, int64_t ldy, int M, int K, int N, int act,
                         const float* eps, gm_slot eps_slot, const float* x_real, int64_t ld_real,
                         float* x_hat, int64_t ld_hat, int rows);
int gm_linear_fwd_gather(void* stream, const float* X, int64_t ldx, gm_slot x_slot, const float* W,
                         const float* bias, float* Y, int64_t ldy, int M, int K, int N, int act,
                         const float* data, int64_t n_rows, const int64_t* idx, gm_slot idx_slot,
                         float* out, int64_t ld_out, int B, int row_elems);
int gm_linear_fwd_gather_bits(void* stream, const float* X, int64_t ldx, gm_slot x_slot, const float* W,
                              const float* bias, float* Y, int64_t ldy, int M, int K, int N, int act,
                              const uint32_t* bits, int words_per_row, int64_t n_rows, const int64_t* idx,
                              gm_slot idx_slot, float* out, int64_t ld_out, int B, int row_elems);
int gm_gather_rows_bits(void* stream, const uint32_t* bits, int words_per_row, int64_t n_rows,
                        const int64_t* idx, gm_slot idx_slot, float* out, int64_t ld_out, int B,
                        int row_elems);
int gm_gather_rows_bits_packed(void* stream, const uint32_t* bits, int words_per_row, int64_t n_rows,
                               const int64_t* idx, gm_slot idx_slot, uint32_t* out_bits, int B);
int gm_linear_fwd_gather_bits_packed(void* stream, const float* X, int64_t ldx, gm_slot x_slot, const float* W,
                                     const float* bias, float* Y, int64_t ldy, int M, int K, int N, int act,
                                     const uint32_t* bits, int words_per_row, int64_t n_rows, const int64_t* idx,
                                     gm_slot idx_slot, uint32_t* out_bits, int B);
int gm_linear_fwd_headpart_bits(void* stream, const float* X, int64_t ldx, gm_slot x_slot, const float* W,
                                const float* bias, float* Y, int64_t ldy, int M, int K, int N, int act,
                                const float* w2, const float* b2, float* part, int64_t ldp, float* snap,
                                const uint32_t* xbits, int words_per_row, int rows);
int gm_linear_bwd_dw_adam_head_fold_bits(void* stream, const float* H, int64_t ldh, const float* X,
                                         int64_t ldx, gm_slot x_slot, float* dW, float* db, int M, int K, int N,
                                         float* pW, float* mW, float* vW, float* pb, float* mb, float* vb,
                                         const float* sched, gm_slot sched_slot, double beta1, double beta2,
                                         double eps, double weight_decay, float clamp,
                                         const gm_head_bwd_args* head, const gm_head_fold_args* fold,
                                         const uint32_t* xbits, int words_per_row, int rows);
typedef struct gm_dw_adam_args {
    const float* dA; int64_t lda; const float* X; int64_t ldx; gm_slot x_slot;
    float* dW; float* db; int M, K, N;
    float* pW; float* mW; float* vW; float* pb; float* mb; float* vb;
    const float* sched; gm_slot sched_slot;
    double beta1, beta2, eps, weight_decay; float clamp;
} gm_dw_adam_args;
int gm_linear_bwd_dw_adam_pair(void* stream, const gm_dw_adam_args* first,
                               const gm_dw_adam_args* second);
typedef struct gm_finalize2_args {
    const float* pa; int na; float scale_a; float* out_a; gm_slot slot_a;
    const float* pb; int nb; float scale_b; float* out_b; gm_slot slot_b;
    int64_t* tick; unsigned int* done;
} gm_finalize2_args;
int gm_linear_bwd_dw_adam_pair_finalize(void* stream, const gm_dw_adam_args* first, const gm_dw_adam_args* second,
                                        const gm_finalize2_args* fin);
int gm_linear_bwd_dx_add(void* stream, const float* dA, int64_t lda, const float* W, float* dX,
                         int64_t ldx, const float* below, int64_t ld_below, int M, int K, int N,
                         int epi, const float* add, int64_t ldadd, float add_scale);

#define GM_STD_WS_BYTES 1088
int gm_std_all(void* stream, const float* X, int64_t ldx, int R, int I, float* out, void* ws);
int gm_std_sums(void* stream, const float* X, int64_t ldx, int R, int I, float* out2, void* ws);
int gm_std_from_sums(void* stream, const float* sums2, int64_t n_total, float* out);
int gm_dragan_xhat(void* stream, const float* x, int64_t ldx, const float* delta, gm_slot delta_slot,
                   const float* U, gm_slot u_slot, const float* std_dev, float C, float* out,
                   int64_t ldo, int B, int I);
int gm_dragan_rows(void* stream, const float* s, const float* V, int64_t ldv, float* dv, int64_t lddv,
                   float* da2, float* pen, float lambda, float inv_b, float K_norm, int B, int I);
int gm_dragan_head_bwd(void* stream, const float* H, int64_t ldh, const float* T, int64_t ldt,
                       const float* da2, const float* w2, float* gw2, float* gb2, float* dA1,
                       int64_t ldd, int B, int Hd);
int gm_fisher_commit(void* stream, float* aux);
int gm_dragan_head_bwd_store(void* stream, const float* H, int64_t ldh, const float* T, int64_t ldt,
                             const float* da2, const float* w2, float* gw2, float* gb2, float* dA1,
                             int64_t ldd, int B, int Hd);

int gm_info_q_loss(void* stream, const float* q, int64_t ldq, const float* noise, gm_slot noise_slot,
                   int64_t ldn, int B, int z_dim, int disc_dim, int cont_dim, float lambda, float* dq,
                   int64_t lddq, float* loss_out, gm_slot loss_slot);
int gm_info_q_loss_dp(void* stream, const float* q, int64_t ldq, const float* noise, gm_slot noise_slot,
                      int64_t ldn, int B, int B_global, int z_dim, int disc_dim, int cont_dim, float lambda,
                      float* dq, int64_t lddq, float* loss_out, gm_slot loss_slot);

int gm_act_bwd(void* stream, const float* dY, const float* Y, float* dA, int64_t n, int act);

#define GM_STAGE_MAX_SEGS 8
typedef struct gm_stage_seg {
    const void* src;
    void* dst;
    int64_t bytes_per_iter;
    int32_t blocks;
    int32_t reserved;
    int64_t src_block_stride, dst_block_stride;
} gm_stage_seg;
int gm_stage_in(void* stream, const gm_stage_seg* segs, int n_segs, gm_slot slot, int n_iters);
int gm_stage_in_gated(void* stream, const gm_stage_seg* segs, int n_segs, gm_slot slot, int n_iters,
                      const int64_t* gate, gm_slot it_slot, double timeout_s, int64_t* publish,
                      int max_blocks);
int gm_host_device_ptr(void* host_ptr, void** dev_ptr_out);

int gm_comm_create(int rank, int world, int64_t n_floats, void** comm_out, void* handle_out64);
int gm_comm_connect(void* comm, const void* all_handles );
int gm_comm_destroy(void* comm);
int gm_comm_error(void* comm, int* flag_out);
int gm_comm_info(void* comm, int* fine_grained_out);
int gm_comm_set_exchange(void* comm, int form);
int gm_comm_set_max_blocks(void* comm, int max_blocks);
int gm_comm_set_wait_seconds(void* comm, double seconds);
int gm_comm_buffer(void* comm, void** ptr_out, int64_t* n_floats_out);
int gm_allreduce_f32(void* comm, void* stream, float* buf, int64_t n);
int gm_allreduce_adam_f32(void* comm, void* stream, float* grad, int64_t n, float* p, float* m,
                          float* v, const float* sched, gm_slot sched_slot, double beta1,
                          double beta2, double eps, double weight_decay, float clamp,
                          const float* lr_scale_or_null);
int gm_allreduce_scalars(void* comm, void* stream, float* vals, int k);
int gm_rccl_available(void);
int gm_rccl_unique_id(void* uid128_out);
int gm_rccl_comm_create(int rank, int world, const void* uid128, void** rccl_comm_out);
int gm_rccl_allreduce_f32(void* rccl_comm, void* stream, float* buf, int64_t n);
int gm_rccl_comm_destroy(void* rccl_comm);

int gm_randperm_prefix(uint64_t seed, int64_t n, int B, int64_t* out_host);
int gm_mt19937_skip(void* torch_cpu_rng_state, int64_t state_bytes, uint64_t n);

typedef struct gm_draw_op {
    int32_t kind;
    int32_t n;
    int64_t a;
    int32_t b, c;
    void* dst;
    int64_t iter_stride;
    int64_t e0, e1;
} gm_draw_op;
enum { GM_DRAW_SAMPLER = 0, GM_DRAW_NORMAL = 1, GM_DRAW_UNIFORM = 2, GM_DRAW_INFO = 3 };
int gm_host_replay(void* torch_cpu_rng_state, int64_t state_bytes, const gm_draw_op* ops, int n_ops,
                   int n_iters);
int gm_host_replay_flavour(int flavour);
int64_t gm_fill_submit(void* torch_cpu_rng_state, int64_t state_bytes, const gm_draw_op* ops, int n_ops,
                       int n_iters, int64_t* gate, int64_t gate_value);
int gm_fill_wait(int64_t id);
int64_t gm_fill_completed(void);
// ... 81 lines not shown
```

Before: 3.963 million images/sec.

## Fuse next iteration's G layer-1 forward into G Adam pair and gather into dX

The generator's layer-1 weight-gradient plus Adam kernel now keeps the freshly updated W1/b1 tile in shared memory and immediately computes the next iteration's first-layer forward (relu(z·W1ᵀ+b)) for the discriminator step, writing into a ping-pong hidden buffer. The next iteration then skips its own layer-1 forward launch. Separately, the next batch's real-data row gather now rides on extra blocks of the G dX backward kernel. Both remove kernel launches and a weight re-read across step boundaries, at the cost of cross-iteration state (ping-pong buffers, next-slot RNG offsets) and a more complex schedule.

```diff
diff --git a/generative_models_amd/_lib.py b/generative_models_amd/_lib.py
--- a/generative_models_amd/_lib.py
+++ b/generative_models_amd/_lib.py
@@ -180,6 +180,12 @@
                                                      ctypes.c_double, ctypes.c_double, ctypes.c_double, c_float,
                                                      POINTER(HeadBwdArgs), POINTER(HeadFoldArgs), _P, c_int, c_int]),
     "gm_linear_bwd_dw_adam_pair": (c_int, [_P, POINTER(DwAdamArgs), POINTER(DwAdamArgs)]),
+    "gm_linear_bwd_dw_adam_pair_l1": (c_int, [_P, POINTER(DwAdamArgs), POINTER(DwAdamArgs), _P, c_int64, Slot, _P,
+                                              c_int64, c_int]),
+    "gm_linear_bwd_dx_gather": (c_int, [_P, _P, c_int64, _P, _P, c_int64, _P, c_int64, c_int, c_int, c_int, c_int,
+                                        _P, c_int64, _P, Slot, _P, c_int64, c_int, c_int]),
+    "gm_linear_bwd_dx_gather_bits": (c_int, [_P, _P, c_int64, _P, _P, c_int64, _P, c_int64, c_int, c_int, c_int,
+                                             c_int, _P, c_int, c_int64, _P, Slot, _P, c_int64, c_int, c_int]),
     "gm_linear_bwd_dw_adam_pair_finalize": (c_int, [_P, POINTER(DwAdamArgs), POINTER(DwAdamArgs),
                                                     POINTER(Finalize2Args)]),
     "gm_linear_bwd_dw_adam_head": (c_int, [_P, _P, c_int64, _P, c_int64, Slot, _P, _P, c_int, c_int,
diff --git a/generative_models_amd/csrc/gm_gemm.hip b/generative_models_amd/csrc/gm_gemm.hip
--- a/generative_models_amd/csrc/gm_gemm.hip
+++ b/generative_models_amd/csrc/gm_gemm.hip
@@ -150,7 +150,7 @@
 }
 
 template <int MODE, bool LBL = false>
-__device__ __forceinline__ void store_element(const GemmP& p, float v, int m, int n) {
+__device__ __forceinline__ void store_element(const GemmP& p, float v, int m, int n, float* kept = nullptr) {
     if (MODE == MODE_FWD) {
         if constexpr (LBL) v += p.lb_E[(int64_t)n * p.lb_C + gm_row_label(p.lb, m, p.lb_C)];
         v = fwd_value(p, v, n);
@@ -192,6 +192,7 @@
             adam_update(P, v, M, V, step_size, bc2_sqrt, p.adam.omb1, p.adam.b2, p.adam.omb2,
                         p.adam.eps, p.adam.wd, p.adam.clamp);
             *pp = P; *mm = M; *vv = V;
+            if (kept) *kept = P;
         }
     }
 }
@@ -260,9 +261,11 @@
     return (w * 32 + row) * 32 + (col ^ ((((row >> 2) ^ row) & 1) << 4));
 }
 
+constexpr int KEEP_LD = 68;
 template <int MODE, int WAVES, int ROWS = 32, bool LBL = false>
 __device__ __forceinline__ void reduce_and_store(const GemmP& p, const float* red, int t, int m0,
-                                                 int n0, int ncap = 0x7fffffff, int rcap = 32) {
+                                                 int n0, int ncap = 0x7fffffff, int rcap = 32,
+                                                 float* kept = nullptr) {
     if (MODE == MODE_FWD && p.hd_part) {
 #pragma unroll
         for (int e = 0; e < 1024 / (WAVES * 64); ++e) {
@@ -328,7 +331,7 @@
         for (int ww = 0; ww < WAVES; ++ww) v += red[red_idx(ww, row, col)];
         const int m = m0 + row, n = n0 + col;
         if (m >= p.M || n >= p.N || n >= ncap) continue;
-        store_element<MODE, LBL>(p, v, m, n);
+        store_element<MODE, LBL>(p, v, m, n, kept ? kept + row * KEEP_LD + col : nullptr);
     }
 }
 
@@ -863,7 +866,8 @@
 template <int MODE, bool VEC, int WAVES, int G, bool XV, int MI, int NI, bool OF = false, int FOLD = 0, bool DMA = false,
           bool TP = false, bool PK = false, bool SL = true, bool LBL = false>
 __device__ __forceinline__ void gemm16_body(const GemmP& p, float* red, int bx, int by,
-                                            float* sds = nullptr, const FoldP* fold = nullptr, int gx = 0) {
+                                            float* sds = nullptr, const FoldP* fold = nullptr, int gx = 0,
+                                            float* kept = nullptr) {
     static_assert(!TP || (FOLD == 1 && !DMA), "two-phase losses: folded weight gradient, operands through registers");
     static_assert(FOLD == 0 || (FOLD == 1 && MODE == MODE_DW && XV) || (FOLD == 2 && MODE == MODE_DX && VEC),
                   "folded head: 16-byte operand paths only");
@@ -1130,7 +1134,8 @@
             if (bm + bn == 0) GM_STAMP(st_slot, st_tile, 10);
             reduce_and_store<MODE, WAVES, (MI > 1 ? 32 : 16), LBL>(p, red, t, m0 + 32 * bm, n0 + 32 * bn,
                                                               (2 * bn + 1 < NI) ? 0x7fffffff : n0 + 32 * bn + 16,
-                                                              (2 * bm + 1 < MI) ? 32 : 16);
+                                                              (2 * bm + 1 < MI) ? 32 : 16,
+                                                              kept ? kept + 32 * bm * KEEP_LD + 32 * bn : nullptr);
         }
     GM_STAMP(st_slot, st_tile, 12);
     GM_STAMP_EDGE(p, true, st_tile, MODE);
@@ -1203,6 +1208,33 @@
         return;
     }
     gemm16_body<MODE_FWD, VEC, 16, G, false, MI, NI>(p, red, blockIdx.x, blockIdx.y - grows);
+}
+
+template <bool VEC, bool XV, int MI, int NI>
+__global__ __launch_bounds__(1024) void gemm16_dx_gather_kernel(GemmP p, GatherP gp, int grows, int gblocks) {
+    __shared__ __attribute__((aligned(16))) float red[16 * 32 * 32];
+    if ((int)blockIdx.y < grows) {
+        const int bid = blockIdx.y * gridDim.x + blockIdx.x;
+        if (bid < gblocks) gather_body(gp, bid);
+        return;
+    }
+    gemm16_body<MODE_DX, VEC, 16, 1, XV, MI, NI, false, 0, false, false, false, false>(p, red, blockIdx.x, blockIdx.y - grows);
+}
+
+__device__ __forceinline__ f32x4 k32_chunk(float4 fa, float4 fb) {
+    f32x4 c4 = f32x4{0.f, 0.f, 0.f, 0.f};
+    c4 = __builtin_amdgcn_mfma_f32_16x16x4f32(fa.x, fb.x, c4, 0, 0, 0);
+    c4 = __builtin_amdgcn_mfma_f32_16x16x4f32(fa.y, fb.y, c4, 0, 0, 0);
+    c4 = __builtin_amdgcn_mfma_f32_16x16x4f32(fa.z, fb.z, c4, 0, 0, 0);
+    c4 = __builtin_amdgcn_mfma_f32_16x16x4f32(fa.w, fb.w, c4, 0, 0, 0);
+    return c4;
+}
+__device__ __forceinline__ float k32_sum(float part0, float part1, bool has_bias, float bv) {
+    float x = 0.f;
+    x += part0;
+    x += part1;
+    if (has_bias) x += bv;
+    return x;
 }
 
 template <bool SL, bool GATHER>
@@ -1242,12 +1274,7 @@
 #pragma unroll
         for (int ni = 0; ni < 2; ++ni) {
             const float4 fb = fix_kc(rb[c][ni], n0 + 16 * ni + i16, p.N, kb, p.K);
-            f32x4 c4 = f32x4{0.f, 0.f, 0.f, 0.f};
-            c4 = __builtin_amdgcn_mfma_f32_16x16x4f32(fa.x, fb.x, c4, 0, 0, 0);
-            c4 = __builtin_amdgcn_mfma_f32_16x16x4f32(fa.y, fb.y, c4, 0, 0, 0);
-            c4 = __builtin_amdgcn_mfma_f32_16x16x4f32(fa.z, fb.z, c4, 0, 0, 0);
-            c4 = __builtin_amdgcn_mfma_f32_16x16x4f32(fa.w, fb.w, c4, 0, 0, 0);
-            part[c][ni] = c4;
+            part[c][ni] = k32_chunk(fa, fb);
             if (c == 0 && ni == 0) { GM_STAMP_AFTER(fa.x); GM_STAMP_AFTER(fb.x); GM_STAMP(st_slot, st_tile, 1); }
         }
     }
@@ -1259,13 +1286,7 @@
         const int n = min(n0 + 16 * ni + i16, p.N - 1);
         const float bv = p.bias ? p.bias[n] : 0.f;
 #pragma unroll
-        for (int r = 0; r < 4; ++r) {
-            float x = 0.f;
-            x += part[0][ni][r];
-            x += part[1][ni][r];
-            if (p.bias) x += bv;
-            v[ni][r] = x;
-        }
+        for (int r = 0; r < 4; ++r) v[ni][r] = k32_sum(part[0][ni][r], part[1][ni][r], p.bias != nullptr, bv);
     }
     if (p.epi == GM_ACT_RELU) {
 #pragma unroll
@@ -1332,6 +1353,68 @@
     }
 }
 
+struct L1RideP {
+    const float* z; int64_t ldz; gm_slot z_slot;
+    float* H; int64_t ldh;
+    int rows;
+    int vec;
+};
+
+__device__ __forceinline__ void l1_ride_fwd(const L1RideP& r, const float* kept, int h0, int N, int K) {
+    const int t = threadIdx.x, lane = t & 63, w = __builtin_amdgcn_readfirstlane(t >> 6);
+    const int i16 = lane & 15, g4 = lane >> 4;
+    const float* Z = r.z + gm_slot_offset(r.z_slot);
+    float4 fw[2];
+#pragma unroll
+    for (int c = 0; c < 2; ++c) {
+        const int kb = 16 * c + 4 * g4;
+        fw[c] = fix_kc(*reinterpret_cast<const float4*>(kept + i16 * KEEP_LD + kb), h0 + i16, N, kb, K);
+    }
+    float bv[4];
+#pragma unroll
+    for (int q = 0; q < 4; ++q) bv[q] = kept[(4 * g4 + q) * KEEP_LD + K];
+    const int h = h0 + 4 * g4;
+    const int nblk = (r.rows + 15) >> 4;
+    for (int b = w; b < nblk; b += 16) {
+        const int m = 16 * b + i16;
+        float4 rz[2];
+#pragma unroll
+        for (int c = 0; c < 2; ++c) rz[c] = raw_kc<true>(Z, r.ldz, m, r.rows, 16 * c + 4 * g4, K);
+        f32x4 part[2];
+#pragma unroll
+        for (int c = 0; c < 2; ++c) part[c] = k32_chunk(fw[c], fix_kc(rz[c], m, r.rows, 16 * c + 4 * g4, K));
+        float v[4];
+#pragma unroll
+        for (int q = 0; q < 4; ++q) v[q] = fmaxf(k32_sum(part[0][q], part[1][q], true, bv[q]), 0.f);
+        if (m < r.rows) {
+            float* hp = r.H + (int64_t)m * r.ldh + h;
+            if (r.vec && h + 3 < N) st4(hp, make_float4(v[0], v[1], v[2], v[3]));
+            else {
+#pragma unroll
+                for (int q = 0; q < 4; ++q)
+                    if (h + q < N) hp[q] = v[q];
+            }
+        }
+    }
+}
+
+template <int MI, int NI>
+__global__ __launch_bounds__(1024) void gemm16_dw_pair_l1_kernel(GemmP pa, GemmP pb, int na, int tna, L1RideP r) {
+    __shared__ __attribute__((aligned(16))) float red[RedSize<MODE_DW, false, MI, NI>::value];
+    __shared__ __attribute__((aligned(16))) float kept[16 * KEEP_LD];
+    static_assert(NI <= 4 && 16 * NI <= KEEP_LD, "one 16-row tile of [W1 | b1] in `kept`");
+    const int id = blockIdx.x;
+    if (id < na) {
+        gemm16_body<MODE_DW, false, 16, 1, true, MI, NI, false, 0, false, false, false, false>(pa, red, id % tna, id / tna);
+        return;
+    }
+    const int by = id - na;
+    gemm16_body<MODE_DW, false, 16, 1, true, 1, NI, false, 0, false, false, false, true>(pb, red, 0, by, nullptr, nullptr, 0,
+                                                                                        kept);
+    __syncthreads();
+    l1_ride_fwd(r, kept, 16 * by, pb.M, pb.n_real);
+}
+
 template <int MODE>
 int vec_epi_ok(const GemmP& p) {
     if (!aligned16(p.C) || p.ldc % 4 != 0) return 0;
@@ -1353,6 +1436,7 @@
     const GemmP* pair = nullptr;
     bool pair_xvec = false;
     const gm_fin2* fin = nullptr;
+    const L1RideP* l1 = nullptr;
 };
 
 enum { T22 = 0, T24, T42, T12, T23, T32 };
@@ -1527,6 +1611,20 @@
     }
     if (head)
         hipLaunchKernelGGL(head_bwd_kernel, dim3(gm_head_bwd_blocks(*head)), dim3(1024), 0, s, *head);
+    if constexpr (MODE == MODE_DX) {
+        if (rider.gather) {
+            const GatherP& gp = *rider.gather;
+            if (vec && xv && (tile == T22 || tile == T12)) {
+                const int gblocks = gm_gather_blocks(gp, 16);
+                const int grows = (gblocks + (int)grid.x - 1) / (int)grid.x;
+                const dim3 ggrid(grid.x, grid.y + grows);
+                if (tile == T12) hipLaunchKernelGGL((gemm16_dx_gather_kernel<true, true, 1, 2>), ggrid, dim3(1024), 0, s, p, gp, grows, gblocks);
+                else hipLaunchKernelGGL((gemm16_dx_gather_kernel<true, true, 2, 2>), ggrid, dim3(1024), 0, s, p, gp, grows, gblocks);
+                GM_LAUNCH_RET();
+            }
+            hipLaunchKernelGGL(gather_rows_kernel, dim3(gm_gather_blocks(gp, 4)), dim3(256), 0, s, gp);
+        }
+    }
     if constexpr (MODE == MODE_FWD) {
         if (rider.gather) {
             const GatherP& gp = *rider.gather;
@@ -1545,10 +1643,36 @@
         if (rider.pair) {
             GemmP pb = *rider.pair;
             pb.vec_epi = vec_epi_ok<MODE_DW>(pb);
-            if (xv && rider.pair_xvec && tile != T12 && pb.K == p.K) {
+            const bool pairable = xv && rider.pair_xvec && tile != T12 && pb.K == p.K;
+            const bool l1_rides = rider.l1 && pairable && !(p.dma && dma_ok(pb, true)) && !slots && !rider.fin &&
+                                  pb.adam.enabled && pb.db && pb.n_real + 1 <= 16 * ni && pb.n_real <= 32 &&
+                                  pb.n_real % 4 == 0 && aligned16(rider.l1->z) && rider.l1->ldz % 4 == 0 &&
+                                  rider.l1->z_slot.stride % 4 == 0;
+            if (rider.l1 && !l1_rides) {
+                Rider r2 = rider;
+                r2.l1 = nullptr;
+                const int rc = launch<MODE_DW>(s, p_in, vec, xvec, r2);
+                if (rc) return rc;
+                const L1RideP& l = *rider.l1;
+                GemmP f{};
+                f.A = l.z; f.B = pb.adam.pW; f.C = l.H; f.M = l.rows; f.N = pb.M; f.K = pb.n_real;
+                f.lda = l.ldz; f.ldb = pb.ldc; f.ldc = l.ldh; f.bias = pb.adam.pb; f.epi = GM_ACT_RELU;
+                f.a_slot = l.z_slot; f.b_slot = gm_slot{};
+                const bool fvec = aligned16(l.z) && aligned16(pb.adam.pW) && (l.ldz % 4 == 0) && (f.K % 4 == 0) &&
+                                  (pb.ldc % 4 == 0) && (l.z_slot.stride % 4 == 0);
+                return launch<MODE_FWD>(s, f, fvec);
+            }
+            if (pairable) {
                 const bool dma = p.dma && dma_ok(pb, true);
                 p.dma = pb.dma = dma;
                 const int tna = (int)grid.x, na = (int)(grid.x * grid.y);
+                if (l1_rides) {
+                    const dim3 lgrid(na + (pb.M + 15) / 16);
+#define GM_LL1(MI_, NI_, D_) hipLaunchKernelGGL((gemm16_dw_pair_l1_kernel<MI_, NI_>), lgrid, dim3(1024), 0, s, p, pb, na, tna, *rider.l1)
+                    GM_TILE_SWITCH(tile, false, GM_LL1);
+#undef GM_LL1
+                    GM_LAUNCH_RET();
+                }
                 const int tnb = (pb.N + 16 * ni - 1) / (16 * ni), tmb = (pb.M + 16 * mi - 1) / (16 * mi);
                 const dim3 pgrid(na + tnb * tmb);
                 const bool sl_b = has_slot(pb.a_slot) || has_slot(pb.b_slot);
@@ -1773,7 +1897,7 @@
 static int dx_impl(void* stream, const float* dA, int64_t lda, const float* W, float* dX, int64_t ldx,
                    const float* below, int64_t ld_below, int M, int K, int N, int epi,
                    const float* add, int64_t ldadd, float add_scale, const HeadBwdP* head = nullptr,
-                   const float* fold_w2 = nullptr);
+                   const float* fold_w2 = nullptr, const GatherP* gather = nullptr);
 
 extern "C" int gm_linear_bwd_dx_head(void* stream, const float* dA, int64_t lda, const float* W,
                                      float* dX, int64_t ldx, const float* below, int64_t ld_below,
@@ -1831,10 +1955,34 @@
     return dx_impl(stream, dA, lda, W, dX, ldx, below, ld_below, M, K, N, epi, add, ldadd, add_scale);
 }
 
+extern "C" int gm_linear_bwd_dx_gather(void* stream, const float* dA, int64_t lda, const float* W,
+                                       float* dX, int64_t ldx, const float* below, int64_t ld_below,
+                                       int M, int K, int N, int epi, const float* data, int64_t n_rows,
+                                       const int64_t* idx, gm_slot idx_slot, float* out, int64_t ld_out,
+                                       int B, int row_elems) {
+    GM_CHECK_ARG(out && out != dA && out != W && out != dX && out != below);
+    GatherP g{};
+    const int rc = gm_gather_fill(data, n_rows, idx, idx_slot, out, ld_out, B, row_elems, &g);
+    if (rc) return rc;
+    return dx_impl(stream, dA, lda, W, dX, ldx, below, ld_below, M, K, N, epi, nullptr, 0, 0.f, nullptr, nullptr, &g);
+}
+
+extern "C" int gm_linear_bwd_dx_gather_bits(void* stream, const float* dA, int64_t lda, const float* W,
+                                            float* dX, int64_t ldx, const float* below, int64_t ld_below,
+                                            int M, int K, int N, int epi, const uint32_t* bits, int words_per_row,
+                                            int64_t n_rows, const int64_t* idx, gm_slot idx_slot, float* out,
+                                            int64_t ld_out, int B, int row_elems) {
+    GM_CHECK_ARG(out && out != dA && out != W && out != dX && out != below);
+    GatherP g{};
+    const int rc = gm_gather_fill_bits(bits, words_per_row, n_rows, idx, idx_slot, out, ld_out, B, row_elems, &g);
+    if (rc) return rc;
+    return dx_impl(stream, dA, lda, W, dX, ldx, below, ld_below, M, K, N, epi, nullptr, 0, 0.f, nullptr, nullptr, &g);
+}
+
 static int dx_impl(void* stream, const float* dA, int64_t lda, const float* W, float* dX, int64_t ldx,
                    const float* below, int64_t ld_below, int M, int K, int N, int epi,
                    const float* add, int64_t ldadd, float add_scale, const HeadBwdP* head,
-                   const float* fold_w2) {
+                   const float* fold_w2, const GatherP* gather) {
     GM_CHECK_ARG(dA && W && dX && M > 0 && K > 0 && N > 0 && lda >= N && ldx >= K);
     GM_CHECK_ARG(epi == GM_ACT_ID || (below && ld_below >= K));
     GemmP p{};
@@ -1847,6 +1995,7 @@
     const bool xvec = aligned16(W) && (K % 4 == 0);
     Rider r;
     r.head = head;
+    r.gather = gather;
     return launch<MODE_DX>((hipStream_t)stream, p, vec, xvec, r);
 }
 
@@ -1988,8 +2137,28 @@
     return dw_fill(a.dA, a.lda, a.X, a.ldx, a.x_slot, a.dW, a.db, a.M, a.K, a.N, 0, &e, p, xvec);
 }
 
+static int pair_launch(void* stream, const gm_dw_adam_args* first, const gm_dw_adam_args* second,
+                       const L1RideP* l1);
+
 extern "C" int gm_linear_bwd_dw_adam_pair(void* stream, const gm_dw_adam_args* first,
                                           const gm_dw_adam_args* second) {
+    return pair_launch(stream, first, second, nullptr);
+}
+
+extern "C" int gm_linear_bwd_dw_adam_pair_l1(void* stream, const gm_dw_adam_args* first,
+                                             const gm_dw_adam_args* second, const float* z, int64_t ldz,
+                                             gm_slot z_slot, float* H, int64_t ldh, int rows) {
+    GM_CHECK_ARG(first && second && second->sched && z && H && rows > 0 && ldz >= second->K && ldh >= second->N);
+    const void* pair_arrays[] = {first->dA, first->X, first->dW, first->db, first->pW, first->pb,
+                                 second->dA, second->X, second->dW, second->db, second->pW, second->pb};
+    for (const void* q : pair_arrays) GM_CHECK_ARG(q != (const void*)H);
+    GM_CHECK_ARG((const void*)z != (const void*)H);
+    const L1RideP l{z, ldz, z_slot, H, ldh, rows, (aligned16(H) && ldh % 4 == 0) ? 1 : 0};
+    return pair_launch(stream, first, second, &l);
+}
+
+static int pair_launch(void* stream, const gm_dw_adam_args* first, const gm_dw_adam_args* second,
+                       const L1RideP* l1) {
     GM_CHECK_ARG(first && second);
     GM_CHECK_ARG(first->dW != second->dW && (first->pW != second->pW || !first->pW));
     GM_CHECK_ARG(!first->pW || ((const float*)first->pW != second->dA && (const float*)first->pW != second->X));
@@ -2004,6 +2173,7 @@
     Rider r;
     r.pair = &pb;
     r.pair_xvec = xb;
+    r.l1 = l1;
     return launch<MODE_DW>((hipStream_t)stream, pa, false, xa, r);
 }
 
diff --git a/generative_models_amd/engine.py b/generative_models_amd/engine.py
--- a/generative_models_amd/engine.py
+++ b/generative_models_amd/engine.py
@@ -356,6 +356,8 @@
         self.use_graph = use_graph
         self.fuse_head = self.fuse_adam = self.fold_tick = self.ride_head_dx = True
         self.group_head = self.ride_gather = self.pair_dw = self.batch_gen_env = True
+        self.ride_l1 = True
+        self._l1_in = self._l1_out = False
         self.fold_env = os.environ.get("GM_FOLD_HEAD", "1")
         self.graph_iters = max(1, int(os.environ.get("GM_GRAPH_ITERS", "32")))
         self.gated = True
@@ -370,6 +372,7 @@
         self.X2, self.Xg2 = self.XX[:2 * Bl], self.XX[2 * Bl:]
         self.HG = z(2 * Bl, H)
         self.Hg, self.Hg2 = self.HG[:Bl], self.HG[Bl:]
+        self._HG_pp = [self.HG, z(2 * Bl, H) if variant in ("ns", "ls") else None]
         self.Hd = z(2 * Bl, Hd)
         self.S2 = z(2 * Bl)
         self.dS = z(2 * Bl)
@@ -516,11 +519,29 @@
         seg(tail, None)
         return segs
 
-    def _issue_iteration(self, st, it):
-        for run, ar in self._segments():
-            run(st, it)
-            if ar is not None:
-                self._allreduce(ar, st, it)
+    def _l1_rides(self):
+        return self.ride_l1 and self.variant in ("ns", "ls") and self._single() and self.D_steps == 1 and \
+            self._batch_gen() and not self._standalone_G and self.pair_dw and self._adam_in_epilogue("G") and \
+            self._gather_rides() and self._fold_head() and self._fold_head_G() and not self._packed_operand() and \
+            2 * self.Bl <= 512 and self._HG_pp[1] is not None
+
+    def _use_hg(self, b):
+        self.HG = self._HG_pp[b]
+        self.Hg, self.Hg2 = self.HG[:self.Bl], self.HG[self.Bl:]
+
+    def _issue_iteration(self, st, it, pos=0, count=1):
+        rides = self._l1_rides()
+        self._l1_in, self._l1_out = rides and pos > 0, rides and pos + 1 < count
+        if rides:
+            self._use_hg(pos & 1)
+            self._l1_next = (pos + 1) & 1
+        try:
+            for run, ar in self._segments():
+                run(st, it)
+                if ar is not None:
+                    self._allreduce(ar, st, it)
+        finally:
+            self._l1_in = self._l1_out = False
 
     def _allreduce(self, ar, st=None, it=0):
         if self._single():
@@ -966,8 +987,8 @@
             def body(k):
                 def fn(st):
                     self._issue_stage_in(st, 0, k)
-                    for _ in range(k):
-                        self._issue_iteration(st, 0)
+                    for i in range(k):
+                        self._issue_iteration(st, 0, i, k)
                 return fn
             self.graph = ops.Graph().capture(body(1))
             self.graphs_by_size = [(1, self.graph)]
@@ -1123,7 +1144,7 @@
             st = ops.stream_ptr()
             self._issue_stage_in(st, it, k)
             for i in range(k):
-                self._issue_iteration(st, it + i)
+                self._issue_iteration(st, it + i, i, k)
 
     def run(self, n_iters, it_start=0, horizon=None):
         if self._dp() and self.variant in ("ra", "fisher", "dra", "be", "info") and not self._peer():
diff --git a/generative_models_amd/gan_steps.py b/generative_models_amd/gan_steps.py
--- a/generative_models_amd/gan_steps.py
+++ b/generative_models_amd/gan_steps.py
@@ -47,7 +47,9 @@
         zD_slot = self._slot(it, d, j, R * d, self.zD_stride)
         zbase = self.zD_base[self.ring_r0 * self.Z:].view(-1, self.Z)
         rows = 2 * Bl if (self._batch_gen() and not self._standalone_G) else Bl
-        if self._gather_rides():
+        if self._l1_in:
+            pass
+        elif self._gather_rides():
             ops.linear_fwd_gather(zbase, G1.W, G1.b, self.HG, "relu", M=rows, x_slot=zD_slot,
                                   stream=st, **self._gather_args(it, j))
         else:
@@ -300,7 +302,16 @@
     def _G_sched_slot(self, it):
         return self._slot(it, 1, self.g_off, 0, 1, post=True)
 
+    def _next_slot(self, it, stride):
+        return self._slot(it, 1, 1, self.R, stride, post=True)
+
     def _G_dh(self, st, it):
+        if self._l1_out:
+            g = self._gather_args(it, 0)
+            g["idx_slot"] = self._next_slot(it, self.ring_B)
+            ops.linear_bwd_dx_gather(self.dXg, self.G2.W, self.dHg, g["data"], g["idx"], g["out"], below=self.Hg2,
+                                     epi="relu", M=self.Bl, B=g["B"], idx_slot=g["idx_slot"], stream=st)
+            return
         ops.linear_bwd_dx(self.dXg, self.G2.W, self.dHg, below=self.Hg2, epi="relu", M=self.Bl,
                           stream=st)
 
@@ -334,10 +345,14 @@
             adam = self._adam_args("G", self._G_sched_slot(it)) if self._adam_in_epilogue("G") else None
             zbase = self.zG_base[self.ring_r0 * self.Z:].view(-1, self.Z)
             zG_slot = self._slot(it, 1, 0, self.R, self.zG_stride, post=True)
-            ops.linear_bwd_dw_adam_pair(
-                dict(dA=self.dXg, X=self.Hg2, lin=self.G2, adam=adam, M=self.Bl),
-                dict(dA=self.dHg, X=zbase, lin=self.G1, adam=adam, M=self.Bl, x_slot=zG_slot),
-                stream=st)
+            first = dict(dA=self.dXg, X=self.Hg2, lin=self.G2, adam=adam, M=self.Bl)
+            second = dict(dA=self.dHg, X=zbase, lin=self.G1, adam=adam, M=self.Bl, x_slot=zG_slot)
+            if self._l1_out:
+                zD = self.zD_base[self.ring_r0 * self.Z:].view(-1, self.Z)
+                ops.linear_bwd_dw_adam_pair_l1(first, second, zD, self._HG_pp[self._l1_next], 2 * self.Bl,
+                                               z_slot=self._next_slot(it, self.zD_stride), stream=st)
+                return
+            ops.linear_bwd_dw_adam_pair(first, second, stream=st)
             return
         self._G_dw2(st, it)
         self._G_dw1(st, it)
diff --git a/generative_models_amd/ops.py b/generative_models_amd/ops.py
--- a/generative_models_amd/ops.py
+++ b/generative_models_amd/ops.py
@@ -114,6 +114,27 @@
               below.data_ptr() if below is not None else None,
               _ld(below) if below is not None else 0, M, K, N,
               ACT[epi] if not isinstance(epi, int) else epi)
+    return dX
+
+
+def linear_bwd_dx_gather(dA, W, dX, data, idx, out, below=None, epi="id", M=None, B=None, idx_slot=NO_SLOT,
+                         stream=None):
+    N, K = W.shape
+    M = dA.shape[0] if M is None else M
+    n_rows, row = data.shape
+    B = out.shape[0] if B is None else B
+    if isinstance(data, PackedData):
+        _lib.call("gm_linear_bwd_dx_gather_bits", stream or stream_ptr(), _chk(dA, "dA").data_ptr(), _ld(dA),
+                  W.data_ptr(), _chk(dX, "dX").data_ptr(), _ld(dX),
+                  below.data_ptr() if below is not None else None, _ld(below) if below is not None else 0, M, K,
+                  N, ACT[epi] if not isinstance(epi, int) else epi, data.data_ptr(), data.wpr, n_rows,
+                  idx.data_ptr(), idx_slot, out.data_ptr(), _ld(out), B, row)
+        return dX
+    _lib.call("gm_linear_bwd_dx_gather", stream or stream_ptr(), _chk(dA, "dA").data_ptr(), _ld(dA),
+              W.data_ptr(), _chk(dX, "dX").data_ptr(), _ld(dX),
+              below.data_ptr() if below is not None else None, _ld(below) if below is not None else 0, M, K, N,
+              ACT[epi] if not isinstance(epi, int) else epi, _chk(data, "data").data_ptr(), n_rows,
+              idx.data_ptr(), idx_slot, out.data_ptr(), _ld(out), B, row)
     return dX
 
 
@@ -184,6 +205,19 @@
                                  d.get("x_slot", NO_SLOT), betas, eps, weight_decay)
     a, b = mk(first), mk(second)
     _lib.call("gm_linear_bwd_dw_adam_pair", stream or stream_ptr(), ctypes.byref(a), ctypes.byref(b))
+
+
+def linear_bwd_dw_adam_pair_l1(first, second, z, H, rows, z_slot=NO_SLOT, betas=(0.9, 0.999), eps=1e-8,
+                               weight_decay=0.0, stream=None):
+    import ctypes
+    mk = lambda d: _dw_adam_args(d["dA"], d["X"], d["lin"], d.get("adam"), d.get("M"),
+                                 d.get("x_slot", NO_SLOT), betas, eps, weight_decay)
+    if second.get("adam") is None:
+        raise _lib.GMError("linear_bwd_dw_adam_pair_l1: the second GEMM needs its Adam step")
+    a, b = mk(first), mk(second)
+    _lib.call("gm_linear_bwd_dw_adam_pair_l1", stream or stream_ptr(), ctypes.byref(a), ctypes.byref(b),
+              _chk(z, "z").data_ptr(), _ld(z), z_slot, _chk(H, "H").data_ptr(), _ld(H), rows)
+    return H
 
 
 def linear_bwd_dw_adam_pair_finalize(first, second, fin, betas=(0.9, 0.999), eps=1e-8, weight_decay=0.0,
diff --git a/include/gm_hip.h b/include/gm_hip.h
--- a/include/gm_hip.h
+++ b/include/gm_hip.h
@@ -243,6 +243,8 @@
 } gm_dw_adam_args;
 int gm_linear_bwd_dw_adam_pair(void* stream, const gm_dw_adam_args* first,
                                const gm_dw_adam_args* second);
+int gm_linear_bwd_dw_adam_pair_l1(void* stream, const gm_dw_adam_args* first, const gm_dw_adam_args* second,
+                                  const float* z, int64_t ldz, gm_slot z_slot, float* H, int64_t ldh, int rows);
 typedef struct gm_finalize2_args {
     const float* pa; int na; float scale_a; float* out_a; gm_slot slot_a;
     const float* pb; int nb; float scale_b; float* out_b; gm_slot slot_b;
@@ -253,6 +255,14 @@
 int gm_linear_bwd_dx_add(void* stream, const float* dA, int64_t lda, const float* W, float* dX,
                          int64_t ldx, const float* below, int64_t ld_below, int M, int K, int N,
                          int epi, const float* add, int64_t ldadd, float add_scale);
+int gm_linear_bwd_dx_gather(void* stream, const float* dA, int64_t lda, const float* W, float* dX, int64_t ldx,
+                            const float* below, int64_t ld_below, int M, int K, int N, int epi, const float* data,
+                            int64_t n_rows, const int64_t* idx, gm_slot idx_slot, float* out, int64_t ld_out, int B,
+                            int row_elems);
+int gm_linear_bwd_dx_gather_bits(void* stream, const float* dA, int64_t lda, const float* W, float* dX, int64_t ldx,
+                                 const float* below, int64_t ld_below, int M, int K, int N, int epi,
+                                 const uint32_t* bits, int words_per_row, int64_t n_rows, const int64_t* idx,
+                                 gm_slot idx_slot, float* out, int64_t ld_out, int B, int row_elems);
 
 #define GM_STD_WS_BYTES 1088
 int gm_std_all(void* stream, const float* X, int64_t ldx, int R, int I, float* out, void* ws);
```

Result: faster. 4.184 million images/sec, median of 6 (+5.6%).
